# YifanXu74/MQ-Det

Measured on AMD Instinct MI355X. Metric: images/sec MQ-GLIP-T 800×1333 5-shot vision queries, 1/2/4/8 MI355X, higher is better.
Workload: dtype f16; 1 GPU; BASELINE.json configs[1]: MQ-GLIP-T (Swin-T + BERT-base + GCP + 6-layer VLDyHead), 5 vision queries x 40 classes, 141-token caption, LVIS-style post-processing; every step a full forward (feature / language caches OFF; only host-side tokenizer / query-selection results are memoised)); global_batch=8, batch_per_gpu=8, image=800x1333 -> 800x1344, parallelism=dp1, weights=seeded random init (no checkpoints offline), residual_streams=fp32

## Files before the change

include/mqdet_hip.h:

```cpp
#ifndef MQDET_HIP_H
#define MQDET_HIP_H
#ifdef __cplusplus
extern "C" {
#endif

int mq_abi_version(void);

long mq_attn_workspace_bytes(int B, int H, int Nq, int D, int nsplit);
int mq_attn_fwd(const void* q, const void* k, const void* vt, void* o, const float* key_bias, const int* kv_len,
                const unsigned char* qk_mask, long mask_bs, long mask_hs, long mask_rs, void* workspace,
                int B, int H, int Nq, int Nk, int D,
                long q_bs, long q_rs, long q_hs, long k_bs, long k_rs, long k_hs, long vt_bs, long vt_rs, long vt_hs,
                long o_bs, long o_rs, long bias_bs, long bias_hs, float scale, float clamp, int nsplit, void* stream);

int mq_attn_resident_fwd(const void* q, const void* k, const void* vt, void* o, const float* key_bias, const int* kv_len,
                         const unsigned char* qk_mask, long mask_bs, long mask_hs, long mask_rs, int B, int H, int Nq, int Nk, int D,
                         long q_bs, long q_rs, long q_hs, long k_bs, long k_rs, long k_hs, long vt_bs, long vt_rs, long vt_hs,
                         long o_bs, long o_rs, long bias_bs, long bias_hs, float scale, float clamp, void* stream);

int mq_attn_chunked_fwd(const void* q, const void* k, const void* vt, void* o, const float* key_bias, const int* kv_len,
                        void* workspace, int B, int H, int Nq, int Nk, int D,
                        long q_bs, long q_rs, long q_hs, long k_bs, long k_rs, long k_hs, long vt_bs, long vt_rs, long vt_hs,
                        long o_bs, long o_rs, long bias_bs, long bias_hs, float scale, float clamp, int nsplit, void* stream);

int mq_window_attn_fwd(const void* qkv, const void* qkv_bias, const float* rel_bias, void* out,
                       int B, int H, int W, int C, int heads, int ws, int shift, void* stream);
int mq_window_attn_qkv_fwd(const void* x, const void* w, const void* bias, const float* rel_bias, void* out,
                           int B, int H, int W, int C, int heads, int ws, int shift, void* stream);

int mq_gcp_sparse_attn_fwd(const void* q, const void* kv, const int* idx, void* out, int B, int T, int V, int S,
                           int heads, int dim_head, void* stream);

int mq_gcp_gate_residual_fwd(const void* sup, const void* h, const void* w2, const void* x, int x_f32, void* out,
                             float* gate_out, long M, int C, int G, void* stream);

int mq_vlfuse_i2t_fwd(const void* v_ln, const void* kf, const void* vo, long kv_bs, long kv_hs, long kv_ts, const float* bias, const int* kv_len,
                      const void* out_bias, void* out, int B, int N, int T, int heads, int max_kv, float clamp, int variant,
                      void* stream);

long mq_vlfuse_t2i_workspace_bytes(int B, int T, int nsplit);
int mq_vlfuse_t2i_fwd(const void* kf, long kv_bs, long kv_hs, long kv_ts, const void* v_ln, const int* kv_len, const unsigned char* key_mask,
                      long key_mask_bs, void* workspace, void* out, int B, int N, int T, int heads, int nsplit, int max_kv, float clamp, int variant,
                      void* stream);

int mq_layernorm_fwd(const void* x, int x_f32, const void* res, int res_f32, const void* gamma, const void* beta, void* y,
                     float* y32, void* xsum, long rows, int C, float eps, void* stream);

int mq_layernorm2_fwd(const void* x, int x_f32, const void* res, int res_f32, const void* gamma, const void* beta, void* y,
                     float* y32, void* xsum, long rows, int C, float eps, void* stream);
int mq_layernorm_clamp_fwd(const void* x, int x_f32, const void* res, int res_f32, const void* gamma, const void* beta, void* y, float* y32,
                           void* xsum, long rows, int C, float eps, float clamp, void* stream);
int mq_clamp_gelu_clamp(const void* x, void* out, long n, float clamp, void* stream);

int mq_patch_merge_ln_fwd(const void* x, int x_f32, const void* gamma, const void* beta, void* y, int B, int H, int W, int C, float eps,
                          void* stream);

int mq_swin_mlp2_fwd(const float* x, const void* delta, const void* ln_g, const void* ln_b, float eps, const void* w1f,
                     const void* b1, const void* w2f, const void* b2, float* out, const void* next_g, const void* next_b,
                     float eps_next, void* y, long M, int C, int flags, void* stream);

int mq_conv3x3_fwd(const void* x, const void* w, const void* bias, void* out, int B, int H, int W, int C, long x_bs,
                   int N, int out_ld, int stride, void* stream);
int mq_conv3x3_nchw32_fwd(const void* x, const void* w, const void* bias, float* out, int B, int H, int W, int C, long x_bs,
                          int N, void* stream);

int mq_conv3x3_nchw32_v2_fwd(const void* x, const void* w, const void* bias, float* out, int B, int H, int W, int C, long x_bs,
                          int N, void* stream);
typedef struct mq_conv_level {
  const void* x; float* out; long x_bs; int H, W;
} mq_conv_level;
int mq_conv3x3_nchw32_group_fwd(const mq_conv_level* levels, int nl, const void* w, const void* bias, int B, int C, int N, void* stream);
int mq_pool2x2_tokens_fwd(const mq_conv_level* levels, int nl, void* out, int B, int C, void* stream);
int mq_dcnv2_stats_blocks(int H, int W, int stride);
typedef struct mq_dcn_branch {
  const void* x; const float* om; const void* w; const void* bias; void* out; float* stats; const float* wy; const float* wx;
  long x_bs;
  int B, H, W, C, oH, oW, N, out_ld, stride, flags;
} mq_dcn_branch;
int mq_dcnv2_group_fwd(const mq_dcn_branch* branches, int n, void* stream);
int mq_dcnv2_fwd(const void* x, const float* om, const void* w, const void* bias, void* out, float* stats, const float* wy,
                 const float* wx, int B, int H, int W, int C, long x_bs, int oH, int oW, int N, int out_ld, int stride,
                 int flags, void* stream);

int mq_dyconv_stats(const void* y, float* sums, const float* wy, const float* wx, int B, int n, int W, int C, void* stream);
typedef struct mq_coef_branch {
  const float* sums; const void* gamma; const void* beta; float* coef; int nblk, n, nbranches, reserved;
} mq_coef_branch;
int mq_dyconv_coef_group(const mq_coef_branch* branches, int nbr, const float* attn_w, const float* attn_b, int B, int C, int G,
                         float eps, void* stream);
int mq_dyconv_coef(const float* sums, const void* gamma, const void* beta, const float* attn_w, const float* attn_b,
                   float* coef, int B, int n, int nblk, int C, int G, float eps, int nbranches, void* stream);
int mq_dyconv_fuse(const void* y0, const float* coef0, int hs0, int ws0, const void* y1, const float* coef1, int hs1,
                   int ws1, const void* y2, const float* coef2, int hs2, int ws2, int nbranches, void* out, long out_bs,
                   float* pool, int B, int H, int W, int C, void* stream);
int mq_dyrelu_coef(const float* pool, const void* w0, const void* b0, const void* w2, const void* b2, float* coef,
                   int B, int n, int C, void* stream);
typedef struct mq_fuse_level {
  const void* y[3]; const float* coef[3]; int hs[3], ws[3];
  int nbranches, H, W, reserved;
  void* out; long out_bs; float* pool; float* relu_coef;
} mq_fuse_level;
int mq_dyconv_epilogue_group(const mq_fuse_level* levels, int nl, const void* w0, const void* b0, const void* w2, const void* b2,
                             int B, int C, void* stream);
int mq_dyrelu_apply(void* x, const float* coef, int B, int n, int C, long x_bs, void* stream);
int mq_add_upsample_nearest(void* dst, const void* src, int B, int H, int W, int Hc, int Wc, int C, void* stream);
int mq_dyrelu_ln_fwd(const void* x, long x_bs, const float* coef, const int* row_first, int NL, const void* gamma, const void* beta,
                     float eps, void* y, int B, int N, int C, void* stream);

int mq_align_scores_fwd(const void* dot, int dot_f32, const float* tbias, const int* tokidx, long tok_bs, const void* ctr,
                        float* out, float* cls_out, int B, int HW, int T, int L, int MT, float thr, long dot_bs, int agg,
                        void* stream);

int mq_align_fused_fwd(const void* tok, const void* tk, const float* tbias, const void* wbc, const float* bbc, const float* scales,
                       const int* tokidx, long tok_bs, const int* lvl_off, float* ranked, float* cls_out, float* reg, float* ctr_out,
                       float* logits, int B, int N, int T, int kv_max, int L, int MT, int NL, float thr, int agg, void* stream);

int mq_box_decode(const float* val, const long* flat, const void* reg, int reg_f32, const float* anchors, const int* label_ids, long lab_bs,
                  const float* im_wh, float* boxes, float* scores, int* labels, int B, int K, int HW, int L,
                  long out_stride, long out_off, void* stream);

int mq_roi_align_fwd(const void* feat, int feat_f32, const float* rois, float* out, int R, int C, int H, int W,
                     long sn, long sc, long sh, long sw, int PH, int PW, float spatial_scale, int sampling_ratio,
                     int aligned, int reduce_mean, void* stream);

int mq_msdeform_attn_fwd(const void* value, int value_f32, const long* shapes, const long* level_start, const float* loc,
                         const float* attn, void* out, int out_f32, int B, int S, int M, int D, int L, int Q, int P, void* stream);

int mq_msdeform_attn_q_fwd(const void* value, int value_f32, long value_bs, long value_ts, const long* shapes,
                           const long* level_start, const void* qproj, const float* ref, int ref_dim, const int* valid_hw,
                           void* out, int out_f32, int B, int S, int M, int D, int L, int Q, int P, void* stream);

long mq_ml_nms_workspace_bytes(int B, int N);
int mq_ml_nms(const float* boxes, const int* labels, const int* nvalid, void* workspace, unsigned char* keep,
              int B, int N, float thr, void* stream);

int mq_ml_nms_topk(const float* boxes, const int* labels, const int* nvalid, void* workspace, unsigned char* keep,
                   int B, int N, float thr, int max_keep, void* stream);

int mq_patch_embed_fwd(const void* img, int img_f32, const void* w, const float* bias, const float* g0, const float* b0, const float* g1,
                       const float* b1, float* x32, void* h1, int B, int Hi, int Wi, int C, float eps, void* stream);

int mq_attn_text_fwd(const void* q, const void* k, const void* v, void* o, const float* key_bias, const int* kv_len,
                     int B, int H, int Nq, int Nk, int D, long q_bs, long q_rs, long q_hs, long k_bs, long k_rs, long k_hs,
                     long v_bs, long v_rs, long v_hs, long o_bs, long o_rs, long bias_bs, long bias_hs, float scale,
                     float clamp, int max_kv, void* stream);

long mq_post_select_workspace_bytes(const int* hw, const int* k, int NL, int B, int L);
int mq_post_select_fwd(const float* const* ranked, const float* const* reg, const float* const* anchors, const int* hw, const int* k,
                       int NL, int B, int L, const int* label_ids, long lab_bs, const float* im_wh, void* workspace, float* boxes,
                       float* scores, int* labels, int* ids, void* stream);
int mq_post_sort_fwd(const float* boxes, const float* scores, const int* labels, const int* off, int NL, float* boxes_o, float* scores_o,
                     int* labels_o, int* nvalid, int B, int tot, void* stream);
int mq_post_finalize_fwd(const float* boxes, const float* scores, const int* labels, const unsigned char* keep, float* out,
                         int* counts, int B, int tot, int K, int K2, void* stream);

int mq_tta_ingest_fwd(const unsigned char* src, const long* src_off, const int* meta, const int* bounds, const int* coef, float* out,
                      float* out_flip, int* err, int B, int Hp, int Wp, int TH, int R, const float* mean, const float* stdv, int bgr, int x255,
                      void* stream);
int mq_tta_merge_prep(const float* packed, const int* counts, const float* tparam, const float* band, const int* cls_rank,
                      int n_cls, float* boxes, float* scores, int* labels, unsigned char* valid, float* boxes_s, float* scores_s,
                      int* labels_s, int* src_s, int* nvalid, int* ndrop, int T, int B, int K, void* stream);
int mq_tta_merge_finalize(const float* boxes_s, const float* scores_s, const int* labels_s, const int* src_s, const unsigned char* keep,
                          const int* nvalid, float* thr, const int* cls_rank, float* boxes_o, float* scores_o, long long* labels_o, int* counts, int B, int N,
                          int top_n, void* stream);

int mq_lvis_match(const int* pair_dt, const int* pair_gt, const unsigned char* pair_nel, const float* dt_box, const double* gt_box,
                  const double* gt_area, const unsigned char* gt_ign, const unsigned char* gt_nz, const double* area_rng, const double* iou_thr,
                  unsigned long long* dt_bits, int* gt_count, unsigned char* ws, int P, long Ng, void* stream);
int mq_lvis_accumulate(const int* cat_off, const int* order, const unsigned long long* dt_bits, const int* num_gt, const double* rec_thr,
                       double* precision, double* recall, int K, void* stream);

int mq_bank_admit(const float* cand, const long long* sorted_labels, const long long* order, float* pool, float* inv_norm, int* slots, int* counts,
                  int* state, int N, int D, int pool_rows, int cap, int label_lo, int num_labels, int maxq, int exclude, float thr, void* stream);

int mq_gcp_attn_fwd(const float* x, float* x_out, void* y, float* gate_out, const void* kv, const int* idx, const void* wq, const void* wout,
                    const void* wg1, const void* w2, const void* ln_a_g, const void* ln_a_b, const void* ln_g_g, const void* ln_g_b,
                    const void* ln_f_g, const void* ln_f_b, long M, int T, int V, int S, int C, int heads, int dim_head, int G, float eps,
                    int rows_per_block, void* stream);

int mq_bert_attn_qkv_fwd(const void* x, const void* w, const void* bias, void* o, const float* key_bias, const int* kv_len,
                         int B, int T, int C, int H, long x_bs, long x_rs, long o_bs, long o_rs, long bias_bs, float scale, float clamp,
                         void* stream);

#ifdef __cplusplus
#define MQ_BF16_TWIN(name) extern decltype(name) name##_bf16;
#else
#define MQ_BF16_TWIN(name) extern __typeof__(name) name##_bf16;
#endif
MQ_BF16_TWIN(mq_attn_fwd)
MQ_BF16_TWIN(mq_attn_resident_fwd)
MQ_BF16_TWIN(mq_attn_text_fwd)
MQ_BF16_TWIN(mq_bert_attn_qkv_fwd)
MQ_BF16_TWIN(mq_patch_embed_fwd)
MQ_BF16_TWIN(mq_attn_chunked_fwd)
MQ_BF16_TWIN(mq_window_attn_fwd)
MQ_BF16_TWIN(mq_window_attn_qkv_fwd)
MQ_BF16_TWIN(mq_gcp_sparse_attn_fwd)
MQ_BF16_TWIN(mq_gcp_gate_residual_fwd)
MQ_BF16_TWIN(mq_gcp_attn_fwd)
MQ_BF16_TWIN(mq_vlfuse_i2t_fwd)
MQ_BF16_TWIN(mq_vlfuse_t2i_fwd)
MQ_BF16_TWIN(mq_layernorm_fwd)
MQ_BF16_TWIN(mq_layernorm2_fwd)
MQ_BF16_TWIN(mq_layernorm_clamp_fwd)
MQ_BF16_TWIN(mq_clamp_gelu_clamp)
MQ_BF16_TWIN(mq_patch_merge_ln_fwd)
MQ_BF16_TWIN(mq_swin_mlp2_fwd)
MQ_BF16_TWIN(mq_conv3x3_fwd)
MQ_BF16_TWIN(mq_conv3x3_nchw32_fwd)
MQ_BF16_TWIN(mq_conv3x3_nchw32_v2_fwd)
MQ_BF16_TWIN(mq_conv3x3_nchw32_group_fwd)
MQ_BF16_TWIN(mq_dcnv2_fwd)
MQ_BF16_TWIN(mq_dcnv2_group_fwd)
MQ_BF16_TWIN(mq_dyconv_stats)
MQ_BF16_TWIN(mq_dyconv_coef)
MQ_BF16_TWIN(mq_dyconv_coef_group)
MQ_BF16_TWIN(mq_dyconv_fuse)
MQ_BF16_TWIN(mq_dyrelu_coef)
MQ_BF16_TWIN(mq_dyconv_epilogue_group)
MQ_BF16_TWIN(mq_dyrelu_apply)
MQ_BF16_TWIN(mq_add_upsample_nearest)
MQ_BF16_TWIN(mq_pool2x2_tokens_fwd)
MQ_BF16_TWIN(mq_dyrelu_ln_fwd)
MQ_BF16_TWIN(mq_align_scores_fwd)
MQ_BF16_TWIN(mq_align_fused_fwd)
MQ_BF16_TWIN(mq_box_decode)
MQ_BF16_TWIN(mq_roi_align_fwd)
MQ_BF16_TWIN(mq_msdeform_attn_fwd)
MQ_BF16_TWIN(mq_msdeform_attn_q_fwd)

#ifdef __cplusplus
#define MQ_F32_TWIN(name) extern decltype(name) name##_f32;
#else
#define MQ_F32_TWIN(name) extern __typeof__(name) name##_f32;
#endif
MQ_F32_TWIN(mq_attn_fwd)
MQ_F32_TWIN(mq_attn_resident_fwd)
MQ_F32_TWIN(mq_attn_text_fwd)
MQ_F32_TWIN(mq_bert_attn_qkv_fwd)
MQ_F32_TWIN(mq_patch_embed_fwd)
MQ_F32_TWIN(mq_attn_chunked_fwd)
MQ_F32_TWIN(mq_window_attn_fwd)
MQ_F32_TWIN(mq_window_attn_qkv_fwd)
MQ_F32_TWIN(mq_gcp_sparse_attn_fwd)
MQ_F32_TWIN(mq_gcp_gate_residual_fwd)
MQ_F32_TWIN(mq_gcp_attn_fwd)
MQ_F32_TWIN(mq_vlfuse_i2t_fwd)
MQ_F32_TWIN(mq_vlfuse_t2i_fwd)
MQ_F32_TWIN(mq_layernorm_fwd)
MQ_F32_TWIN(mq_layernorm2_fwd)
MQ_F32_TWIN(mq_layernorm_clamp_fwd)
MQ_F32_TWIN(mq_clamp_gelu_clamp)
MQ_F32_TWIN(mq_patch_merge_ln_fwd)
MQ_F32_TWIN(mq_swin_mlp2_fwd)
MQ_F32_TWIN(mq_conv3x3_fwd)
MQ_F32_TWIN(mq_conv3x3_nchw32_fwd)
MQ_F32_TWIN(mq_conv3x3_nchw32_v2_fwd)
MQ_F32_TWIN(mq_conv3x3_nchw32_group_fwd)
MQ_F32_TWIN(mq_dcnv2_fwd)
MQ_F32_TWIN(mq_dcnv2_group_fwd)
MQ_F32_TWIN(mq_dyconv_stats)
MQ_F32_TWIN(mq_dyconv_coef)
MQ_F32_TWIN(mq_dyconv_coef_group)
MQ_F32_TWIN(mq_dyconv_fuse)
MQ_F32_TWIN(mq_dyrelu_coef)
MQ_F32_TWIN(mq_dyconv_epilogue_group)
MQ_F32_TWIN(mq_dyrelu_apply)
MQ_F32_TWIN(mq_dyrelu_ln_fwd)
MQ_F32_TWIN(mq_add_upsample_nearest)
MQ_F32_TWIN(mq_pool2x2_tokens_fwd)
MQ_F32_TWIN(mq_align_scores_fwd)
MQ_F32_TWIN(mq_align_fused_fwd)
MQ_F32_TWIN(mq_box_decode)
MQ_F32_TWIN(mq_msdeform_attn_fwd)
MQ_F32_TWIN(mq_msdeform_attn_q_fwd)

#ifdef __cplusplus
}
#endif
#endif
```

mq_det_amd/build.py:

```python
import os
import subprocess
import sys

HERE = os.path.dirname(os.path.abspath(__file__))
CSRC = os.path.join(HERE, "csrc")
LIB_DIR = os.path.join(HERE, "lib")
LIB = os.path.join(LIB_DIR, "libmqdet_hip.so")
SOURCES = ["api.hip", "attn.hip", "attn_resident.hip", "attn_text.hip", "bert_attn.hip", "vlfuse_attn.hip", "window_attn.hip", "patch_embed.hip", "gcp.hip", "gcp_fused.hip", "conv_igemm.hip", "conv_small.hip", "conv_small2.hip", "conv_small3.hip", "dcn_fused.hip", "layernorm.hip", "layernorm2.hip", "dyconv.hip", "post.hip", "post2.hip", "align_fused.hip", "nms2.hip", "roi_align.hip", "swin_mlp2.hip", "msda.hip", "tta.hip", "lvis_eval.hip", "query_bank.hip"]
F32_SKIP = ("roi_align.hip", "nms2.hip", "post2.hip", "tta.hip", "lvis_eval.hip", "query_bank.hip")
FLAGS = ["--offload-arch=gfx950", "-O3", "-std=c++17", "-fPIC"]
EXTRA_FLAGS = {"dcn_fused.hip": ["-fno-slp-vectorize"],
               "swin_mlp2.hip": ["-fno-slp-vectorize"],
               "attn_resident.hip": ["-fno-slp-vectorize", "-mllvm", "-amdgpu-mfma-vgpr-form"],
               "attn_text.hip": ["-fno-slp-vectorize", "-mllvm", "-amdgpu-mfma-vgpr-form"],
               "bert_attn.hip": ["-fno-slp-vectorize", "-mllvm", "-amdgpu-mfma-vgpr-form"]}


STAMP = os.path.join(LIB_DIR, "libmqdet_hip.stamp")


def _digest():
    import hashlib
    h = hashlib.sha256()
    deps = sorted(os.path.join(CSRC, f) for f in os.listdir(CSRC)) + [os.path.join(HERE, "..", "include", "mqdet_hip.h"), os.path.abspath(__file__)]
    for d in deps:
        if os.path.isfile(d):
            with open(d, "rb") as f:
                h.update(os.path.basename(d).encode() + b"\0" + f.read())
    return h.hexdigest()


def _stale():
    if not os.path.exists(LIB) or not os.path.exists(STAMP):
        return True
    with open(STAMP) as f:
        return f.read().strip() != _digest()


def build(force=False, verbose=True):
    if not force and not _stale():
        return LIB
    os.makedirs(LIB_DIR, exist_ok=True)
    digest = _digest()
    hipcc = os.environ.get("HIPCC", "/opt/rocm/bin/hipcc")
    objs = []
    procs = []
    for src in SOURCES:
        for suffix, defs in (("", []), ("_bf16", ["-DMQ_BF16"]), ("_f32", ["-DMQ_F32"])):
            if suffix and src == "api.hip":
                continue
            if suffix == "_f32" and src in F32_SKIP:
                continue
            obj = os.path.join(LIB_DIR, src.replace(".hip", suffix + ".o"))
            objs.append(obj)
            procs.append((src + suffix, subprocess.Popen([hipcc, *FLAGS, *EXTRA_FLAGS.get(src, []), *defs, "-c", os.path.join(CSRC, src), "-o", obj],
                                                         stdout=subprocess.PIPE, stderr=subprocess.STDOUT)))
    for src, p in procs:
        out, _ = p.communicate()
        if p.returncode != 0:
            raise RuntimeError(f"hipcc failed on {src}:\n{out.decode()}")
    subprocess.check_call([hipcc, "--offload-arch=gfx950", "-shared", "-fPIC", *objs, "-o", LIB])
    with open(STAMP, "w") as f:
        f.write(digest)
    if verbose:
        print(f"built {LIB}")
    return LIB


if __name__ == "__main__":
    build(force="--force" in sys.argv)
```

mq_det_amd/modeling/pipeline.py:

```python
import math
import os

import torch
import torch.nn.functional as F

from .. import ops

NEG = -1.0e30


def _pack_swin(P, sd, SW, p, device, dtype):
    def h(name):
        return sd[name].detach().to(device=device, dtype=dtype).contiguous()
    ws = SW.WINDOW_SIZE
    N = ws * ws
    for i, (depth, heads) in enumerate(zip(SW.DEPTHS, SW.NUM_HEADS)):
        for j in range(depth):
            b = f"{p}.layers.{i}.blocks.{j}.attn"
            idx = sd[b + ".relative_position_index"].to(device).reshape(-1)
            rel = sd[b + ".relative_position_bias_table"].detach().to(device=device, dtype=torch.float32)[idx]
            rel = rel.reshape(N, N, heads).permute(2, 0, 1)
            NP = ops.window_pad(ws)
            P[b + ".rel_bias"] = F.pad(rel, (0, NP - N, 0, NP - N)).contiguous()
    P["_swin_fused_mlp"] = bool(SW.get("FUSED_MLP", True)) and P["_r32"] and ops.KERNELS["SWIN_MLP_VARIANT"] == 2
    P["_swin_fused_widths"] = tuple(w for w in SW.get("FUSED_MLP_WIDTHS", ops.SWIN_MLP_WIDTHS) if w in ops.SWIN_MLP_WIDTHS)
    for i, depth in enumerate(SW.DEPTHS):
        Ci = SW.EMBED_DIM * 2 ** i
        if P["_swin_fused_mlp"] and Ci in P["_swin_fused_widths"]:
            for j in range(depth):
                b = f"{p}.layers.{i}.blocks.{j}.mlp"
                P[b + ".w1f"], P[b + ".w2f"] = ops.swin_mlp2_pack(h(b + ".fc1.weight"), h(b + ".fc2.weight"))
    w = sd[p + ".patch_embed.proj.weight"].detach().to(device=device, dtype=torch.float32)
    P[p + ".patch_embed.lin"] = w.permute(0, 2, 3, 1).reshape(w.shape[0], -1).to(dtype).contiguous()
    if w.shape[0] in (96, 192) and tuple(w.shape[1:]) == (3, 4, 4):
        P[p + ".patch_embed.wpk"] = ops.patch_embed_pack(w).to(dtype).contiguous()
        P[p + ".patch_embed.wpk_nchw"] = ops.patch_embed_pack(w, nchw=True).to(dtype).contiguous()
        P[p + ".patch_embed.f32"] = [sd[n].detach().to(device=device, dtype=torch.float32).contiguous() for n in
                                     (p + ".patch_embed.proj.bias", p + ".patch_embed.norm.weight", p + ".patch_embed.norm.bias",
                                      p + ".layers.0.blocks.0.norm1.weight", p + ".layers.0.blocks.0.norm1.bias")]


def _pack_language(P, sd, cfg, p, device, dtype):
    def h(name):
        return sd[name].detach().to(device=device, dtype=dtype).contiguous()

    def f32(name):
        return sd[name].detach().to(device=device, dtype=torch.float32).contiguous()
    LB = cfg.MODEL.LANGUAGE_BACKBONE
    nl = LB.get("NUM_HIDDEN_LAYERS", 12)
    for i in range(nl):
        _pack_bert_layer(P, sd, f"{p}.encoder.layer.{i}", device, dtype)
    if cfg.VISION_QUERY.ENABLED:
        qv0 = LB.get("QV_START", 6)
        for i in range(nl - qv0):
            b = f"{p}.encoder.qv_layer.{i}"
            P[b + ".ff.linear2.gated"] = (f32(b + ".ff.linear2.weight") * torch.tanh(f32(b + ".ff_gate"))).to(dtype)
            P[b + ".attn_gate.w2"] = h(b + ".attn_gate.linear2.weight").reshape(-1)
            for n in (".attn.to_q", ".attn.to_out", ".attn_gate.linear1"):
                _pack_frag(P, b + n + ".frag", h(b + n + ".weight"))
        for i in range(2):
            b = f"{p}.pre_select.layers.{i}.image_condition"
            wkv = h(b + ".to_kv.weight")
            half = wkv.shape[0] // 2
            P[b + ".to_k.weight"], P[b + ".to_v.weight"] = wkv[:half].contiguous(), wkv[half:].contiguous()


def _pack_frag(P, key, w):
    if w.shape[0] % 16 == 0 and w.shape[1] % 32 == 0:
        P[key] = ops.pack_b_fragments(w)


def _pack_bert_layer(P, sd, b, device, dtype):
    def h(name):
        return sd[name].detach().to(device=device, dtype=dtype).contiguous()
    P[b + ".qk.weight"] = torch.cat([h(b + ".attention.self.query.weight"), h(b + ".attention.self.key.weight")], 0)
    P[b + ".qk.bias"] = torch.cat([h(b + ".attention.self.query.bias"), h(b + ".attention.self.key.bias")], 0)
    P[b + ".qkv.weight"] = torch.cat([P[b + ".qk.weight"], h(b + ".attention.self.value.weight")], 0)
    P[b + ".qkv.bias"] = torch.cat([P[b + ".qk.bias"], h(b + ".attention.self.value.bias")], 0)
    _pack_frag(P, b + ".qkv.frag", P[b + ".qkv.weight"])


def _dcn_tiles(P, key):
    if ops.dcn_bdma():
        P[key + ".tiles"] = ops.dcn_weight_tiles(P[key + ".packed"])


def _dcn_w(P, key):
    return P[key + ".tiles"] if (ops.dcn_bdma() and (key + ".tiles") in P) else P[key + ".packed"]


def build_plan(sd, cfg, device, dtype=torch.float16):
    P = {}
    M = cfg.MODEL
    P["_r32"] = bool(M.get("RESIDUAL_FP32", True))

    def h(name):
        return sd[name].detach().to(device=device, dtype=dtype).contiguous()

    def f32(name):
        return sd[name].detach().to(device=device, dtype=torch.float32).contiguous()
    for k, v in sd.items():
        if v.dtype.is_floating_point:
            P[k] = v.detach().to(device=device, dtype=dtype).contiguous()
    _pack_swin(P, sd, M.SWINT, "backbone.body", device, dtype)
    for k in list(P):
        if torch.is_tensor(P[k]) and P[k].dim() == 4:
            P[k] = P[k].contiguous(memory_format=torch.channels_last)
    _pack_language(P, sd, cfg, "language_backbone.body.model", device, dtype)

    def bert(b):
        _pack_bert_layer(P, sd, b, device, dtype)
    D = M.DYHEAD
    hd = 2048 // 8
    for i in range(D.NUM_CONVS):
        b = f"rpn.head.dyhead_tower.{3 * i}.b_attn"
        sc = hd ** -0.5
        P[b + ".q.weight"] = (f32(b + ".attn.v_proj.weight") * sc).to(dtype)
        P[b + ".q.bias"] = (f32(b + ".attn.v_proj.bias") * sc).to(dtype)
        gv, gl = f32(b + ".gamma_v"), f32(b + ".gamma_l")
        P[b + ".ov.weight"] = (f32(b + ".attn.out_v_proj.weight") * gv[:, None]).to(dtype)
        P[b + ".ov.bias"] = (f32(b + ".attn.out_v_proj.bias") * gv).to(dtype)
        P[b + ".ol.weight"] = (f32(b + ".attn.out_l_proj.weight") * gl[:, None]).to(dtype)
        P[b + ".ol.bias"] = (f32(b + ".attn.out_l_proj.bias") * gl).to(dtype)
        P[b + ".Wov8"] = P[b + ".ov.weight"].reshape(-1, 8, hd).permute(1, 2, 0).contiguous()
        P[b + ".Wq8"] = P[b + ".q.weight"].reshape(8, hd, -1).contiguous()
        P[b + ".bq8"] = (f32(b + ".attn.v_proj.bias") * sc).reshape(8, hd).contiguous()
        wol = (f32(b + ".attn.out_l_proj.weight") * gl[:, None]).reshape(-1, 8, hd)
        wvv = f32(b + ".attn.values_v_proj.weight").reshape(8, hd, -1)
        P[b + ".olc.weight"] = torch.einsum("ohe,hec->ohc", wol, wvv).reshape(wol.shape[0], -1).to(dtype).contiguous()
        P[b + ".olc.bias"] = (torch.einsum("ohe,he->o", wol, f32(b + ".attn.values_v_proj.bias").reshape(8, hd))
                              + f32(b + ".attn.out_l_proj.bias") * gl).to(dtype)
        wl = f32(b + ".attn.l_proj.weight").reshape(8, hd, -1)
        bl = f32(b + ".attn.l_proj.bias").reshape(8, hd)
        wvl = f32(b + ".attn.values_l_proj.weight").reshape(8, hd, -1)
        bvl = f32(b + ".attn.values_l_proj.bias").reshape(8, hd)
        wq8 = (f32(b + ".attn.v_proj.weight") * sc).reshape(8, hd, -1)
        bq8 = (f32(b + ".attn.v_proj.bias") * sc).reshape(8, hd)
        wov8 = (f32(b + ".attn.out_v_proj.weight") * gv[:, None]).reshape(-1, 8, hd).permute(1, 2, 0)
        w_kf = torch.einsum("hec,hek->hck", wq8, wl).reshape(8 * wq8.shape[2], -1)
        b_kf = torch.einsum("hec,he->hc", wq8, bl).reshape(-1)
        w_vo = torch.einsum("heo,hek->hok", wov8, wvl).reshape(8 * wov8.shape[2], -1)
        b_vo = torch.einsum("heo,he->ho", wov8, bvl).reshape(-1)
        w_b = torch.einsum("he,hek->hk", bq8, wl)
        b_b = (bq8 * bl).sum(-1)
        z = w_b.new_zeros(8, w_b.shape[1])
        P[b + ".tprep.weight"] = torch.cat([w_kf, w_vo, w_b, z], 0).to(dtype).contiguous()
        P[b + ".tprep.bias"] = torch.cat([b_kf, b_vo, b_b, b_b.new_zeros(8)], 0).to(dtype).contiguous()
        bert(f"rpn.head.dyhead_tower.{3 * i + 1}")
        b = f"rpn.head.dyhead_tower.{3 * i + 2}"
        for k in range(3):
            w = f32(f"{b}.DyConv.{k}.conv.weight")
            P[f"{b}.DyConv.{k}.packed"] = w.permute(0, 2, 3, 1).reshape(w.shape[0], -1).to(dtype).contiguous()
            _dcn_tiles(P, f"{b}.DyConv.{k}")
        wo = f32(b + ".offset.weight").permute(0, 2, 3, 1).reshape(27, -1)
        P[b + ".offset.packed"] = torch.cat([wo, wo.new_zeros(5, wo.shape[1])], 0).to(dtype).contiguous()
        P[b + ".attn_w"] = f32(b + ".AttnConv.1.weight").reshape(-1)
        P[b + ".attn_b"] = f32(b + ".AttnConv.1.bias")
    for n in ("fpn_layer2", "fpn_layer3", "fpn_layer4", "top_blocks.p6", "top_blocks.p7"):
        w = f32(f"backbone.fpn.{n}.weight")
        P[f"backbone.fpn.{n}.packed"] = w.permute(0, 2, 3, 1).reshape(w.shape[0], -1).to(dtype).contiguous()
        _dcn_tiles(P, f"backbone.fpn.{n}")
    for n in ("fpn_inner2", "fpn_inner3", "fpn_inner4"):
        P[f"backbone.fpn.{n}.lin"] = h(f"backbone.fpn.{n}.weight").reshape(sd[f"backbone.fpn.{n}.weight"].shape[0], -1).contiguous()
    for l in range(5):
        s = f32(f"rpn.head.scales.{l}.scale")
        wb = (f32("rpn.head.bbox_pred.weight") * s).reshape(4, -1)
        wc = f32("rpn.head.centerness.weight").reshape(1, -1)
        P[f"rpn.head.boxctr.{l}.weight"] = torch.cat([wb, wc, wb.new_zeros(3, wb.shape[1])], 0).to(dtype).contiguous()
        P[f"rpn.head.boxctr.{l}.bias"] = torch.cat([f32("rpn.head.bbox_pred.bias") * s, f32("rpn.head.centerness.bias"),
                                                    wb.new_zeros(3)], 0).to(dtype).contiguous()
    wbc = torch.cat([f32("rpn.head.bbox_pred.weight").reshape(4, -1), f32("rpn.head.centerness.weight").reshape(1, -1)], 0)
    P["rpn.head.wbc"] = torch.cat([wbc, wbc.new_zeros(11, wbc.shape[1])], 0).to(dtype).contiguous()
    P["rpn.head.bbc"] = torch.cat([f32("rpn.head.bbox_pred.bias"), f32("rpn.head.centerness.bias"), wbc.new_zeros(3)], 0).contiguous()
    P["rpn.head.scales"] = torch.cat([f32(f"rpn.head.scales.{l}.scale").reshape(1) for l in range(5)], 0).contiguous()
    P["rpn.head.tok.weight"] = f32("rpn.head.dot_product_projection_text.weight")
    P["rpn.head.tok.bias"] = f32("rpn.head.dot_product_projection_text.bias")
    P["rpn.head.bias_lang32"] = f32("rpn.head.bias_lang")
    P["rpn.head.bias0_32"] = f32("rpn.head.bias0")
    P["rpn.head.inv_scale"] = float(math.exp(-float(sd["rpn.head.log_scale"])))
    for l in range(5):
        P[f"anchors.cell.{l}"] = f32(f"rpn.anchor_generator.cell_anchors.{l}")
    return P


def _ln(P, name, x, eps=1e-5, **kw):
    return ops.layer_norm(x.contiguous(), P[name + ".weight"], P[name + ".bias"], eps, **kw)


def _add_ln(P, name, x, res, eps=1e-5, **kw):
    return ops.layer_norm(x.contiguous(), P[name + ".weight"], P[name + ".bias"], eps, residual=res.contiguous(), **kw)


def _lin(P, name, x):
    return F.linear(x, P[name + ".weight"], P.get(name + ".bias"))


_NSPLIT_TARGET = int(os.environ.get("MQ_NSPLIT_TARGET", "768"))


def _nsplit(n_blocks, n_key_tiles, target=None):
    target = target or _NSPLIT_TARGET
    if n_blocks >= 256 or n_key_tiles < 8:
        return 1
    return max(1, min(n_key_tiles // 4, -(-target // n_blocks), 32))


def _nsplit_t2i(n_img, heads, t_live, n_key_tiles, cus_per_xcd=32):
    if n_key_tiles < 8:
        return 1
    members = -(-(heads * (-(-t_live // 16))) // 8)
    best, best_cost = 1, None
    for ns in range(1, min(32, n_key_tiles // 4) + 1):
        per_xcd = -(-(n_img * ns) // 8) * members
        cost = (-(-per_xcd // cus_per_xcd)) * (-(-n_key_tiles // ns) + 6)
        if best_cost is None or cost < best_cost:
            best, best_cost = ns, cost
    return best


def swin_forward(P, cfg, img, p="backbone.body", SW=None):
    M = SW if SW is not None else cfg.MODEL.SWINT
    ws = M.WINDOW_SIZE
    _, _, H0, W0 = img.shape
    if W0 % 4 or H0 % 4:
        img = F.pad(img, (0, (4 - W0 % 4) % 4, 0, (4 - H0 % 4) % 4))
    B, Cin, Hi, Wi = img.shape
    H, W = Hi // 4, Wi // 4
    r32 = P["_r32"]
    h1_first = None
    nhwc = img.permute(0, 2, 3, 1)
    pe = ops.KERNELS["PATCH_EMBED_FUSED"] == 1 and r32 and Cin == 3 and (p + ".patch_embed.wpk") in P
    if pe and img.dtype == torch.float32 and img.is_contiguous():
        x, h1_first = ops.patch_embed(img, P[p + ".patch_embed.wpk_nchw"], *P[p + ".patch_embed.f32"], eps=1e-5)
    elif pe and img.dtype != torch.float32 and nhwc.is_contiguous():
        x, h1_first = ops.patch_embed(nhwc, P[p + ".patch_embed.wpk"], *P[p + ".patch_embed.f32"], eps=1e-5)
    else:
        if img.dtype == torch.float32:
            nhwc = nhwc.to(P[p + ".patch_embed.lin"].dtype)
        patches = nhwc.reshape(B, H, 4, W, 4, Cin).permute(0, 1, 3, 2, 4, 5).reshape(B, H * W, 16 * Cin)
        x = F.linear(patches, P[p + ".patch_embed.lin"], P[p + ".patch_embed.proj.bias"])
        x = _ln(P, p + ".patch_embed.norm", x, want_y=not r32, want_y32=r32)
    outs = []
    for i, (depth, heads) in enumerate(zip(M.DEPTHS, M.NUM_HEADS)):
        C = x.shape[-1]
        fused = P["_swin_fused_mlp"] and C in P["_swin_fused_widths"] and x.dtype == torch.float32
        pend = None
        h1 = None
        if i == 0 and h1_first is not None:
            h1 = h1_first
        for j in range(depth):
            b = f"{p}.layers.{i}.blocks.{j}"
            shift = 0 if j % 2 == 0 else ws // 2
            if h1 is None:
                if pend is None:
                    h1 = _ln(P, b + ".norm1", x)
                else:
                    h1, x = _add_ln(P, b + ".norm1", pend, x)
            if ops.window_qkv_fused(C, ws, h1.numel()):
                a = ops.window_attention_qkv(h1.reshape(B, H, W, C), P[b + ".attn.qkv.weight"], P[b + ".attn.qkv.bias"],
                                             P[b + ".attn.rel_bias"], heads, ws, shift)
            else:
                qkv = _lin(P, b + ".attn.qkv", h1).reshape(B, H, W, 3 * C)
                a = ops.window_attention(qkv, P[b + ".attn.qkv.bias"], P[b + ".attn.rel_bias"], heads, ws, shift)
            proj = _lin(P, b + ".attn.proj", a.reshape(B, H * W, C))
            if fused:
                nxt = f"{p}.layers.{i}.blocks.{j + 1}.norm1" if j + 1 < depth else (f"{p}.norm{i}" if i > 0 else None)
                nln = None if nxt is None else (P[nxt + ".weight"], P[nxt + ".bias"], 1e-5)
                r = ops.swin_mlp2(x.contiguous(), proj.contiguous(), P[b + ".norm2.weight"], P[b + ".norm2.bias"], 1e-5,
                                  P[b + ".mlp.w1f"], P[b + ".mlp.fc1.bias"], P[b + ".mlp.w2f"], P[b + ".mlp.fc2.bias"], next_ln=nln)
                x, h1 = r if nxt is not None else (r, None)
                pend = None
            else:
                h2, x = _add_ln(P, b + ".norm2", proj, x)
                pend = _lin(P, b + ".mlp.fc2", F.gelu(_lin(P, b + ".mlp.fc1", h2)))
                h1 = None
        if fused:
            if i > 0:
                outs.append(h1.reshape(B, H, W, C))
        elif i > 0:
            o, x = _add_ln(P, f"{p}.norm{i}", pend, x)
            outs.append(o.reshape(B, H, W, C))
        else:
            x = x + pend
        if i < len(M.DEPTHS) - 1:
            d = f"{p}.layers.{i}.downsample"
            if ops.KERNELS["PATCH_MERGE_FUSED"] == 1:
                yn = ops.patch_merge_ln(x.reshape(B, H, W, C).contiguous(), P[d + ".norm.weight"], P[d + ".norm.bias"], 1e-5)
                H, W = (H + 1) // 2, (W + 1) // 2
            else:
                y = x.reshape(B, H, W, C)
                if H % 2 or W % 2:
                    y = F.pad(y, (0, 0, 0, W % 2, 0, H % 2))
                y = torch.cat([y[:, 0::2, 0::2], y[:, 1::2, 0::2], y[:, 0::2, 1::2], y[:, 1::2, 1::2]], -1)
                H, W = (H + 1) // 2, (W + 1) // 2
                yn = _ln(P, d + ".norm", y.reshape(B, H * W, 4 * C))
            wr = P[d + ".reduction.weight"]
            if r32 and yn.is_cuda and yn.dtype != torch.float32 and os.environ.get("MQ_SWIN_RED_F32OUT") == "1":
                x = torch.mm(yn.reshape(-1, yn.shape[-1]), wr.t(), out_dtype=torch.float32).view(B, H * W, wr.shape[0])
            else:
                x = F.linear(yn, wr)
                if r32:
                    x = x.float()
    return outs


def fpn_forward(P, feats_nhwc):
    p = "backbone.fpn"
    c3, c4, c5 = feats_nhwc

    def lateral(name, x):
        return F.linear(x, P[f"{p}.{name}.lin"], P[f"{p}.{name}.bias"])

    def conv3(name, x, stride=1):
        return ops.conv3x3(x, P[f"{p}.{name}.packed"], P[f"{p}.{name}.bias"], P[f"{p}.{name}.packed"].shape[0], stride)
    via_dcn = ops.KERNELS["FPN_VIA_DCN"] == 1
    inner = lateral("fpn_inner4", c5)
    inners = [("fpn_layer4", inner)]
    for feat, idx in ((c4, 3), (c3, 2)):
        lat = lateral(f"fpn_inner{idx}", feat)
        if ops.KERNELS["FPN_TOPDOWN_FUSED"] == 1:
            inner = ops.add_upsample_nearest_(lat.contiguous(), inner.contiguous())
        else:
            up = F.interpolate(inner.permute(0, 3, 1, 2), size=lat.shape[1:3], mode="nearest").permute(0, 2, 3, 1)
            inner = (lat + up).contiguous()
        inners.insert(0, (f"fpn_layer{idx}", inner))
    if via_dcn:
        outs = ops.dcnv2_group([dict(x=x, om=_zero_offsets(x.shape[0], x.shape[1], x.shape[2], x.device), w=_dcn_w(P, f"{p}.{n}"),
                                     bias=P[f"{p}.{n}.bias"], stride=1, plain=True) for n, x in inners], want_stats=False, tag="dcnv2_fpn")
        res = [y.reshape(x.shape[0], hw[0], hw[1], 256) for (y, hw, _), (_, x) in zip(outs, inners)]

        def conv3s2(name, x):
            Ho, Wo = (x.shape[1] - 1) // 2 + 1, (x.shape[2] - 1) // 2 + 1
            y, hw = ops.dcnv2(x, _zero_offsets(x.shape[0], Ho, Wo, x.device), _dcn_w(P, f"{p}.{name}"), P[f"{p}.{name}.bias"], 2, tag="dcnv2_fpn", plain=True)
            return y.reshape(x.shape[0], hw[0], hw[1], 256)
        p6 = conv3s2("top_blocks.p6", res[-1])
        p7 = conv3s2("top_blocks.p7", F.relu(p6))
    else:
        res = [conv3(n, x) for n, x in inners]
        p6 = conv3("top_blocks.p6", res[-1], 2)
        p7 = conv3("top_blocks.p7", F.relu(p6), 2)
    return [t.permute(0, 3, 1, 2) for t in res + [p6, p7]]


_ZERO_OM = {}


def _zero_offsets(B, Ho, Wo, device):
    key = (B, Ho, Wo, str(device))
    if key not in _ZERO_OM:
        if len(_ZERO_OM) > 64:
            _ZERO_OM.clear()
        om = torch.zeros(B, 27, Ho, Wo, dtype=torch.float32, device=device)
        om[:, 18:] = 100.0
        _ZERO_OM[key] = om
    return _ZERO_OM[key]


def pooled_fpn_tokens(feats):
    if ops.KERNELS.get("POOLED_TOKENS_FUSED", 0) == 1 and ops.pool2x2_tokens_supported(feats):
        return ops.pool2x2_tokens(feats)
    return torch.cat([F.avg_pool2d(f, 2).permute(0, 2, 3, 1).flatten(1, 2) for f in feats], 1)


def bert_layer(P, b, x, key_bias, clamp, kv_len=None, x32=None, qk_mask=None, max_kv=0):
    Bn, T, C = x.shape
    r32 = x32 is not None
    if ops.KERNELS["BERT_ATTN_QKV_FUSED"] >= 1 and qk_mask is None and (b + ".qkv.frag") in P and ops.bert_attention_qkv_fits(T, C, 12, key_bias, batch=Bn):
        ctx = ops.bert_attention_qkv(x, P[b + ".qkv.frag"], P[b + ".qkv.bias"], 12, key_bias=key_bias, clamp=50000.0 if clamp else 0.0, kv_len=kv_len, packed=True)
    elif ops.KERNELS["BERT_QKV_FUSED"] == 1 and qk_mask is None and ops.attention_text_fits(T, kv_len, max_kv) and (b + ".qkv.weight") in P \
            and (key_bias is None or key_bias.dim() == 2):
        ctx = ops.attention_text(_lin(P, b + ".qkv", x), 12, key_bias=key_bias, clamp=50000.0 if clamp else 0.0, kv_len=kv_len, max_kv=max_kv)
    else:
        qk = _lin(P, b + ".qk", x)
        vt = torch.baddbmm(P[b + ".attention.self.value.bias"][None, :, None], P[b + ".attention.self.value.weight"][None]
                           .expand(Bn, -1, -1), x.transpose(1, 2))
        ctx = ops.attention(qk[:, :, :C], qk[:, :, C:], vt, 12, C // 12, key_bias=key_bias, clamp=50000.0 if clamp else 0.0,
                            kv_len=kv_len, qk_mask=qk_mask)
    a = _add_ln(P, b + ".attention.output.LayerNorm", _lin(P, b + ".attention.output.dense", ctx), x32 if r32 else x, 1e-12,
                want_sum=False, want_y32=r32)
    a16, a32 = a if r32 else (a, None)
    hmid = _lin(P, b + ".intermediate.dense", a16)
    if clamp and ops.KERNELS["BERT_CLAMP_FUSED"] == 1 and hmid.numel() % 8 == 0:
        o = _lin(P, b + ".output.dense", ops.clamp_gelu_clamp(hmid.contiguous(), 50000.0))
        return ops.layer_norm(o.contiguous(), P[b + ".output.LayerNorm.weight"], P[b + ".output.LayerNorm.bias"], 1e-12,
                              residual=(a32 if r32 else a16).contiguous(), want_sum=False, want_y32=r32, clamp=50000.0)
    if clamp:
        hmid = F.gelu(hmid.clamp(-50000, 50000)).clamp(-50000, 50000)
        o = _lin(P, b + ".output.dense", hmid).clamp(-50000, 50000)
    else:
        o = _lin(P, b + ".output.dense", F.gelu(hmid))
    y = _add_ln(P, b + ".output.LayerNorm", o, a32 if r32 else a16, 1e-12, want_sum=False, want_y32=r32)
    if not r32:
        return y.clamp(-50000, 50000) if clamp else y
    y16, y32 = y
    if clamp:
        y16, y32 = y16.clamp(-50000, 50000), y32.clamp(-50000, 50000)
    return y16, y32


def pre_select(P, p, vision, image, scale, side_ok=False):
    vision, image = vision * scale, image * scale
    Bn, Np, C = image.shape
    pad = (-Np) % 8
    if pad:
        image = F.pad(image, (0, 0, 0, pad))

    def image_kv(i):
        ic = f"{p}.layers.{i}.image_condition"
        kn = _ln(P, ic + ".norm_kv", image)
        return F.linear(kn, P[ic + ".to_k.weight"]), torch.matmul(P[ic + ".to_v.weight"], kn.transpose(1, 2))
    ahead = None
    if side_ok and image.is_cuda:
        main, side = torch.cuda.current_stream(), _side_streams(image.device, 1, "pre_kv")[0]
        side.wait_stream(main)
        with torch.cuda.stream(side):
            ahead = image_kv(1)
    for i in range(2):
        b = f"{p}.layers.{i}"
        ic = b + ".image_condition"
        q = F.linear(_ln(P, ic + ".norm", vision), P[ic + ".to_q.weight"])
        if i == 1 and ahead is not None:
            main.wait_stream(side)
            k, vt = ahead
        else:
            k, vt = image_kv(i)
        nq_tiles = -(-q.shape[1] // 128)
        att = ops.attention(q, k, vt, 8, 32, nk=Np, nsplit=_nsplit(nq_tiles * Bn * 8, -(-Np // 64)))
        v16 = vision if vision.dtype == image.dtype else vision.to(image.dtype)
        res = F.linear(v16, P[b + ".res_mapping.weight"]) if (b + ".res_mapping.weight") in P else vision
        att_o = F.linear(att, P[ic + ".to_out.weight"])
        vision = att_o.float() + res.float() if P["_r32"] else att_o + res
        ff = b + ".ff"
        vision = vision + F.linear(F.gelu(F.linear(_ln(P, ff + ".norm", vision), P[ff + ".linear1.weight"])),
                                   P[ff + ".linear2.weight"])
    return vision


def gcp_kv(P, b, vision):
    return F.linear(_ln(P, b + ".attn.norm_kv", vision), P[b + ".attn.to_kv.weight"])


def gcp_block(P, b, x, vision, idx, gates=None, kv=None):
    if kv is None:
        kv = gcp_kv(P, b, vision)
    ff = b + ".ff"
    if ops.KERNELS["GCP_ATTN_FUSED"] >= 1 and (b + ".attn.to_q.frag") in P and ops.gcp_attention_fits(x, idx, policy=True):
        def ln(n):
            return (P[n + ".weight"], P[n + ".bias"])
        r = ops.gcp_attention(x.contiguous(), kv.contiguous(), idx, P[b + ".attn.to_q.frag"], P[b + ".attn.to_out.frag"], P[b + ".attn_gate.linear1.frag"],
                              P[b + ".attn_gate.w2"], ln(b + ".attn.norm"), ln(b + ".attn_gate.norm"), ln(ff + ".norm"), want_gate=gates is not None,
                              packed=True)
        x, xn = r[0], r[1]
        if gates is not None:
            gates.append(r[2])
        return x + F.linear(F.gelu(F.linear(xn, P[ff + ".linear1.weight"])), P[ff + ".linear2.gated"])
    q = F.linear(_ln(P, b + ".attn.norm", x), P[b + ".attn.to_q.weight"])
    sup = F.linear(ops.gcp_sparse_attention(q, kv, idx), P[b + ".attn.to_out.weight"])
    gh = F.linear(_ln(P, b + ".attn_gate.norm", sup), P[b + ".attn_gate.linear1.weight"])
    if gates is not None:
        x, g = ops.gcp_gate_residual(sup, gh, P[b + ".attn_gate.w2"], x.contiguous(), want_gate=True)
        gates.append(g)
    else:
        x = ops.gcp_gate_residual(sup, gh, P[b + ".attn_gate.w2"], x.contiguous())
    return x + F.linear(F.gelu(F.linear(_ln(P, ff + ".norm", x), P[ff + ".linear1.weight"])), P[ff + ".linear2.gated"])


def language_front(P, cfg, input_ids, attention_mask, use_vq, p="language_backbone.body.model", position_ids=None, qk_mask=None, max_kv=0):
    LB = cfg.MODEL.LANGUAGE_BACKBONE
    T = input_ids.shape[1]
    pe = P[p + ".embeddings.position_embeddings.weight"]
    e = P[p + ".embeddings.word_embeddings.weight"][input_ids].float() \
        + P[p + ".embeddings.token_type_embeddings.weight"][0].float() \
        + (pe[:T].float()[None] if position_ids is None else pe[position_ids].float())
    x32 = F.layer_norm(e, (e.shape[-1],), P[p + ".embeddings.LayerNorm.weight"].float(),
                       P[p + ".embeddings.LayerNorm.bias"].float(), 1e-12)
    x = x32.to(P[p + ".embeddings.LayerNorm.weight"].dtype)
    if not P["_r32"]:
        x32 = None
    key_bias = kv_len = None
    if attention_mask is not None:
        key_bias = ((1.0 - attention_mask.float()) * NEG).contiguous()
        kv_len = (attention_mask.to(torch.int32) * torch.arange(1, T + 1, device=attention_mask.device, dtype=torch.int32)) \
            .amax(1).to(torch.int32).contiguous()
    nl, qv0 = LB.get("NUM_HIDDEN_LAYERS", 12), LB.get("QV_START", 6)
    n_front = qv0 if use_vq else nl
    hidden = []
    for i in range(n_front):
        x, x32 = _bert(P, f"{p}.encoder.layer.{i}", x, x32, key_bias, False, kv_len, qk_mask, max_kv=max_kv)
        hidden.append(x if x32 is None else x32)
    return {"x": x, "x32": x32, "hidden": hidden, "key_bias": key_bias, "kv_len": kv_len, "next": n_front, "qk_mask": qk_mask}


def _bert(P, b, x, x32, key_bias, clamp, kv_len, qk_mask=None, max_kv=0):
    if x32 is None:
        return bert_layer(P, b, x, key_bias, clamp, kv_len, qk_mask=qk_mask, max_kv=max_kv), None
    return bert_layer(P, b, x, key_bias, clamp, kv_len, x32=x32, qk_mask=qk_mask, max_kv=max_kv)


def language_backbone(P, cfg, input_ids, attention_mask, vision, images, idx, want_gates=False, front=None, max_kv=0, side_ok=False):
    p = "language_backbone.body.model"
    LB = cfg.MODEL.LANGUAGE_BACKBONE
    use_vq = vision is not None
    if front is None:
        front = language_front(P, cfg, input_ids, attention_mask, use_vq, max_kv=max_kv)
    x, x32, hidden, key_bias, kv_len = front["x"], front.get("x32"), list(front["hidden"]), front["key_bias"], front["kv_len"]
    nl, qv0 = LB.get("NUM_HIDDEN_LAYERS", 12), LB.get("QV_START", 6)
    kv_ahead, kv_join = {}, None
    if use_vq:
        vision = pre_select(P, p + ".pre_select", vision, images, cfg.VISION_QUERY.VISION_SCALE, side_ok=side_ok)
        first = max(front["next"], qv0)
        if side_ok and vision.is_cuda and nl - first > 1:
            main, side = torch.cuda.current_stream(), _side_streams(vision.device, 1, "gcp_kv")[0]
            side.wait_stream(main)
            with torch.cuda.stream(side):
                for i in range(first + 1, nl):
                    kv_ahead[i] = gcp_kv(P, f"{p}.encoder.qv_layer.{i - qv0}", vision)
            kv_join = (main, side)
    gates = [] if want_gates else None
    for i in range(front["next"], nl):
        if use_vq and i >= qv0:
            if kv_join is not None and i in kv_ahead:
                kv_join[0].wait_stream(kv_join[1])
                kv_join = None
            if x32 is None:
                x = gcp_block(P, f"{p}.encoder.qv_layer.{i - qv0}", x, vision, idx, gates, kv=kv_ahead.get(i))
            else:
                x32 = gcp_block(P, f"{p}.encoder.qv_layer.{i - qv0}", x32, vision, idx, gates, kv=kv_ahead.get(i))
                x = x32.to(x.dtype)
        x, x32 = _bert(P, f"{p}.encoder.layer.{i}", x, x32, key_bias, False, kv_len, max_kv=max_kv)
        hidden.append(x if x32 is None else x32)
    n = LB.N_LAYERS
    feats = hidden[-1].float() if n == 1 else torch.stack(hidden[-n:], 1).float().mean(1) / n
    m = attention_mask.unsqueeze(-1).float()
    embedded = feats * m
    aggregate = embedded.sum(1) / attention_mask.sum(-1, keepdim=True).float()
    return {"aggregate": aggregate, "embedded": embedded, "masks": attention_mask, "hidden": x, "hidden32": x32,
            "key_bias": key_bias, "kv_len": kv_len, "vision_query_gates": gates, "augmented_vision": vision}


def _to_tokens(feats):
    sizes = [tuple(f.shape[-2:]) for f in feats]
    return torch.cat([f.permute(0, 2, 3, 1).flatten(1, 2) for f in feats], 1), sizes


def _level_views(tok, sizes):
    Bn, N, C = tok.shape
    out, s = [], 0
    for (hh, ww) in sizes:
        out.append(tok[:, s:s + hh * ww].reshape(Bn, hh, ww, C).permute(0, 3, 1, 2))
        s += hh * ww
    return out


def vl_text_prep(P, b, hidden, key_bias, hidden32=None):
    Bn = hidden.shape[0]
    if hidden32 is not None:
        l_ln, l_res = _ln(P, b + ".layer_norm_l", hidden32, want_y32=True)
    else:
        l_ln = l_res = _ln(P, b + ".layer_norm_l", hidden)
    T = l_ln.shape[1]
    C = P[b + ".Wq8"].shape[2]
    t = _lin(P, b + ".tprep", l_ln)
    kf = t[..., :8 * C].unflatten(-1, (8, C)).permute(0, 2, 1, 3)
    vo = t[..., 8 * C:16 * C].unflatten(-1, (8, C)).permute(0, 2, 1, 3)
    bias = (t[..., 16 * C:16 * C + 8].float().permute(0, 2, 1) + key_bias[:, None, :]).contiguous()
    return {"l_ln": l_ln, "l_res": l_res, "kf": kf, "vo": vo, "bias": bias}


def vl_image_side(P, b, v_ln, prep, kv_len=None, max_kv=0):
    return ops.vlfuse_i2t(v_ln, prep["kf"], prep["vo"], prep["bias"], P[b + ".ov.bias"], kv_len=kv_len, max_kv=max_kv)


def vl_text_side(P, b, v_ln, prep, kv_len=None, max_kv=0):
    Bn, N, _ = v_ln.shape
    T = prep["l_ln"].shape[1]
    t_live = min(T, max_kv) if (kv_len is not None and max_kv > 0) else T
    out_l = ops.vlfuse_t2i(prep["kf"], v_ln, _nsplit_t2i(Bn, prep["kf"].shape[1], t_live, -(-N // 64)), kv_len=kv_len, max_kv=t_live)
    return prep["l_res"] + _lin(P, b + ".olc", out_l)


def vl_fuse_tokens(P, b, v, hidden, key_bias, kv_len=None, max_kv=0):
    v_ln = ops.layer_norm(v, P[b + ".layer_norm_v.weight"], P[b + ".layer_norm_v.bias"], 1e-5)
    prep = vl_text_prep(P, b, hidden, key_bias)
    return vl_image_side(P, b, v_ln, prep, kv_len, max_kv), vl_text_side(P, b, v_ln, prep, kv_len, max_kv)


def vl_fuse(P, b, feats, hidden, key_bias, kv_len=None, max_kv=0):
    v, sizes = _to_tokens(feats)
    v_new, l_new = vl_fuse_tokens(P, b, v.contiguous(), hidden, key_bias, kv_len, max_kv)
    return _level_views(v_new, sizes), l_new


_UP_W = {}


def _upsample_pool_weights(hs, ws, H, W, device):
    key = (hs, ws, H, W, device)
    if key not in _UP_W:
        def axis(n_src, n_dst):
            w = torch.zeros(n_src, dtype=torch.float64)
            for o in range(n_dst):
                s = o * (n_src - 1) / (n_dst - 1) if n_dst > 1 else 0.0
                i0 = min(int(s), n_src - 1)
                i1 = min(i0 + 1, n_src - 1)
                l = s - i0
                w[i0] += 1 - l
                w[i1] += l
            return (w / n_dst).float().to(device)
        _UP_W[key] = (axis(hs, H), axis(ws, W))
    return _UP_W[key]


def dyconv_tokens(P, cfg, b, tok, sizes, defer_relu=False):
    G = cfg.MODEL.GROUP_NORM
    nl = len(sizes)
    Bn, N, C = tok.shape
    offs = [0]
    for (hh, ww) in sizes:
        offs.append(offs[-1] + hh * ww)
    lv = [tok[:, offs[l]:offs[l + 1]].reshape(Bn, sizes[l][0], sizes[l][1], C) for l in range(nl)]
    out = torch.empty_like(tok)
    streams = bool(cfg.MODEL.DYHEAD.get("LEVEL_STREAMS", True) and tok.is_cuda and nl > 1)

    def fan_out(fn):
        if not streams:
            for l in range(nl):
                fn(l)
            return
        main = torch.cuda.current_stream()
        side = _side_streams(tok.device, max(1, min(nl - 1, _LEVEL_SIDE_STREAMS)))
        for s_ in side:
            s_.wait_stream(main)
        for l in range(1, nl):
            with torch.cuda.stream(side[(l - 1) % len(side)]):
                fn(l)
        fn(0)
        for s_ in side:
            main.wait_stream(s_)

    om = [None] * nl

    def offsets(lvl):
        om[lvl] = ops.conv3x3_nchw32(lv[lvl], P[b + ".offset.packed"], P[b + ".offset.bias"], 27)
    if ops.KERNELS["OFFSET_CONV_VARIANT"] == 3 and ops.conv3x3_nchw32_group_supported(lv, 27):
        om = ops.conv3x3_nchw32_group(lv, P[b + ".offset.packed"], P[b + ".offset.bias"], 27)
    else:
        fan_out(offsets)

    branches, owner = [], []
    for lvl in range(nl):
        H, W = sizes[lvl]
        spec = [(1, lv[lvl], 1)]
        if lvl > 0:
            spec.append((2, lv[lvl - 1], 2))
        if lvl < nl - 1:
            spec.append((0, lv[lvl + 1], 1))
        for k, x_nhwc, stride in spec:
            Ho, Wo = (x_nhwc.shape[1] - 1) // stride + 1, (x_nhwc.shape[2] - 1) // stride + 1
            wy = wx = None
            if (Ho, Wo) != (H, W):
                wy, wx = _upsample_pool_weights(Ho, Wo, H, W, tok.device)
            branches.append({"x": x_nhwc, "om": om[lvl], "w": _dcn_w(P, f"{b}.DyConv.{k}"), "bias": P[f"{b}.DyConv.{k}.conv.bias"],
                             "stride": stride, "wy": wy, "wx": wx})
            owner.append((lvl, k, len(spec)))
    ys = ops.dcnv2_group(branches, want_stats=True)
    coefs = ops.dyconv_coef_group(
        [{"sums": sums, "n": Ho * Wo, "gamma": P[f"{b}.DyConv.{k}.bn.weight"], "beta": P[f"{b}.DyConv.{k}.bn.bias"], "nbranches": nb}
         for (lvl, k, nb), (y, (Ho, Wo), sums) in zip(owner, ys)], P[b + ".attn_w"], P[b + ".attn_b"], G.NUM_GROUPS, G.EPSILON)

    relu_coef = torch.empty(nl, Bn, 4, C, dtype=torch.float32, device=tok.device) if defer_relu else None

    def epilogue(lvl):
        H, W = sizes[lvl]
        fused = [(y, coef, Ho, Wo) for (l2, k, nb), (y, (Ho, Wo), sums), coef in zip(owner, ys, coefs) if l2 == lvl]
        o = out[:, offs[lvl]:offs[lvl + 1]]
        _, pool = ops.dyconv_fuse(fused, H, W, out=o)
        rw = (P[b + ".relu.fc.0.weight"], P[b + ".relu.fc.0.bias"], P[b + ".relu.fc.2.weight"], P[b + ".relu.fc.2.bias"])
        if defer_relu:
            ops.dyrelu_coef(pool, H * W, *rw, out=relu_coef[lvl])
        else:
            ops.dyrelu_(o, pool, *rw)
    if ops.KERNELS["DYCONV_EPILOGUE_GROUPED"] == 1 and C == 256 and nl <= 8:
        rw = (P[b + ".relu.fc.0.weight"], P[b + ".relu.fc.0.bias"], P[b + ".relu.fc.2.weight"], P[b + ".relu.fc.2.bias"])
        rc = relu_coef if defer_relu else torch.empty(nl, Bn, 4, C, dtype=torch.float32, device=tok.device)
        ops.dyconv_epilogue_group(
            [([(y, coef, Ho, Wo) for (l2, k, nb), (y, (Ho, Wo), sums), coef in zip(owner, ys, coefs) if l2 == lvl], sizes[lvl][0], sizes[lvl][1],
              out[:, offs[lvl]:offs[lvl + 1]]) for lvl in range(nl)], *rw, rc)
        if not defer_relu:
            fan_out(lambda lvl: ops.dyrelu_apply_(out[:, offs[lvl]:offs[lvl + 1]], rc[lvl]))
    else:
        fan_out(epilogue)
    return (out, relu_coef) if defer_relu else out


def dyconv(P, cfg, b, feats):
    tok, sizes = _to_tokens(feats)
    return _level_views(dyconv_tokens(P, cfg, b, tok.contiguous(), sizes), sizes)


_SIDE_STREAMS = {}
_LEVEL_SIDE_STREAMS = int(os.environ.get("MQ_LEVEL_SIDE_STREAMS", "4"))


_STREAM_PRIORITY = dict((kv.split(":")[0], int(kv.split(":")[1])) for kv in os.environ.get("MQ_STREAM_PRIORITY", "").split(",") if ":" in kv)


def _side_streams(device, n, tag="levels"):
    key = (device.index, n, tag)
    if key not in _SIDE_STREAMS:
        _SIDE_STREAMS[key] = [torch.cuda.Stream(device=device, priority=_STREAM_PRIORITY.get(tag, 0)) for _ in range(n)]
    return _SIDE_STREAMS[key]


def vldyhead(P, cfg, feats, lang, trace=None):
    p = "rpn.head"
    hidden, key_bias, kv_len = lang["hidden"], lang["key_bias"], lang.get("kv_len")
    h32 = lang.get("hidden32")
    max_kv = lang.get("max_kv", 0)
    tok, sizes = _to_tokens(feats)
    tok = tok.contiguous()
    L = cfg.MODEL.DYHEAD.NUM_CONVS
    t = f"{p}.dyhead_tower"
    two_streams = bool(tok.is_cuda and cfg.MODEL.DYHEAD.get("LEVEL_STREAMS", True)) and trace is None

    def text_side(b, v_ln, prep):
        hnew = vl_text_side(P, b, v_ln, prep, kv_len, max_kv)
        return (hnew.to(tok.dtype), hnew) if h32 is not None else (hnew, None)

    defer = ops.KERNELS["DYRELU_IN_LN"] == 1 and tok.shape[-1] == 256 and len(sizes) <= 8
    relu_coef = None

    def relu_applied_copy():
        if relu_coef is None:
            return tok
        cp, off = tok.clone(), 0
        for l, (hh, ww) in enumerate(sizes):
            ops.dyrelu_apply_(cp[:, off:off + hh * ww], relu_coef[l])
            off += hh * ww
        return cp

    def norm_v(b):
        if relu_coef is not None:
            return ops.dyrelu_layer_norm(tok, relu_coef, sizes, P[b + ".layer_norm_v.weight"], P[b + ".layer_norm_v.bias"], 1e-5)
        return ops.layer_norm(tok, P[b + ".layer_norm_v.weight"], P[b + ".layer_norm_v.bias"], 1e-5)

    def dyconv_layer(i):
        if defer and i + 1 < L:
            return dyconv_tokens(P, cfg, f"{t}.{3 * i + 2}", tok, sizes, defer_relu=True)
        return dyconv_tokens(P, cfg, f"{t}.{3 * i + 2}", tok, sizes), None

    if not two_streams:
        for i in range(L):
            b = f"{t}.{3 * i}.b_attn"
            v_ln = norm_v(b)
            prep = vl_text_prep(P, b, hidden, key_bias, h32)
            tok = vl_image_side(P, b, v_ln, prep, kv_len, max_kv)
            hidden, h32 = text_side(b, v_ln, prep)
            rec = {"fuse_tok": tok, "fuse_hidden": hidden if h32 is None else h32}
            hidden, h32 = _bert(P, f"{t}.{3 * i + 1}", hidden, h32, key_bias, True, kv_len, max_kv=max_kv)
            tok, relu_coef = dyconv_layer(i)
            if trace is not None:
                rec.update(bert_hidden=hidden if h32 is None else h32, dyconv_tok=relu_applied_copy())
                trace.append(rec)
    else:
        main, text = torch.cuda.current_stream(), _side_streams(tok.device, 1, "text")[0]
        text.wait_stream(main)
        with torch.cuda.stream(text):
            prep = vl_text_prep(P, f"{t}.0.b_attn", hidden, key_bias, h32)
        keep = []
        for i in range(L):
            b = f"{t}.{3 * i}.b_attn"
            v_ln = norm_v(b)
            main.wait_stream(text)
            keep.clear()
            keep.append(v_ln)
            text.wait_stream(main)
            cur = prep
            with torch.cuda.stream(text):
                hidden, h32 = text_side(b, v_ln, cur)
                hidden, h32 = _bert(P, f"{t}.{3 * i + 1}", hidden, h32, key_bias, True, kv_len, max_kv=max_kv)
                if i + 1 < L:
                    prep = vl_text_prep(P, f"{t}.{3 * (i + 1)}.b_attn", hidden, key_bias, h32)
            tok = vl_image_side(P, b, v_ln, cur, kv_len, max_kv)
            tok, relu_coef = dyconv_layer(i)
        main.wait_stream(text)
        keep.clear()
    emb = F.normalize((hidden if h32 is None else h32).float(), p=2, dim=-1)
    tk = F.linear(emb / 2.0, P[p + ".tok.weight"], P[p + ".tok.bias"]) * P[p + ".inv_scale"]
    tbias = (emb @ P[p + ".bias_lang32"] + P[p + ".bias0_32"]).contiguous()
    live = min(tk.shape[1], max_kv) if max_kv > 0 else tk.shape[1]
    fits = ops.f32_operands() != 1 or -(-live // 16) * 16 <= 144
    if ops.KERNELS["ALIGN_FUSED"] == 1 and tk.shape[1] <= 256 and tok.shape[-1] == 256 and len(sizes) <= 8 and fits:
        return {"tok": tok, "sizes": sizes, "tk16": tk.to(tok.dtype).contiguous(), "tbias": tbias, "max_kv": max_kv,
                "wbc": P[p + ".wbc"], "bbc": P[p + ".bbc"], "scales": P[p + ".scales"],
                "feats": _level_views(tok, sizes), "hidden": hidden if h32 is None else h32}
    tok16_t = tk.to(tok.dtype).transpose(1, 2)
    Bn, N, C = tok.shape
    dots_all = torch.bmm(tok, tok16_t)
    bbox, ctr, dots = [], [], []
    off = 0
    for l, (H, W) in enumerate(sizes):
        tokens = tok[:, off:off + H * W]
        bc = F.linear(tokens, P[f"{p}.boxctr.{l}.weight"], P[f"{p}.boxctr.{l}.bias"]).reshape(Bn, H, W, 8)
        bbox.append(bc[..., :4].permute(0, 3, 1, 2))
        ctr.append(bc[..., 4:5].permute(0, 3, 1, 2))
        dots.append(dots_all[:, off:off + H * W])
        off += H * W
    return {"bbox_reg": bbox, "centerness": ctr, "dot": dots, "tbias": tbias, "feats": _level_views(tok, sizes),
            "hidden": hidden if h32 is None else h32}


def grid_anchors(P, sizes, strides, device):
    out = []
    for l, ((H, W), s) in enumerate(zip(sizes, strides)):
        sx = torch.arange(0, W * s, step=s, dtype=torch.float32, device=device)
        sy = torch.arange(0, H * s, step=s, dtype=torch.float32, device=device)
        yy, xx = torch.meshgrid(sy, sx, indexing="ij")
        sh = torch.stack([xx.reshape(-1), yy.reshape(-1), xx.reshape(-1), yy.reshape(-1)], 1)
        out.append((sh[:, None, :] + P[f"anchors.cell.{l}"][None]).reshape(-1, 4).contiguous())
    return out


TIE_SLOTS = 16


def postprocess(cfg, head, anchors, im_wh, tokidx, label_ids, want_cls=False, level_streams=None):
    A = cfg.MODEL.ATSS
    dev = head["tbias"].device
    Bn = head["tbias"].shape[0]
    L = tokidx.shape[-2]
    if not torch.is_tensor(im_wh):
        im_wh = torch.tensor([[w, h] for (h, w) in im_wh], dtype=torch.float32, device=dev)
    agg = ops.SCORE_AGG[str(cfg.MODEL.DYHEAD.get("SCORE_AGG", "MEAN")).upper()]
    fused = None
    if "tok" in head:
        fused = ops.align_fused(head["tok"], head["tk16"], head["tbias"], head["wbc"], head["bbc"], head["scales"], tokidx, head["sizes"],
                                A.INFERENCE_TH, agg=agg, kv_max=head.get("max_kv", 0), want_cls=want_cls, want_logits=want_cls)
        hws = [h * w for (h, w) in head["sizes"]]
        if want_cls:
            T = head["tbias"].shape[1]
            offs_ = [0]
            for n_ in hws:
                offs_.append(offs_[-1] + n_)
            head["dot"] = [fused["logits"][:, offs_[l]:offs_[l + 1]] for l in range(len(hws))]
            head["bbox_reg"] = [fused["reg"][l].reshape(Bn, h, w, 4).permute(0, 3, 1, 2) for l, (h, w) in enumerate(head["sizes"])]
            head["centerness"] = [fused["ctr"][:, offs_[l]:offs_[l + 1]].reshape(Bn, 1, h, w) for l, (h, w) in enumerate(head["sizes"])]
    else:
        hws = [d.shape[1] for d in head["dot"]]
    ks = [min(A.PRE_NMS_TOP_N, hw * L) for hw in hws]
    tot = sum(ks)
    Kd = int(A.DETECTIONS_PER_IMG)
    K = min(Kd, tot) if Kd > 0 else tot
    K2 = min(K + int(A.get("TIE_SLOTS", TIE_SLOTS)), tot) if Kd > 0 else tot
    if ops.KERNELS["POST_FUSED"] == 1 and tot <= 16384 and (Kd <= 0 or tot <= 6656) and all(a.shape[0] == hw for a, hw in zip(anchors, hws)) \
            and ops.post_select_supported(hws, ks, Bn, L):
        if fused is not None:
            ranked_l, reg_l = fused["ranked"], fused["reg"]
            cls_all = fused["cls"] if want_cls else None
        else:
            ranked_l, reg_l, cls_all = [], [], []
            for l, HW in enumerate(hws):
                ctr_flat = head["centerness"][l].permute(0, 2, 3, 1).reshape(Bn, HW).contiguous()
                r = ops.align_scores(head["dot"][l], head["tbias"], tokidx, ctr_flat, A.INFERENCE_TH, want_cls=want_cls, agg=agg)
                if want_cls:
                    r, c_ = r
                    cls_all.append(c_)
                ranked_l.append(r.float().contiguous())
                reg_l.append(head["bbox_reg"][l].permute(0, 2, 3, 1).reshape(Bn, HW, 4).float().contiguous())
        lab32 = label_ids if label_ids.dtype == torch.int32 else label_ids.to(torch.int32)
        wh32 = im_wh if (im_wh.dtype == torch.float32 and im_wh.is_contiguous()) else im_wh.float().contiguous()
        ub, us, ul, uid = ops.post_select(ranked_l, reg_l, [a.contiguous() for a in anchors], ks, lab32.contiguous(), wh32)
        boxes, scores, labels, nvalid = ops.post_sort(ub, us, ul, ks)
        keep8 = ops.ml_nms(boxes, labels, nvalid, A.NMS_TH, max_keep=K2 if Kd > 0 else 0, as_bool=False)
        packed, cnt = ops.post_finalize(boxes, scores, labels, keep8, K, K2)
        out = {"boxes": packed[..., :4], "scores": packed[..., 4], "labels": packed[..., 5].to(torch.int64), "counts": cnt & 0xFFFF,
               "tie_overflow": (cnt >> 16) > 0, "packed": packed, "counts_packed": cnt,
               "pre_nms": {"boxes": boxes, "scores": scores, "labels": labels, "nvalid": nvalid, "keep": keep8.bool()}}
        if want_cls:
            out["cls"] = cls_all
        return out
    boxes = torch.empty(Bn, tot, 4, dtype=torch.float32, device=dev)
    scores = torch.empty(Bn, tot, dtype=torch.float32, device=dev)
    labels = torch.empty(Bn, tot, dtype=torch.int32, device=dev)
    cls_all = [None] * len(ks)
    offs = [0]
    for k in ks:
        offs.append(offs[-1] + k)

    def level(l):
        anc, k, HW = anchors[l], ks[l], hws[l]
        if fused is not None:
            r, reg_nhwc = fused["ranked"][l], fused["reg"][l]
            if want_cls:
                cls_all[l] = fused["cls"][l]
        else:
            dot, reg, ctr = head["dot"][l], head["bbox_reg"][l], head["centerness"][l]
            ctr_flat = ctr.permute(0, 2, 3, 1).reshape(Bn, HW).contiguous()
            r = ops.align_scores(dot, head["tbias"], tokidx, ctr_flat, A.INFERENCE_TH, want_cls=want_cls, agg=agg)
            if want_cls:
                r, cls_all[l] = r
            reg_nhwc = reg.permute(0, 2, 3, 1).reshape(Bn, HW, 4).contiguous()
        val, flat = torch.topk(r.reshape(Bn, HW * L), k, dim=1, sorted=False)
        ops.box_decode(val.contiguous(), flat.contiguous(), reg_nhwc, anc, label_ids, im_wh, boxes, scores, labels, HW, L, offs[l])

    if level_streams is None:
        level_streams = cfg.MODEL.DYHEAD.get("LEVEL_STREAMS", True)
    if boxes.is_cuda and level_streams and len(ks) > 1:
        main = torch.cuda.current_stream()
        side = _side_streams(dev, len(ks) - 1)
        for s_ in side:
            s_.wait_stream(main)
        for l in range(1, len(ks)):
            with torch.cuda.stream(side[l - 1]):
                level(l)
        level(0)
        for s_ in side:
            main.wait_stream(s_)
    else:
        for l in range(len(ks)):
            level(l)
    order = torch.argsort(scores, dim=1, descending=True, stable=True)
    scores = torch.gather(scores, 1, order)
    labels = torch.gather(labels, 1, order.to(torch.int64)).contiguous()
    boxes = torch.gather(boxes, 1, order[:, :, None].expand(-1, -1, 4)).contiguous()
    nvalid = (scores > 0).sum(1).to(torch.int32)
    keep = ops.ml_nms(boxes, labels, nvalid, A.NMS_TH, max_keep=K2 if Kd > 0 else 0)
    kept_scores = torch.where(keep, scores, torch.full_like(scores, -1.0))
    top, ti = torch.topk(kept_scores, K2, dim=1, sorted=True)
    if K2 > K:
        tie = top[:, K:] == top[:, K - 1:K]
        top = torch.cat([top[:, :K], torch.where(tie, top[:, K:], torch.full_like(top[:, K:], -1.0))], 1)
    overflow = ((top[:, K2 - 1] == top[:, K - 1]) & (top[:, K - 1] > 0)) if 0 < K < K2 < tot else torch.zeros(Bn, dtype=torch.bool, device=dev)
    out = {"boxes": torch.gather(boxes, 1, ti[:, :, None].expand(-1, -1, 4)), "scores": top,
           "labels": torch.gather(labels, 1, ti).to(torch.int64), "counts": (top > 0).sum(1), "tie_overflow": overflow,
           "pre_nms": {"boxes": boxes, "scores": scores, "labels": labels, "nvalid": nvalid, "keep": keep}}
    if want_cls:
        out["cls"] = cls_all
    return out
```

mq_det_amd/ops.py:

```python
import ctypes
import math
import os

import torch

_LIB = None
_LIB_PATH = os.path.join(os.path.dirname(os.path.abspath(__file__)), "lib", "libmqdet_hip.so")

_vp, _i, _l, _f = ctypes.c_void_p, ctypes.c_int, ctypes.c_long, ctypes.c_float
EXPECTED_ABI = 31
_SIGNATURES = {
    "mq_abi_version": (_i, []),
    "mq_attn_workspace_bytes": (_l, [_i, _i, _i, _i, _i]),
    "mq_attn_fwd": (_i, [_vp, _vp, _vp, _vp, _vp, _vp, _vp, _l, _l, _l, _vp, _i, _i, _i, _i, _i] + [_l] * 13 + [_f, _f, _i, _vp]),
    "mq_attn_resident_fwd": (_i, [_vp, _vp, _vp, _vp, _vp, _vp, _vp, _l, _l, _l, _i, _i, _i, _i, _i] + [_l] * 13 + [_f, _f, _vp]),
    "mq_patch_embed_fwd": (_i, [_vp, _i, _vp, _vp, _vp, _vp, _vp, _vp, _vp, _vp, _i, _i, _i, _i, _f, _vp]),
    "mq_attn_text_fwd": (_i, [_vp, _vp, _vp, _vp, _vp, _vp, _i, _i, _i, _i, _i] + [_l] * 13 + [_f, _f, _i, _vp]),
    "mq_bert_attn_qkv_fwd": (_i, [_vp, _vp, _vp, _vp, _vp, _vp, _i, _i, _i, _i, _l, _l, _l, _l, _l, _f, _f, _vp]),
    "mq_attn_chunked_fwd": (_i, [_vp, _vp, _vp, _vp, _vp, _vp, _vp, _i, _i, _i, _i, _i] + [_l] * 13 + [_f, _f, _i, _vp]),
    "mq_window_attn_fwd": (_i, [_vp, _vp, _vp, _vp, _i, _i, _i, _i, _i, _i, _i, _vp]),
    "mq_window_attn_qkv_fwd": (_i, [_vp, _vp, _vp, _vp, _vp, _i, _i, _i, _i, _i, _i, _i, _vp]),
    "mq_gcp_sparse_attn_fwd": (_i, [_vp, _vp, _vp, _vp, _i, _i, _i, _i, _i, _i, _vp]),
    "mq_gcp_gate_residual_fwd": (_i, [_vp, _vp, _vp, _vp, _i, _vp, _vp, _l, _i, _i, _vp]),
    "mq_gcp_attn_fwd": (_i, [_vp] * 16 + [_l, _i, _i, _i, _i, _i, _i, _i, _f, _i, _vp]),
    "mq_vlfuse_i2t_fwd": (_i, [_vp, _vp, _vp, _l, _l, _l, _vp, _vp, _vp, _vp, _i, _i, _i, _i, _i, _f, _i, _vp]),
    "mq_vlfuse_t2i_workspace_bytes": (_l, [_i, _i, _i]),
    "mq_vlfuse_t2i_fwd": (_i, [_vp, _l, _l, _l, _vp, _vp, _vp, _l, _vp, _vp, _i, _i, _i, _i, _i, _i, _f, _i, _vp]),
    "mq_layernorm_fwd": (_i, [_vp, _i, _vp, _i, _vp, _vp, _vp, _vp, _vp, _l, _i, _f, _vp]),
    "mq_layernorm2_fwd": (_i, [_vp, _i, _vp, _i, _vp, _vp, _vp, _vp, _vp, _l, _i, _f, _vp]),
    "mq_layernorm_clamp_fwd": (_i, [_vp, _i, _vp, _i, _vp, _vp, _vp, _vp, _vp, _l, _i, _f, _f, _vp]),
    "mq_clamp_gelu_clamp": (_i, [_vp, _vp, _l, _f, _vp]),
    "mq_patch_merge_ln_fwd": (_i, [_vp, _i, _vp, _vp, _vp, _i, _i, _i, _i, _f, _vp]),
    "mq_swin_mlp2_fwd": (_i, [_vp, _vp, _vp, _vp, _f, _vp, _vp, _vp, _vp, _vp, _vp, _vp, _f, _vp, _l, _i, _i, _vp]),
    "mq_conv3x3_fwd": (_i, [_vp, _vp, _vp, _vp, _i, _i, _i, _i, _l, _i, _i, _i, _vp]),
    "mq_conv3x3_nchw32_fwd": (_i, [_vp, _vp, _vp, _vp, _i, _i, _i, _i, _l, _i, _vp]),
    "mq_conv3x3_nchw32_v2_fwd": (_i, [_vp, _vp, _vp, _vp, _i, _i, _i, _i, _l, _i, _vp]),
    "mq_conv3x3_nchw32_group_fwd": (_i, [_vp, _i, _vp, _vp, _i, _i, _i, _vp]),
    "mq_dcnv2_stats_blocks": (_i, [_i, _i, _i]),
    "mq_dcnv2_fwd": (_i, [_vp, _vp, _vp, _vp, _vp, _vp, _vp, _vp, _i, _i, _i, _i, _l, _i, _i, _i, _i, _i, _i, _vp]),
    "mq_dcnv2_group_fwd": (_i, [_vp, _i, _vp]),
    "mq_dyconv_stats": (_i, [_vp, _vp, _vp, _vp, _i, _i, _i, _i, _vp]),
    "mq_dyconv_coef": (_i, [_vp, _vp, _vp, _vp, _vp, _vp, _i, _i, _i, _i, _i, _f, _i, _vp]),
    "mq_dyconv_coef_group": (_i, [_vp, _i, _vp, _vp, _i, _i, _i, _f, _vp]),
    "mq_dyconv_fuse": (_i, [_vp, _vp, _i, _i, _vp, _vp, _i, _i, _vp, _vp, _i, _i, _i, _vp, _l, _vp, _i, _i, _i, _i, _vp]),
    "mq_dyrelu_coef": (_i, [_vp, _vp, _vp, _vp, _vp, _vp, _i, _i, _i, _vp]),
    "mq_dyconv_epilogue_group": (_i, [_vp, _i, _vp, _vp, _vp, _vp, _i, _i, _vp]),
    "mq_add_upsample_nearest": (_i, [_vp, _vp, _i, _i, _i, _i, _i, _i, _vp]),
    "mq_pool2x2_tokens_fwd": (_i, [_vp, _i, _vp, _i, _i, _vp]),
    "mq_dyrelu_ln_fwd": (_i, [_vp, _l, _vp, _vp, _i, _vp, _vp, _f, _vp, _i, _i, _i, _vp]),
    "mq_dyrelu_apply": (_i, [_vp, _vp, _i, _i, _i, _l, _vp]),
    "mq_align_scores_fwd": (_i, [_vp, _i, _vp, _vp, _l, _vp, _vp, _vp, _i, _i, _i, _i, _i, _f, _l, _i, _vp]),
    "mq_align_fused_fwd": (_i, [_vp, _vp, _vp, _vp, _vp, _vp, _vp, _l, _vp, _vp, _vp, _vp, _vp, _vp, _i, _i, _i, _i, _i, _i, _i, _f, _i, _vp]),
    "mq_box_decode": (_i, [_vp, _vp, _vp, _i, _vp, _vp, _l, _vp, _vp, _vp, _vp, _i, _i, _i, _i, _l, _l, _vp]),
    "mq_roi_align_fwd": (_i, [_vp, _i, _vp, _vp, _i, _i, _i, _i, _l, _l, _l, _l, _i, _i, _f, _i, _i, _i, _vp]),
    "mq_msdeform_attn_fwd": (_i, [_vp, _i, _vp, _vp, _vp, _vp, _vp, _i, _i, _i, _i, _i, _i, _i, _i, _vp]),
    "mq_msdeform_attn_q_fwd": (_i, [_vp, _i, _l, _l, _vp, _vp, _vp, _vp, _i, _vp, _vp, _i, _i, _i, _i, _i, _i, _i, _i, _vp]),
    "mq_post_select_workspace_bytes": (_l, [_vp, _vp, _i, _i, _i]),
    "mq_post_select_fwd": (_i, [_vp, _vp, _vp, _vp, _vp, _i, _i, _i, _vp, _l, _vp, _vp, _vp, _vp, _vp, _vp, _vp]),
    "mq_post_sort_fwd": (_i, [_vp, _vp, _vp, _vp, _i, _vp, _vp, _vp, _vp, _i, _i, _vp]),
    "mq_post_finalize_fwd": (_i, [_vp, _vp, _vp, _vp, _vp, _vp, _i, _i, _i, _i, _vp]),
    "mq_ml_nms_workspace_bytes": (_l, [_i, _i]),
    "mq_ml_nms_topk": (_i, [_vp, _vp, _vp, _vp, _vp, _i, _i, _f, _i, _vp]),
    "mq_ml_nms": (_i, [_vp, _vp, _vp, _vp, _vp, _i, _i, _f, _vp]),
    "mq_tta_ingest_fwd": (_i, [_vp] * 8 + [_i] * 5 + [_vp, _vp, _i, _i, _vp]),
    "mq_tta_merge_prep": (_i, [_vp] * 5 + [_i] + [_vp] * 10 + [_i, _i, _i, _vp]),
    "mq_tta_merge_finalize": (_i, [_vp] * 12 + [_i, _i, _i, _vp]),
    "mq_lvis_match": (_i, [_vp] * 13 + [_i, _l, _vp]),
    "mq_lvis_accumulate": (_i, [_vp] * 7 + [_i, _vp]),
    "mq_bank_admit": (_i, [_vp] * 8 + [_i] * 8 + [_f, _vp]),
}
BF16_TWINS = ("mq_attn_fwd", "mq_attn_resident_fwd", "mq_attn_text_fwd", "mq_bert_attn_qkv_fwd", "mq_patch_embed_fwd", "mq_attn_chunked_fwd", "mq_window_attn_fwd", "mq_window_attn_qkv_fwd", "mq_gcp_sparse_attn_fwd", "mq_gcp_gate_residual_fwd", "mq_gcp_attn_fwd", "mq_vlfuse_i2t_fwd", "mq_vlfuse_t2i_fwd",
              "mq_layernorm_fwd", "mq_layernorm2_fwd", "mq_layernorm_clamp_fwd", "mq_clamp_gelu_clamp", "mq_patch_merge_ln_fwd", "mq_swin_mlp2_fwd", "mq_conv3x3_fwd", "mq_conv3x3_nchw32_fwd", "mq_conv3x3_nchw32_v2_fwd", "mq_conv3x3_nchw32_group_fwd", "mq_dcnv2_fwd", "mq_dcnv2_group_fwd",
              "mq_dyconv_stats", "mq_dyconv_coef", "mq_dyconv_coef_group", "mq_dyconv_fuse", "mq_dyrelu_coef", "mq_dyconv_epilogue_group", "mq_dyrelu_apply", "mq_dyrelu_ln_fwd", "mq_add_upsample_nearest", "mq_pool2x2_tokens_fwd",
              "mq_align_scores_fwd", "mq_align_fused_fwd", "mq_box_decode", "mq_roi_align_fwd", "mq_msdeform_attn_fwd", "mq_msdeform_attn_q_fwd")
F32_TWINS = tuple(n for n in BF16_TWINS if n not in ("mq_roi_align_fwd",))
for _n in BF16_TWINS:
    _SIGNATURES[_n + "_bf16"] = _SIGNATURES[_n]
for _n in F32_TWINS:
    _SIGNATURES[_n + "_f32"] = _SIGNATURES[_n]
EXPORTS = tuple(_SIGNATURES)


from .selection import KERNEL_DEFAULTS, KERNELS, _ThreadLocalTable, configure, activate


def lib_path():
    return _LIB_PATH


def load_library():
    global _LIB
    if _LIB is None:
        if not os.path.exists(_LIB_PATH):
            raise RuntimeError(f"{_LIB_PATH} not found: the MI355X HIP library is required (python -m mq_det_amd.build); "
                               "there is no CPU / eager fallback for the MQ-Det hot path")
        lib = ctypes.CDLL(_LIB_PATH)
        for name, (res, args) in _SIGNATURES.items():
            fn = getattr(lib, name)
            fn.restype, fn.argtypes = res, args
        got = lib.mq_abi_version()
        if got != EXPECTED_ABI:
            raise RuntimeError(f"{_LIB_PATH} has ABI version {got}, these bindings are written for {EXPECTED_ABI}: "
                               "rebuild it (python -m mq_det_amd.build --force)")
        _LIB = lib
    return _LIB


def _stream():
    return ctypes.c_void_p(torch.cuda.current_stream().cuda_stream)


_TIMING = None


def timing_active():
    return _TIMING is not None


def start_timing():
    global _TIMING
    _TIMING = []


def stop_timing():
    global _TIMING
    rec, _TIMING = _TIMING or [], None
    torch.cuda.synchronize()
    out = {}
    for tag, a, b, nb in rec:
        n, t, by = out.get(tag, (0, 0.0, 0))
        out[tag] = (n + 1, t + a.elapsed_time(b), by + nb)
    return out


class _timed:

    def __init__(self, tag, nbytes=0):
        self.tag, self.nbytes = tag, nbytes

    def __enter__(self):
        if _TIMING is not None:
            self.a = torch.cuda.Event(enable_timing=True)
            self.a.record()

    def __exit__(self, *exc):
        if _TIMING is not None:
            b = torch.cuda.Event(enable_timing=True)
            b.record()
            _TIMING.append((self.tag, self.a, b, int(self.nbytes)))


def _ptr(t):
    return ctypes.c_void_p(t.data_ptr()) if t is not None else ctypes.c_void_p(0)


def _chk(rc, name):
    if rc != 0:
        raise RuntimeError(f"{name} failed with code {rc}")


class _OperandTypes:

    def _cur(self):
        return (torch.float32,) if KERNELS.get("F32_OPERANDS", 0) else (torch.float16, torch.bfloat16)

    def __contains__(self, dtype):
        return dtype in self._cur()

    def __iter__(self):
        return iter(self._cur())

    def __getitem__(self, i):
        return self._cur()[i]

    def __add__(self, other):
        return self._cur() + tuple(other)

    def __radd__(self, other):
        return tuple(other) + self._cur()


_H16 = _OperandTypes()


def f32_operands():
    return KERNELS.get("F32_OPERANDS", 0)


def _fn(lib, name, *ts):
    if KERNELS.get("F32_OPERANDS", 0):
        return getattr(lib, name + "_f32") if name in F32_TWINS else getattr(lib, name)
    kinds = {t.dtype for t in ts if t is not None and t.dtype in (torch.float16, torch.bfloat16)}
    if len(kinds) > 1:
        raise TypeError(f"{name}: fp16 and bf16 operands in one call")
    return getattr(lib, name + "_bf16") if torch.bfloat16 in kinds else getattr(lib, name)


def _need_gpu(*ts):
    for t in ts:
        if t is not None and not t.is_cuda:
            raise RuntimeError("mq_det_amd ops need GPU tensors: the hot path has no CPU fallback")


def patch_embed_pack(w, nchw=False):
    C = w.shape[0]
    out = w.new_zeros(C, 64)
    out[:, :48] = w.reshape(C, 48) if nchw else w.permute(0, 2, 3, 1).reshape(C, 48)
    return out.contiguous()


def patch_embed(img, wpk, bias, g0, b0, g1, b1, eps=1e-5):
    lib = load_library()
    _need_gpu(img, wpk, bias, g0, b0, g1, b1)
    f32 = img.dtype == torch.float32
    if f32 and f32_operands() and img.shape[-1] == 3 and img.shape[1] != 3:
        f32 = False
    if f32:
        B, Cin, Hi, Wi = img.shape
    else:
        B, Hi, Wi, Cin = img.shape
    C = wpk.shape[0]
    assert Cin == 3 and img.is_contiguous() and (f32 or img.dtype == wpk.dtype) and wpk.dtype in _H16 and wpk.shape == (C, 64) and wpk.is_contiguous()
    assert all(t.dtype == torch.float32 and t.is_contiguous() and t.numel() == C for t in (bias, g0, b0, g1, b1))
    n = (Hi // 4) * (Wi // 4)
    x32 = torch.empty(B, n, C, dtype=torch.float32, device=img.device)
    h1 = torch.empty(B, n, C, dtype=wpk.dtype, device=img.device)
    with _timed(f"patch_embed_c{C}", img.numel() * img.element_size() + x32.numel() * 4 + h1.numel() * 2):
        _chk(_fn(lib, "mq_patch_embed_fwd", wpk)(_ptr(img), int(f32), _ptr(wpk), _ptr(bias), _ptr(g0), _ptr(b0), _ptr(g1), _ptr(b1), _ptr(x32), _ptr(h1),
                                                 B, Hi, Wi, C, float(eps), _stream()), "mq_patch_embed_fwd")
    return x32, h1


def attention_text_fits(T, kv_len=None, max_kv=0):
    live = max_kv if (kv_len is not None and 0 < max_kv < T) else T
    return T <= 256 and (f32_operands() != 1 or live <= 160)


FUSED_TEXT_MAX_ROWS = 9216
FUSED_BERT_MAX_WORKGROUPS = 768


def bert_attention_qkv_fits(T, C, heads, key_bias=None, batch=None):
    ok = (C == 768 and C == 64 * heads and T <= (160 if f32_operands() == 1 else 256) and (key_bias is None or key_bias.dim() == 2))
    if ok and batch is not None and KERNELS["BERT_ATTN_QKV_FUSED"] == 1:
        ok = batch * heads <= FUSED_BERT_MAX_WORKGROUPS and not f32_operands()
    return ok


def bert_attention_qkv(x, wqkv, bqkv, heads, key_bias=None, clamp=0.0, kv_len=None, scale=None, packed=False):
    lib = load_library()
    _need_gpu(x, wqkv, bqkv, key_bias, kv_len)
    B, T, C = x.shape
    assert bert_attention_qkv_fits(T, C, heads, key_bias) and x.dtype in _H16 and x.stride(2) == 1
    wqkv = _b_fragments(wqkv, 3 * C, C, packed)
    assert bqkv.shape == (3 * C,) and bqkv.is_contiguous() and wqkv.dtype == bqkv.dtype == x.dtype
    bias_bs = 0
    if key_bias is not None:
        assert key_bias.dtype == torch.float32 and key_bias.shape == (B, T) and key_bias.stride(1) == 1
        bias_bs = key_bias.stride(0)
    if kv_len is not None:
        assert kv_len.dtype == torch.int32 and kv_len.shape == (B,) and kv_len.is_contiguous()
    o = torch.empty(B, T, C, dtype=x.dtype, device=x.device)
    D = C // heads
    with _timed(f"bert_attn_qkv_t{T}"):
        rc = _fn(lib, "mq_bert_attn_qkv_fwd", x)(_ptr(x), _ptr(wqkv), _ptr(bqkv), _ptr(o), _ptr(key_bias), _ptr(kv_len), B, T, C, heads,
                                                 x.stride(0), x.stride(1), o.stride(0), o.stride(1), bias_bs,
                                                 float(scale if scale is not None else 1.0 / math.sqrt(D)), float(clamp), _stream())
    _chk(rc, "mq_bert_attn_qkv_fwd")
    return o


def attention_text(qkv, heads, key_bias=None, clamp=0.0, kv_len=None, max_kv=0, scale=None):
    lib = load_library()
    _need_gpu(qkv, key_bias, kv_len)
    B, T, C3 = qkv.shape
    HD = C3 // 3
    D = HD // heads
    assert C3 == 3 * heads * D and qkv.dtype in _H16 and qkv.stride(2) == 1 and T <= 256 and D in (32, 64)
    assert attention_text_fits(T, kv_len, max_kv), "precise mode: mq_attn_text_fwd_f32 holds up to 160 live keys in LDS"
    if kv_len is not None:
        assert kv_len.dtype == torch.int32 and kv_len.shape == (B,) and kv_len.is_contiguous()
        if max_kv > 0 and os.environ.get("MQ_DEBUG_SYNC") == "1":
            assert int(kv_len.max()) <= max(max_kv, 1), f"attention_text: max_kv = {max_kv} < kv_len.max() = {int(kv_len.max())}"
    bias_bs = bias_hs = 0
    if key_bias is not None:
        assert key_bias.dtype == torch.float32 and key_bias.shape[-1] == T and key_bias.stride(-1) == 1
        if key_bias.dim() == 2:
            bias_bs = key_bias.stride(0)
        else:
            bias_bs, bias_hs = key_bias.stride(0), key_bias.stride(1)
    o = torch.empty(B, T, HD, dtype=qkv.dtype, device=qkv.device)
    q, k, v = qkv[:, :, :HD], qkv[:, :, HD:2 * HD], qkv[:, :, 2 * HD:]
    bs, rs = qkv.stride(0), qkv.stride(1)
    with _timed(f"attn_text_d{D}_nq{T}_nk{T}"):
        rc = _fn(lib, "mq_attn_text_fwd", qkv)(_ptr(q), _ptr(k), _ptr(v), _ptr(o), _ptr(key_bias), _ptr(kv_len), B, heads, T, T, D,
                                               bs, rs, D, bs, rs, D, bs, rs, D, o.stride(0), o.stride(1), bias_bs, bias_hs,
                                               float(scale if scale is not None else 1.0 / math.sqrt(D)), float(clamp), int(max_kv), _stream())
    _chk(rc, "mq_attn_text_fwd")
    return o


def attention4(q4, k4, vt4, key_bias=None, scale=None, clamp=0.0, nsplit=1, nk=None, kv_len=None, qk_mask=None):
    lib = load_library()
    _need_gpu(q4, k4, vt4, key_bias, kv_len)
    B, Nq, H, D = q4.shape
    if kv_len is not None:
        assert kv_len.dtype == torch.int32 and kv_len.shape == (B,) and kv_len.is_contiguous()
    Nk = k4.shape[1] if nk is None else nk
    assert k4.shape[0] == B and k4.shape[2:] == (H, D) and vt4.shape[:3] == (B, H, D) and vt4.shape[3] >= Nk
    assert q4.dtype == k4.dtype == vt4.dtype and q4.dtype in _H16
    assert q4.stride(3) == 1 and k4.stride(3) == 1 and vt4.stride(3) == 1
    bias_bs = bias_hs = 0
    if key_bias is not None:
        assert key_bias.dtype == torch.float32 and key_bias.shape[-1] == Nk and key_bias.stride(-1) == 1
        if key_bias.dim() == 2:
            assert key_bias.shape == (B, Nk)
            bias_bs = key_bias.stride(0)
        else:
            assert key_bias.shape == (B, H, Nk)
            bias_bs, bias_hs = key_bias.stride(0), key_bias.stride(1)
    mask_bs = mask_hs = mask_rs = 0
    if qk_mask is not None:
        _need_gpu(qk_mask)
        if qk_mask.dtype == torch.bool:
            qk_mask = qk_mask.view(torch.uint8)
        assert qk_mask.dtype == torch.uint8 and qk_mask.shape == (B, H, Nq, Nk) and qk_mask.stride(3) == 1
        mask_bs, mask_hs, mask_rs = qk_mask.stride(0), qk_mask.stride(1), qk_mask.stride(2)
    o = torch.empty(B, Nq, H * D, dtype=q4.dtype, device=q4.device)
    mask_ok = qk_mask is None or (Nk % 4 == 0 and mask_bs % 4 == 0 and mask_hs % 4 == 0 and mask_rs % 4 == 0 and qk_mask.data_ptr() % 4 == 0)
    if nsplit <= 1 and Nk <= 256 and D in (32, 64) and mask_ok and o.stride(1) % 4 == 0 and KERNELS["ATTN_RESIDENT"] == 1:
        with _timed(f"attn_res_d{D}_nq{Nq}_nk{Nk}"):
            rc = _fn(lib, "mq_attn_resident_fwd", q4)(
                _ptr(q4), _ptr(k4), _ptr(vt4), _ptr(o), _ptr(key_bias), _ptr(kv_len), _ptr(qk_mask), mask_bs, mask_hs, mask_rs,
                B, H, Nq, Nk, D, q4.stride(0), q4.stride(1), q4.stride(2), k4.stride(0), k4.stride(1), k4.stride(2),
                vt4.stride(0), vt4.stride(2), vt4.stride(1), o.stride(0), o.stride(1), bias_bs, bias_hs,
                float(scale if scale is not None else 1.0 / math.sqrt(D)), float(clamp), _stream())
        _chk(rc, "mq_attn_resident_fwd")
        return o
    ws = None
    if nsplit > 1:
        ws = torch.empty(lib.mq_attn_workspace_bytes(B, H, Nq, D, nsplit) // 4, dtype=torch.float32, device=q4.device)
    if qk_mask is None and D in (32, 64) and o.stride(1) % 4 == 0 and KERNELS["ATTN_RESIDENT"] == 1:
        with _timed(f"attn_chk_d{D}_nq{Nq}_nk{Nk}_s{nsplit}"):
            rc = _fn(lib, "mq_attn_chunked_fwd", q4)(
                _ptr(q4), _ptr(k4), _ptr(vt4), _ptr(o), _ptr(key_bias), _ptr(kv_len), _ptr(ws), B, H, Nq, Nk, D,
                q4.stride(0), q4.stride(1), q4.stride(2), k4.stride(0), k4.stride(1), k4.stride(2),
                vt4.stride(0), vt4.stride(2), vt4.stride(1), o.stride(0), o.stride(1), bias_bs, bias_hs,
                float(scale if scale is not None else 1.0 / math.sqrt(D)), float(clamp), int(nsplit), _stream())
        _chk(rc, "mq_attn_chunked_fwd")
        return o
    with _timed(f"attn_d{D}_nq{Nq}_nk{Nk}_s{nsplit}"):
        rc = _fn(lib, "mq_attn_fwd", q4)(_ptr(q4), _ptr(k4), _ptr(vt4), _ptr(o), _ptr(key_bias), _ptr(kv_len), _ptr(qk_mask), mask_bs, mask_hs,
                             mask_rs, _ptr(ws), B, H, Nq, Nk, D,
                             q4.stride(0), q4.stride(1), q4.stride(2), k4.stride(0), k4.stride(1), k4.stride(2),
                             vt4.stride(0), vt4.stride(2), vt4.stride(1), o.stride(0), o.stride(1), bias_bs, bias_hs,
                             float(scale if scale is not None else 1.0 / math.sqrt(D)), float(clamp), int(nsplit), _stream())
    _chk(rc, "mq_attn_fwd")
    return o


def attention(q, k, vt, num_heads, head_dim, key_bias=None, scale=None, clamp=0.0, nsplit=1, nk=None, kv_len=None, qk_mask=None):
    B, Nq, HD = q.shape
    H, D = num_heads, head_dim
    assert HD == H * D and k.shape[2] == HD and vt.shape[1] == HD
    assert q.stride(2) == 1 and k.stride(2) == 1 and vt.stride(2) == 1
    q4 = q.as_strided((B, Nq, H, D), (q.stride(0), q.stride(1), D, 1), q.storage_offset())
    k4 = k.as_strided((B, k.shape[1], H, D), (k.stride(0), k.stride(1), D, 1), k.storage_offset())
    vt4 = vt.as_strided((B, H, D, vt.shape[2]), (vt.stride(0), D * vt.stride(1), vt.stride(1), 1), vt.storage_offset())
    return attention4(q4, k4, vt4, key_bias, scale, clamp, nsplit, nk, kv_len, qk_mask)


def window_pad(ws):
    n = ws * ws
    if n > 160:
        raise ValueError(f"window {ws}x{ws} = {n} tokens: mq_window_attn_fwd supports up to 160")
    return 64 if n <= 64 else 160


def pad_rel_bias(rel_bias, ws=None):
    h, n, _ = rel_bias.shape
    npad = window_pad(ws) if ws is not None else (64 if n <= 64 else 160)
    out = rel_bias.new_zeros(h, npad, npad)
    out[:, :n, :n] = rel_bias
    return out.contiguous()


def window_attention(qkv, qkv_bias, rel_bias, heads, ws, shift):
    lib = load_library()
    _need_gpu(qkv, qkv_bias, rel_bias)
    B, H, W, C3 = qkv.shape
    C = C3 // 3
    NP = window_pad(ws)
    assert qkv.is_contiguous() and qkv.dtype in _H16 and qkv_bias.dtype == qkv.dtype
    if rel_bias.shape == (heads, ws * ws, ws * ws) and ws * ws != NP:
        rel_bias = pad_rel_bias(rel_bias, ws)
    assert rel_bias.dtype == torch.float32 and rel_bias.is_contiguous() and rel_bias.shape == (heads, NP, NP)
    out = torch.empty(B, H, W, C, dtype=qkv.dtype, device=qkv.device)
    with _timed(f"window_attn_c{C}", qkv.numel() * 2 + out.numel() * 2):
        _chk(_fn(lib, "mq_window_attn_fwd", qkv)(_ptr(qkv), _ptr(qkv_bias), _ptr(rel_bias), _ptr(out), B, H, W, C, heads, ws, shift,
                                    _stream()), "mq_window_attn_fwd")
    return out


WINDOW_QKV_WIDTHS = (96, 192)


def window_qkv_fused(C, ws, numel=0):
    k = KERNELS["SWIN_QKV_FUSED"]
    return ws * ws <= 64 and numel < 2 ** 31 and ((k >= 1 and C == 96) or (k >= 2 and C == 192))



def window_attention_qkv(x, w, bias, rel_bias, heads, ws, shift):
    lib = load_library()
    _need_gpu(x, w, bias, rel_bias)
    B, H, W, C = x.shape
    NP = window_pad(ws)
    assert C in WINDOW_QKV_WIDTHS and NP == 64 and heads * 32 == C
    assert x.is_contiguous() and x.dtype in _H16 and w.dtype == x.dtype == bias.dtype and w.is_contiguous() and w.shape == (3 * C, C)
    if rel_bias.shape == (heads, ws * ws, ws * ws) and ws * ws != NP:
        rel_bias = pad_rel_bias(rel_bias, ws)
    assert rel_bias.dtype == torch.float32 and rel_bias.is_contiguous() and rel_bias.shape == (heads, NP, NP)
    out = torch.empty(B, H, W, C, dtype=x.dtype, device=x.device)
    with _timed(f"window_attn_qkv_c{C}", 2 * x.numel() * 2):
        _chk(_fn(lib, "mq_window_attn_qkv_fwd", x)(_ptr(x), _ptr(w), _ptr(bias), _ptr(rel_bias), _ptr(out), B, H, W, C, heads, ws, shift,
                                                   _stream()), "mq_window_attn_qkv_fwd")
    return out


def gcp_sparse_attention(q, kv, idx, heads=8, dim_head=64):
    lib = load_library()
    _need_gpu(q, kv, idx)
    B, T, HD = q.shape
    V, S = kv.shape[1], idx.shape[2]
    assert q.is_contiguous() and kv.is_contiguous() and idx.is_contiguous() and idx.dtype == torch.int32
    assert q.dtype == kv.dtype and q.dtype in _H16 and kv.shape[2] == 2 * HD
    out = torch.empty_like(q)
    with _timed(f"gcp_sparse_attn_s{S}", q.numel() * 4 + kv.numel() * 2):
        _chk(_fn(lib, "mq_gcp_sparse_attn_fwd", q)(_ptr(q), _ptr(kv), _ptr(idx), _ptr(out), B, T, V, S, heads, dim_head, _stream()),
             "mq_gcp_sparse_attn_fwd")
    return out


def gcp_attention_fits(x, idx, policy=False):
    ok = x.dtype == torch.float32 and x.shape[-1] == 768 and idx.shape[-1] <= 8
    if ok and policy and KERNELS["GCP_ATTN_FUSED"] == 1:
        ok = x.numel() // 768 <= FUSED_TEXT_MAX_ROWS and not f32_operands()
    return ok


def pack_b_fragments(w):
    N, K = w.shape
    assert N % 16 == 0 and K % 32 == 0
    return w.view(N // 16, 16, K // 32, 4, 8).permute(0, 2, 3, 1, 4).contiguous().view(N // 16, K // 32, 64, 8)


def unpack_b_fragments(wp):
    nt, ks = wp.shape[:2]
    return wp.view(nt, ks, 4, 16, 8).permute(0, 3, 1, 2, 4).reshape(nt * 16, ks * 32)


def _b_fragments(w, N, K, packed):
    if packed:
        assert w.shape == (N // 16, K // 32, 64, 8) and w.is_contiguous(), "expected pack_b_fragments(weight)"
        return w
    assert w.shape == (N, K)
    return pack_b_fragments(w)


def gcp_attention(x, kv, idx, wq, wout, wg1, w2, ln_a, ln_g, ln_f=None, eps=1e-5, want_gate=False, rows_per_block=0, packed=False):
    lib = load_library()
    _need_gpu(x, kv, idx, wq, wout, wg1, w2)
    B, T, C = x.shape
    V, S = kv.shape[1], idx.shape[2]
    assert gcp_attention_fits(x, idx) and x.is_contiguous() and kv.shape == (B, V, 1024) and kv.is_contiguous() and kv.dtype in _H16
    assert idx.dtype == torch.int32 and idx.shape[:2] == (B, T) and idx.is_contiguous()
    wq, wout, wg1 = _b_fragments(wq, 512, C, packed), _b_fragments(wout, C, 512, packed), _b_fragments(wg1, 384, C, packed)
    assert w2.numel() == 384
    ws = [wq, wout, wg1, w2, *ln_a, *ln_g] + (list(ln_f) if ln_f is not None else [])
    assert all(w.dtype == kv.dtype and w.is_contiguous() for w in ws)
    out = torch.empty_like(x)
    y = torch.empty(B, T, C, dtype=kv.dtype, device=x.device) if ln_f is not None else None
    gate = torch.empty(B, T, dtype=torch.float32, device=x.device) if want_gate else None
    with _timed(f"gcp_attn_fused_s{S}"):
        rc = _fn(lib, "mq_gcp_attn_fwd", kv)(_ptr(x), _ptr(out), _ptr(y), _ptr(gate), _ptr(kv), _ptr(idx), _ptr(wq), _ptr(wout), _ptr(wg1), _ptr(w2),
                                            _ptr(ln_a[0]), _ptr(ln_a[1]), _ptr(ln_g[0]), _ptr(ln_g[1]),
                                            _ptr(ln_f[0]) if ln_f is not None else _vp(0), _ptr(ln_f[1]) if ln_f is not None else _vp(0),
                                            B * T, T, V, S, C, 8, 64, 384, float(eps), int(rows_per_block), _stream())
    _chk(rc, "mq_gcp_attn_fwd")
    res = (out,) + ((y,) if y is not None else ()) + ((gate,) if want_gate else ())
    return res if len(res) > 1 else out


def gcp_gate_residual(sup, h, w2, x, want_gate=False):
    lib = load_library()
    _need_gpu(sup, h, w2, x)
    C, G = sup.shape[-1], h.shape[-1]
    M = sup.numel() // C
    assert sup.is_contiguous() and h.is_contiguous() and x.is_contiguous() and w2.is_contiguous()
    assert sup.dtype == h.dtype == w2.dtype and sup.dtype in _H16 and x.dtype in (sup.dtype, torch.float32)
    out = torch.empty_like(x)
    gate = torch.empty(M, dtype=torch.float32, device=x.device) if want_gate else None
    _chk(_fn(lib, "mq_gcp_gate_residual_fwd", sup)(_ptr(sup), _ptr(h), _ptr(w2), _ptr(x), int(x.dtype == torch.float32), _ptr(out), _ptr(gate),
                                      M, C, G, _stream()), "mq_gcp_gate_residual_fwd")
    return (out, gate) if want_gate else out


def _kv_strides(kf, vo=None):
    st = kf.stride()
    unit = 16 // kf.element_size()
    assert st[3] == 1 and st[2] >= 256 and all(x % unit == 0 for x in st[:3]) and kf.data_ptr() % 16 == 0, st
    if vo is not None:
        assert vo.stride() == st and vo.data_ptr() % 16 == 0, (vo.stride(), st)
    return int(st[0]), int(st[1]), int(st[2])


def vlfuse_i2t(v_ln, kf, vo, bias, out_bias, kv_len=None, max_kv=0, clamp=50000.0, variant=None):
    lib = load_library()
    _need_gpu(v_ln, kf, vo, out_bias)
    B, N, C = v_ln.shape
    Hh, T = kf.shape[1], kf.shape[2]
    assert C == 256 and kf.shape == (B, Hh, T, 256) and vo.shape == kf.shape and T <= 256 and 1 <= Hh <= 8
    assert v_ln.is_contiguous() and out_bias.is_contiguous()
    kv_bs, kv_hs, kv_ts = _kv_strides(kf, vo)
    assert v_ln.dtype == kf.dtype == vo.dtype == out_bias.dtype and v_ln.dtype in _H16
    if bias is not None:
        assert bias.shape == (B, Hh, T) and bias.dtype == torch.float32 and bias.is_contiguous()
    if kv_len is not None:
        assert kv_len.dtype == torch.int32 and kv_len.numel() == B and kv_len.is_contiguous()
    live = max_kv if (kv_len is not None and 0 < max_kv < T) else T
    out = torch.empty_like(v_ln)
    variant = KERNELS["VLFUSE_I2T_VARIANT"] if variant is None else int(variant)
    if f32_operands():
        variant = 0
    with _timed(f"vlfuse_i2t_n{N}_t{T}"):
        _chk(_fn(lib, "mq_vlfuse_i2t_fwd", v_ln)(_ptr(v_ln), _ptr(kf), _ptr(vo), kv_bs, kv_hs, kv_ts, _ptr(bias), _ptr(kv_len), _ptr(out_bias), _ptr(out),
                                   B, N, T, Hh, int(max_kv), float(clamp), int(variant),
                                   _stream()), "mq_vlfuse_i2t_fwd")
    return out


def vlfuse_t2i(kf, v_ln, nsplit, clamp=50000.0, kv_len=None, key_mask=None, max_kv=0, variant=0):
    lib = load_library()
    _need_gpu(kf, v_ln, key_mask)
    B, N, C = v_ln.shape
    Hh, T = kf.shape[1], kf.shape[2]
    assert C == 256 and kf.shape == (B, Hh, T, 256) and v_ln.is_contiguous() and 1 <= Hh <= 8
    kv_bs, kv_hs, kv_ts = _kv_strides(kf)
    km_bs = 0
    if key_mask is not None:
        assert key_mask.dtype == torch.uint8 and key_mask.dim() == 2 and key_mask.shape[0] == B and key_mask.stride(1) == 1
        km_bs = key_mask.stride(0)
        assert km_bs % 4 == 0 and key_mask.shape[1] >= -(-N // 64) * 64
    assert kf.dtype == v_ln.dtype and kf.dtype in _H16
    nsplit = max(1, int(nsplit))
    if kv_len is not None:
        assert kv_len.dtype == torch.int32 and kv_len.numel() == B and kv_len.is_contiguous()
    else:
        max_kv = 0
    ws = torch.empty(lib.mq_vlfuse_t2i_workspace_bytes(B, T, nsplit) // 4, dtype=torch.float32, device=kf.device)
    out = torch.empty(B, T, Hh * 256, dtype=kf.dtype, device=kf.device)
    with _timed(f"vlfuse_t2i_n{N}_t{T}_s{nsplit}"):
        _chk(_fn(lib, "mq_vlfuse_t2i_fwd", kf)(_ptr(kf), kv_bs, kv_hs, kv_ts, _ptr(v_ln), _ptr(kv_len), _ptr(key_mask), km_bs, _ptr(ws), _ptr(out), B, N, T, Hh,
                                   nsplit, int(max_kv), float(clamp), int(variant), _stream()), "mq_vlfuse_t2i_fwd")
    return out


def image_key_mask(mask):
    B, N = mask.shape
    out = torch.ones(B, -(-N // 64) * 64, dtype=torch.uint8, device=mask.device)
    out[:, :N] = mask.to(torch.uint8)
    return out


def layer_norm(x, gamma, beta, eps=1e-5, residual=None, want_sum=True, want_y32=False, want_y=True, clamp=0.0):
    lib = load_library()
    _need_gpu(x, gamma, beta, residual)
    C = x.shape[-1]
    h16 = gamma.dtype
    assert x.is_contiguous() and x.dtype in (h16, torch.float32)
    assert h16 in _H16 and beta.dtype == h16
    rows = x.numel() // C
    xf = x.dtype == torch.float32
    rf = False
    y = torch.empty(x.shape, dtype=h16, device=x.device) if want_y else None
    y32 = torch.empty(x.shape, dtype=torch.float32, device=x.device) if want_y32 else None
    xsum = None
    if residual is not None:
        assert residual.shape == x.shape and residual.is_contiguous() and residual.dtype in (h16, torch.float32)
        rf = residual.dtype == torch.float32
        if want_sum:
            xsum = torch.empty(x.shape, dtype=torch.float32 if (xf or rf) else h16, device=x.device)
    with _timed(f"layernorm_c{C}", sum(t.numel() * t.element_size() for t in (x, residual, y, y32, xsum) if t is not None)):
        name = "mq_layernorm2_fwd" if KERNELS["LN_VARIANT"] == 2 else "mq_layernorm_fwd"
        if clamp > 0:
            _chk(_fn(lib, "mq_layernorm_clamp_fwd", gamma)(_ptr(x), int(xf), _ptr(residual), int(rf), _ptr(gamma), _ptr(beta), _ptr(y), _ptr(y32), _ptr(xsum),
                                                           rows, C, float(eps), float(clamp), _stream()), "mq_layernorm_clamp_fwd")
        else:
            _chk(_fn(lib, name, gamma)(_ptr(x), int(xf), _ptr(residual), int(rf), _ptr(gamma), _ptr(beta), _ptr(y), _ptr(y32), _ptr(xsum),
                                       rows, C, float(eps), _stream()), name)
    out = [t for t in (y, y32, xsum) if t is not None]
    return out[0] if len(out) == 1 else tuple(out)


def clamp_gelu_clamp(x, clamp):
    lib = load_library()
    _need_gpu(x)
    assert x.is_contiguous() and x.dtype in _H16 and x.numel() % 8 == 0 and clamp > 0
    out = torch.empty_like(x)
    with _timed("clamp_gelu_clamp", 2 * x.numel() * 2):
        _chk(_fn(lib, "mq_clamp_gelu_clamp", x)(_ptr(x), _ptr(out), x.numel(), float(clamp), _stream()), "mq_clamp_gelu_clamp")
    return out


def patch_merge_ln(x, gamma, beta, eps=1e-5):
    lib = load_library()
    _need_gpu(x, gamma, beta)
    B, H, W, C = x.shape
    h16 = gamma.dtype
    assert x.is_contiguous() and x.dtype in (h16, torch.float32) and h16 in _H16 and beta.dtype == h16
    assert gamma.numel() == 4 * C and beta.numel() == 4 * C and C % 8 == 0 and 4 * C <= 3072
    y = torch.empty(B, ((H + 1) // 2) * ((W + 1) // 2), 4 * C, dtype=h16, device=x.device)
    with _timed(f"patch_merge_ln_c{C}", x.numel() * x.element_size() + y.numel() * 2):
        _chk(_fn(lib, "mq_patch_merge_ln_fwd", gamma)(_ptr(x), int(x.dtype == torch.float32), _ptr(gamma), _ptr(beta), _ptr(y), B, H, W, C,
                                                     float(eps), _stream()), "mq_patch_merge_ln_fwd")
    return y


SWIN_MLP_WIDTHS = (96, 192, 384)


def swin_mlp_w2_perm(K, device=None):
    k = torch.arange(K, device=device)
    blk, slot = k >> 5, k & 31
    g, t = slot >> 3, slot & 7
    return blk * 32 + torch.where(t < 4, 4 * g + t, 16 + 4 * g + (t - 4))


def split_planar_blocks(t, block=512):
    assert t.dtype == torch.float32 and t.numel() % block == 0
    x = t.reshape(-1, block)
    hi = x.to(torch.float16)
    lo = ((x - hi.float()) * 2048.0).to(torch.float16)
    return torch.cat([hi, lo], 1).contiguous().view(torch.float32).reshape(t.shape)


def unsplit_planar_blocks(t, block=512):
    h = t.reshape(-1, block).contiguous().view(torch.float16).reshape(-1, 2, block).float()
    return (h[:, 0] + h[:, 1] / 2048.0).reshape(t.shape)


def swin_mlp2_pack(w1, w2):
    HID, C = w1.shape
    assert w2.shape == (C, HID) and C % 32 == 0 and HID % 32 == 0
    KS, CT, NCH = C // 32, C // 16, HID // 32
    w1f = w1.reshape(NCH, 2, 16, KS, 4, 8).permute(0, 1, 3, 4, 2, 5).reshape(NCH, -1)
    w1f = torch.cat([w1f, w1f.new_zeros(2, w1f.shape[1])], 0).reshape(-1).contiguous()
    w2p = w2[:, swin_mlp_w2_perm(HID, w2.device)]
    w2f = w2p.reshape(CT, 16, NCH, 4, 8).permute(2, 0, 3, 1, 4).reshape(-1).contiguous()
    if w1f.dtype == torch.float32 and f32_operands():
        w1f, w2f = split_planar_blocks(w1f), split_planar_blocks(w2f)
    return w1f, w2f


def swin_mlp2(x, delta, ln_g, ln_b, eps, w1f, b1, w2f, b2, next_ln=None, flags=None, into=None):
    lib = load_library()
    _need_gpu(x, delta, ln_g, ln_b, w1f, b1, w2f, b2)
    C = x.shape[-1]
    M = x.numel() // C
    assert C in SWIN_MLP_WIDTHS and x.dtype == torch.float32 and x.is_contiguous()
    assert delta is None or (delta.dtype == w1f.dtype and delta.is_contiguous() and delta.shape == x.shape)
    assert w1f.numel() == (4 * C // 32 + 2) * (C // 16) * 512 and w2f.numel() == (4 * C // 32) * (C // 16) * 512
    assert w1f.is_contiguous() and w2f.is_contiguous() and w1f.dtype == w2f.dtype == b1.dtype == b2.dtype == ln_g.dtype and w1f.dtype in _H16
    out = torch.empty_like(x) if into is None else into[0]
    y, ng, nb, ne = None, None, None, 0.0
    if next_ln is not None:
        ng, nb, ne = next_ln
        y = torch.empty(x.shape, dtype=w1f.dtype, device=x.device) if into is None else into[1]
    flags = KERNELS["SWIN_MLP2_FLAGS"] if flags is None else int(flags)
    auto = flags < 0
    if auto:
        flags = 3 if C < 384 else 2
    if f32_operands():
        flags = 0 if auto else flags & ~2
    fn = _fn(lib, "mq_swin_mlp2_fwd", w1f)

    def call(fl):
        _chk(fn(_ptr(x), _ptr(delta), _ptr(ln_g), _ptr(ln_b), float(eps), _ptr(w1f), _ptr(b1), _ptr(w2f), _ptr(b2),
                _ptr(out), _ptr(ng), _ptr(nb), float(ne), _ptr(y), M, C, fl, _stream()), "mq_swin_mlp2_fwd")
    side = _tail_stream(x.device) if (KERNELS["SWIN_MLP_TAIL_STREAM"] == 1 and x.is_cuda and not (flags & 29) and _TIMING is None) else None
    with _timed(f"swin_mlp_c{C}", M * C * (4 + 4 + (2 if delta is not None else 0) + (2 if y is not None else 0))):
        if side is None:
            call(flags)
        else:
            main = torch.cuda.current_stream()
            side.wait_stream(main)
            with torch.cuda.stream(side):
                call(flags | 16)
            call(flags | 8)
            main.wait_stream(side)
    return (out, y) if y is not None else out


_TAIL_STREAMS = {}


def _tail_stream(device):
    s = _TAIL_STREAMS.get(device.index)
    if s is None:
        s = _TAIL_STREAMS[device.index] = torch.cuda.Stream(device=device)
    return s


def conv3x3(x_nhwc, w_packed, bias, n_out, stride=1):
    lib = load_library()
    _need_gpu(x_nhwc, w_packed, bias)
    B, H, W, C = x_nhwc.shape
    assert x_nhwc.dtype in _H16 and x_nhwc.stride(3) == 1 and x_nhwc.stride(2) == C and x_nhwc.stride(1) == W * C
    assert w_packed.is_contiguous() and w_packed.shape == (32 if n_out <= 32 else 256, 9 * C) and w_packed.dtype == x_nhwc.dtype
    Ho, Wo = (H + 2 - 3) // stride + 1, (W + 2 - 3) // stride + 1
    ld = n_out if n_out % 8 == 0 else (n_out + 7) // 8 * 8
    out = torch.empty(B, Ho, Wo, ld, dtype=x_nhwc.dtype, device=x_nhwc.device)
    with _timed("conv3x3"):
        _chk(_fn(lib, "mq_conv3x3_fwd", x_nhwc)(_ptr(x_nhwc), _ptr(w_packed), _ptr(bias), _ptr(out), B, H, W, C, x_nhwc.stride(0), n_out, ld,
                                stride, _stream()), "mq_conv3x3_fwd")
    return out if ld == n_out else out[..., :n_out]


def conv3x3_nchw32(x_nhwc, w_packed, bias, n_out):
    lib = load_library()
    _need_gpu(x_nhwc, w_packed, bias)
    B, H, W, C = x_nhwc.shape
    assert x_nhwc.dtype in _H16 and x_nhwc.stride(3) == 1 and x_nhwc.stride(2) == C and x_nhwc.stride(1) == W * C
    assert w_packed.is_contiguous() and w_packed.shape == (32, 9 * C) and w_packed.dtype == x_nhwc.dtype and n_out <= 32
    out = torch.empty(B, n_out, H, W, dtype=torch.float32, device=x_nhwc.device)
    with _timed("conv3x3_small", B * H * W * C * 2 + out.numel() * 4):
        name = "mq_conv3x3_nchw32_v2_fwd" if KERNELS["OFFSET_CONV_VARIANT"] >= 2 else "mq_conv3x3_nchw32_fwd"
        _chk(_fn(lib, name, x_nhwc)(_ptr(x_nhwc), _ptr(w_packed), _ptr(bias), _ptr(out), B, H, W, C, x_nhwc.stride(0), n_out, _stream()), name)
    return out


class _ConvLevel(ctypes.Structure):
    _fields_ = [("x", _vp), ("out", _vp), ("x_bs", _l), ("H", _i), ("W", _i)]


def conv3x3_nchw32_group_supported(levels, n_out):
    if f32_operands() == 1:
        return False
    return 0 < len(levels) <= 8 and n_out <= 32 and all(x.shape[3] == 256 and x.shape[1] * x.shape[2] * 256 < 2 ** 31 for x in levels)


def conv3x3_nchw32_group(levels, w_packed, bias, n_out):
    lib = load_library()
    _need_gpu(w_packed, bias, *levels)
    assert conv3x3_nchw32_group_supported(levels, n_out)
    B, C = levels[0].shape[0], levels[0].shape[3]
    assert w_packed.is_contiguous() and w_packed.shape == (32, 9 * C) and w_packed.dtype == levels[0].dtype
    arr = (_ConvLevel * len(levels))()
    outs, nbytes = [], 0
    for a, x in zip(arr, levels):
        Bx, H, W, Cx = x.shape
        assert Bx == B and Cx == C and x.dtype == levels[0].dtype and x.stride(3) == 1 and x.stride(2) == C and x.stride(1) == W * C
        out = torch.empty(B, n_out, H, W, dtype=torch.float32, device=x.device)
        a.x, a.out, a.x_bs, a.H, a.W = _ptr(x).value, _ptr(out).value, x.stride(0), H, W
        outs.append(out)
        nbytes += B * H * W * C * 2 + out.numel() * 4
    with _timed("conv3x3_group", nbytes):
        _chk(_fn(lib, "mq_conv3x3_nchw32_group_fwd", levels[0])(ctypes.cast(arr, _vp), len(levels), _ptr(w_packed), _ptr(bias), B, C, n_out, _stream()),
             "mq_conv3x3_nchw32_group_fwd")
    return outs


def dcnv2(x_nhwc, om, w_packed, bias, stride, want_stats=False, wy=None, wx=None, mask_prob=False, tag="dcnv2_fused", plain=False):
    lib = load_library()
    _need_gpu(x_nhwc, om, w_packed, bias, wy, wx)
    B, H, W, C = x_nhwc.shape
    assert x_nhwc.dtype in _H16 and x_nhwc.stride(3) == 1 and x_nhwc.stride(2) == C and x_nhwc.stride(1) == W * C
    assert om.is_contiguous() and om.dtype == torch.float32 and om.shape[1] == 27
    assert w_packed.is_contiguous() and w_packed.shape == (256, 9 * C) and w_packed.dtype == x_nhwc.dtype
    Ho, Wo = (H + 2 - 3) // stride + 1, (W + 2 - 3) // stride + 1
    y = torch.empty(B, Ho * Wo, 256, dtype=x_nhwc.dtype, device=x_nhwc.device)
    sums = None
    if want_stats:
        sums = torch.empty(B, lib.mq_dcnv2_stats_blocks(H, W, stride), 256, 3, dtype=torch.float32, device=y.device)
        if wy is not None:
            assert wy.dtype == wx.dtype == torch.float32 and wy.numel() == Ho and wx.numel() == Wo
    w_packed, wflag = _dcn_w(w_packed)
    with _timed(tag):
        _chk(_fn(lib, "mq_dcnv2_fwd", x_nhwc)(_ptr(x_nhwc), _ptr(om), _ptr(w_packed), _ptr(bias), _ptr(y), _ptr(sums), _ptr(wy), _ptr(wx),
                              B, H, W, C, x_nhwc.stride(0), om.shape[2], om.shape[3], 256, 256, stride, int(bool(mask_prob)) | (2 if plain else 0) | wflag,
                              _stream()), "mq_dcnv2_fwd")
    return (y, (Ho, Wo), sums) if want_stats else (y, (Ho, Wo))


_DCN_TILED = {}


def dcn_weight_tiles(w):
    import weakref
    N, K = w.shape
    C = K // 9
    assert N == 256 and K == 9 * C and C % 128 == 0 and w.is_contiguous()
    if w.dtype == torch.float32:
        blk = w.view(256, 9, C // 32, 32).permute(2, 1, 0, 3).reshape(-1, 256 * 32)
        hi = blk.to(torch.float16)
        lo = ((blk - hi.float()) * 2048.0).to(torch.float16)
        out = torch.cat([hi, lo], 1).contiguous().view(torch.float32).reshape(256, K)
    else:
        blk = w.view(256, 9, C // 64, 8, 8).permute(2, 1, 0, 3, 4).reshape(-1, 256, 8, 8)
        r = torch.arange(256, device=w.device)[:, None]
        pos = torch.arange(8, device=w.device)[None, :]
        src = (pos ^ (r & 7))
        out = torch.gather(blk, 2, src[None, :, :, None].expand(blk.shape[0], -1, -1, 8)).reshape(256, K).contiguous()
    if len(_DCN_TILED) > 4096:
        for k in [k for k, ref in _DCN_TILED.items() if ref() is None]:
            del _DCN_TILED[k]
    _DCN_TILED[id(out)] = weakref.ref(out)
    return out


def dcn_weight_rows(wt):
    N, K = wt.shape
    C = K // 9
    assert N == 256 and K == 9 * C and C % 128 == 0
    if wt.dtype == torch.float32:
        planes = wt.contiguous().view(torch.float16).reshape(-1, 2, 256, 32)
        blk = planes[:, 0].float() + planes[:, 1].float() / 2048.0
        return blk.view(C // 32, 9, 256, 32).permute(2, 1, 0, 3).reshape(256, K).contiguous()
    blk = wt.contiguous().view(-1, 256, 8, 8)
    r = torch.arange(256, device=wt.device)[:, None]
    pos = torch.arange(8, device=wt.device)[None, :]
    chunk = torch.gather(blk, 2, (pos ^ (r & 7))[None, :, :, None].expand(blk.shape[0], -1, -1, 8))
    return chunk.view(C // 64, 9, 256, 8, 8).permute(2, 1, 0, 3, 4).reshape(256, K).contiguous()


def dcn_is_tiled(w):
    ref = _DCN_TILED.get(id(w))
    return ref is not None and ref() is w


def dcn_bdma():
    k = KERNELS.get("DCN_BDMA", 1)
    return k == 1 or (k == -1 and bool(f32_operands()))


def _dcn_w(w):
    ref = _DCN_TILED.get(id(w))
    if ref is not None and ref() is w:
        return w, 4
    if dcn_bdma():
        return dcn_weight_tiles(w), 4
    return w, 0


class _DcnBranch(ctypes.Structure):
    _fields_ = [(n, _vp) for n in ("x", "om", "w", "bias", "out", "stats", "wy", "wx")] + [("x_bs", _l)] + \
               [(n, _i) for n in ("B", "H", "W", "C", "oH", "oW", "N", "out_ld", "stride", "flags")]


def dcnv2_group(branches, want_stats=True, tag="dcnv2_fused", ablation=0):
    lib = load_library()
    arr = (_DcnBranch * len(branches))()
    outs = []
    keep = []
    for i, (a, br) in enumerate(zip(arr, branches)):
        x, om, w, bias, stride = br["x"], br["om"], br["w"], br["bias"], br["stride"]
        wy, wx = br.get("wy"), br.get("wx")
        _need_gpu(x, om, w, bias, wy, wx)
        B, H, W, C = x.shape
        assert x.dtype in _H16 and x.stride(3) == 1 and x.stride(2) == C and x.stride(1) == W * C
        assert om.is_contiguous() and om.dtype == torch.float32 and om.shape[1] == 27
        assert w.is_contiguous() and w.shape == (256, 9 * C) and w.dtype == x.dtype
        Ho, Wo = (H + 2 - 3) // stride + 1, (W + 2 - 3) // stride + 1
        y = torch.empty(B, Ho * Wo, 256, dtype=x.dtype, device=x.device)
        sums = None
        if want_stats:
            sums = torch.empty(B, lib.mq_dcnv2_stats_blocks(H, W, stride), 256, 3, dtype=torch.float32, device=y.device)
            if wy is not None:
                assert wy.dtype == wx.dtype == torch.float32 and wy.numel() == Ho and wx.numel() == Wo
        w, wflag = _dcn_w(w)
        keep.append(w)
        a.x, a.om, a.w, a.bias, a.out = _ptr(x).value, _ptr(om).value, _ptr(w).value, _ptr(bias).value, _ptr(y).value
        a.stats, a.wy, a.wx = _ptr(sums).value, _ptr(wy).value, _ptr(wx).value
        a.x_bs, a.B, a.H, a.W, a.C, a.oH, a.oW = x.stride(0), B, H, W, C, om.shape[2], om.shape[3]
        a.N, a.out_ld, a.stride, a.flags = 256, 256, stride, (int(bool(br.get("mask_prob", False))) | (2 if br.get("plain", False) else 0) | wflag
                                                             | ((int(ablation) & 15) << 8 if i == 0 else 0))
        outs.append((y, (Ho, Wo), sums))
    with _timed(tag):
        _chk(_fn(lib, "mq_dcnv2_group_fwd", *[br["x"] for br in branches])(ctypes.cast(arr, _vp), len(branches), _stream()), "mq_dcnv2_group_fwd")
    return outs


def dyconv_branch_coef(y, Wsrc, gamma, beta, attn_w, attn_b, groups, eps, nbranches, wy=None, wx=None, sums=None):
    lib = load_library()
    _need_gpu(y, gamma, beta, attn_w, attn_b, wy, wx)
    B, n, C = y.shape
    assert y.is_contiguous() and y.dtype in _H16 and gamma.dtype == y.dtype
    assert attn_w.dtype == torch.float32 and attn_b.dtype == torch.float32
    coef = torch.empty(B, C, 2, dtype=torch.float32, device=y.device)
    nblk = 0
    if sums is None:
        sums = torch.empty(B, (n + 255) // 256, C, 3, dtype=torch.float32, device=y.device)
        with _timed("dyconv_stats"):
            _chk(_fn(lib, "mq_dyconv_stats", y)(_ptr(y), _ptr(sums), _ptr(wy), _ptr(wx), B, n, Wsrc, C, _stream()), "mq_dyconv_stats")
    else:
        assert sums.dtype == torch.float32 and sums.is_contiguous() and sums.shape[0] == B and sums.shape[2:] == (C, 3)
        nblk = sums.shape[1]
    _chk(_fn(lib, "mq_dyconv_coef", gamma)(_ptr(sums), _ptr(gamma), _ptr(beta), _ptr(attn_w), _ptr(attn_b), _ptr(coef), B, n, nblk, C, groups,
                            float(eps), nbranches, _stream()), "mq_dyconv_coef")
    return coef


class _CoefBranch(ctypes.Structure):
    _fields_ = [(n, _vp) for n in ("sums", "gamma", "beta", "coef")] + [(n, _i) for n in ("nblk", "n", "nbranches", "reserved")]


def dyconv_coef_group(items, attn_w, attn_b, groups, eps):
    lib = load_library()
    arr = (_CoefBranch * len(items))()
    outs = []
    B = C = None
    for a, it in zip(arr, items):
        sums = it["sums"]
        _need_gpu(sums, it["gamma"], it["beta"], attn_w, attn_b)
        assert sums.dtype == torch.float32 and sums.is_contiguous() and sums.shape[2:] == (256, 3)
        B, C = sums.shape[0], sums.shape[2]
        coef = torch.empty(B, C, 2, dtype=torch.float32, device=sums.device)
        a.sums, a.gamma, a.beta, a.coef = _ptr(sums).value, _ptr(it["gamma"]).value, _ptr(it["beta"]).value, _ptr(coef).value
        a.nblk, a.n, a.nbranches, a.reserved = sums.shape[1], int(it["n"]), int(it["nbranches"]), 0
        outs.append(coef)
    _chk(_fn(lib, "mq_dyconv_coef_group", *[it["gamma"] for it in items])(ctypes.cast(arr, _vp), len(items), _ptr(attn_w), _ptr(attn_b), B, C, groups, float(eps), _stream()),
         "mq_dyconv_coef_group")
    return outs


def dyconv_fuse(branches, H, W, out=None):
    lib = load_library()
    y0 = branches[0][0]
    B, _, C = y0.shape
    if out is None:
        out = torch.empty(B, H * W, C, dtype=y0.dtype, device=y0.device)
    assert out.shape == (B, H * W, C) and out.dtype == y0.dtype and y0.dtype in _H16 and out.stride(2) == 1 and out.stride(1) == C
    pool = torch.empty(B, (H * W + 127) // 128, C, dtype=torch.float32, device=y0.device)
    args = []
    for k in range(3):
        if k < len(branches):
            y, cf, hs, ws = branches[k]
            _need_gpu(y, cf)
            assert y.is_contiguous() and cf.is_contiguous() and y.shape[1] == hs * ws
            args += [_ptr(y), _ptr(cf), hs, ws]
        else:
            args += [_ptr(None), _ptr(None), 0, 0]
    with _timed("dyconv_fuse", sum(b_[0].numel() * 2 for b_ in branches) + out.shape[0] * out.shape[1] * C * 2):
        _chk(_fn(lib, "mq_dyconv_fuse", *[b_[0] for b_ in branches])(*args, len(branches), _ptr(out), out.stride(0), _ptr(pool), B, H, W, C, _stream()), "mq_dyconv_fuse")
    return out, pool


class _FuseLevel(ctypes.Structure):
    _fields_ = [("y", _vp * 3), ("coef", _vp * 3), ("hs", _i * 3), ("ws", _i * 3), ("nbranches", _i), ("H", _i), ("W", _i), ("reserved", _i),
                ("out", _vp), ("out_bs", _l), ("pool", _vp), ("relu_coef", _vp)]


def dyconv_epilogue_group(levels, w0, b0, w2, b2, relu_coef):
    lib = load_library()
    _need_gpu(w0, b0, w2, b2, relu_coef)
    y0 = levels[0][0][0][0]
    B, _, C = y0.shape
    assert 0 < len(levels) <= 8 and C == 256 and relu_coef.shape == (len(levels), B, 4, C) and relu_coef.is_contiguous() and relu_coef.dtype == torch.float32
    assert w0.is_contiguous() and w2.is_contiguous() and w0.dtype == y0.dtype and y0.dtype in _H16
    arr = (_FuseLevel * len(levels))()
    keep, nbytes = [], 0
    for l, (a, (branches, H, W, out)) in enumerate(zip(arr, levels)):
        assert out.shape == (B, H * W, C) and out.dtype == y0.dtype and out.stride(2) == 1 and out.stride(1) == C and 1 <= len(branches) <= 3
        pool = torch.empty(B, (H * W + 127) // 128, C, dtype=torch.float32, device=y0.device)
        keep.append(pool)
        for k, (y, cf, hs, ws) in enumerate(branches):
            _need_gpu(y, cf)
            assert y.is_contiguous() and cf.is_contiguous() and y.shape == (B, hs * ws, C) and y.dtype == y0.dtype and cf.dtype == torch.float32
            a.y[k], a.coef[k], a.hs[k], a.ws[k] = _ptr(y).value, _ptr(cf).value, hs, ws
            nbytes += y.numel() * 2
        a.nbranches, a.H, a.W, a.reserved = len(branches), H, W, 0
        a.out, a.out_bs, a.pool, a.relu_coef = _ptr(out).value, out.stride(0), _ptr(pool).value, _ptr(relu_coef[l]).value
        nbytes += B * H * W * C * 2
    with _timed("dyconv_epilogue_group", nbytes):
        _chk(_fn(lib, "mq_dyconv_epilogue_group", y0)(ctypes.cast(arr, _vp), len(levels), _ptr(w0), _ptr(b0), _ptr(w2), _ptr(b2), B, C, _stream()),
             "mq_dyconv_epilogue_group")
    return relu_coef


def dyrelu_(x, pool, w0, b0, w2, b2):
    lib = load_library()
    _need_gpu(x, pool, w0, b0, w2, b2)
    B, n, C = x.shape
    assert x.stride(2) == 1 and x.stride(1) == C and w0.is_contiguous() and w2.is_contiguous() and w0.dtype == x.dtype and x.dtype in _H16
    coef = torch.empty(B, 4, C, dtype=torch.float32, device=x.device)
    _chk(_fn(lib, "mq_dyrelu_coef", w0)(_ptr(pool), _ptr(w0), _ptr(b0), _ptr(w2), _ptr(b2), _ptr(coef), B, n, C, _stream()),
         "mq_dyrelu_coef")
    with _timed("dyrelu_apply", 2 * B * n * C * 2):
        _chk(_fn(lib, "mq_dyrelu_apply", x)(_ptr(x), _ptr(coef), B, n, C, x.stride(0), _stream()), "mq_dyrelu_apply")
    return x


def dyrelu_coef(pool, n, w0, b0, w2, b2, out=None):
    lib = load_library()
    _need_gpu(pool, w0, b0, w2, b2)
    B, C = pool.shape[0], pool.shape[-1]
    assert pool.is_contiguous() and pool.dtype == torch.float32 and pool.numel() == B * ((int(n) + 127) // 128) * C
    coef = torch.empty(B, 4, C, dtype=torch.float32, device=pool.device) if out is None else out
    assert coef.shape == (B, 4, C) and coef.is_contiguous() and coef.dtype == torch.float32 and w0.is_contiguous() and w2.is_contiguous()
    _chk(_fn(lib, "mq_dyrelu_coef", w0)(_ptr(pool), _ptr(w0), _ptr(b0), _ptr(w2), _ptr(b2), _ptr(coef), B, int(n), C, _stream()), "mq_dyrelu_coef")
    return coef


def add_upsample_nearest_(dst, src):
    lib = load_library()
    _need_gpu(dst, src)
    B, H, W, C = dst.shape
    assert src.shape[0] == B and src.shape[3] == C and dst.is_contiguous() and src.is_contiguous() and dst.dtype == src.dtype and dst.dtype in _H16
    with _timed("fpn_topdown", 2 * dst.numel() * 2 + src.numel() * 2):
        _chk(_fn(lib, "mq_add_upsample_nearest", dst)(_ptr(dst), _ptr(src), B, H, W, src.shape[1], src.shape[2], C, _stream()),
             "mq_add_upsample_nearest")
    return dst


def pool2x2_tokens_supported(feats):
    if not (0 < len(feats) <= 8):
        return False
    B, C = feats[0].shape[0], feats[0].shape[1]
    for f in feats:
        if f.dim() != 4 or f.shape[0] != B or f.shape[1] != C or f.dtype != feats[0].dtype or f.shape[2] < 2 or f.shape[3] < 2:
            return False
        if f.stride(1) != 1 or f.stride(3) != C or f.stride(2) != f.shape[3] * C or f.data_ptr() % 16 or f.stride(0) % 8:
            return False
    return C % 8 == 0 and feats[0].dtype in (torch.float16, torch.bfloat16, torch.float32)


def pool2x2_tokens(feats):
    lib = load_library()
    _need_gpu(*feats)
    assert 0 < len(feats) <= 8
    B, C = feats[0].shape[0], feats[0].shape[1]
    arr = (_ConvLevel * len(feats))()
    n = 0
    for a, f in zip(arr, feats):
        x = f.permute(0, 2, 3, 1)
        Bx, H, W, Cx = x.shape
        assert Bx == B and Cx == C and x.dtype == feats[0].dtype and x.stride(3) == 1 and x.stride(2) == C and x.stride(1) == W * C and H >= 2 and W >= 2
        a.x, a.out, a.x_bs, a.H, a.W = _ptr(x).value, None, x.stride(0), H, W
        n += (H // 2) * (W // 2)
    out = torch.empty(B, n, C, dtype=feats[0].dtype, device=feats[0].device)
    with _timed("pool2x2_tokens", sum(f.numel() for f in feats) * 2 + out.numel() * 2):
        _chk(_fn(lib, "mq_pool2x2_tokens_fwd", feats[0])(ctypes.cast(arr, _vp), len(feats), _ptr(out), B, C, _stream()), "mq_pool2x2_tokens_fwd")
    return out


def dyrelu_apply_(x, coef):
    lib = load_library()
    _need_gpu(x, coef)
    B, n, C = x.shape
    assert x.stride(2) == 1 and x.stride(1) == C and x.dtype in _H16 and coef.shape == (B, 4, C) and coef.is_contiguous()
    _chk(_fn(lib, "mq_dyrelu_apply", x)(_ptr(x), _ptr(coef), B, n, C, x.stride(0), _stream()), "mq_dyrelu_apply")
    return x


def dyrelu_layer_norm(x, coef, sizes, gamma, beta, eps):
    lib = load_library()
    _need_gpu(x, coef, gamma, beta)
    B, N, C = x.shape
    NL = len(sizes)
    offs = [0]
    for (h, w) in sizes:
        offs.append(offs[-1] + int(h) * int(w))
    assert C == 256 and offs[-1] == N and x.stride(2) == 1 and x.stride(1) == C and x.dtype in _H16 and gamma.dtype == x.dtype
    assert coef.shape == (NL, B, 4, C) and coef.is_contiguous() and coef.dtype == torch.float32
    y = torch.empty(B, N, C, dtype=x.dtype, device=x.device)
    rf = (ctypes.c_int * (NL + 1))(*offs)
    with _timed("layernorm_c256_dyrelu", 2 * x.numel() * 2):
        _chk(_fn(lib, "mq_dyrelu_ln_fwd", x)(_ptr(x), x.stride(0), _ptr(coef), ctypes.cast(rf, _vp), NL, _ptr(gamma), _ptr(beta), float(eps),
                                             _ptr(y), B, N, C, _stream()), "mq_dyrelu_ln_fwd")
    return y


SCORE_AGG = {"MEAN": 0, "MAX": 1, "POWER": 2, "ONEHOT": 0}


def align_scores(dot, tbias, tokidx, ctr, thr, want_cls=False, agg=0):
    lib = load_library()
    _need_gpu(dot, tbias, tokidx, ctr)
    B, HW, T = dot.shape
    L, MT = tokidx.shape[-2:]
    assert dot.stride(2) == 1 and dot.stride(1) == T and dot.dtype in (ctr.dtype, torch.float32)
    assert ctr.dtype in _H16 and ctr.is_contiguous()
    assert tbias.dtype == torch.float32 and tbias.is_contiguous() and tokidx.dtype == torch.int32 and tokidx.is_contiguous()
    assert tokidx.dim() == 2 or tokidx.shape[0] == B
    out = torch.empty(B, HW, L, dtype=torch.float32, device=dot.device)
    cls = torch.empty_like(out) if want_cls else None
    with _timed("align_scores", B * HW * T * dot.element_size() + out.numel() * 4):
        _chk(_fn(lib, "mq_align_scores_fwd", ctr)(_ptr(dot), int(dot.dtype == torch.float32), _ptr(tbias), _ptr(tokidx),
                                     L * MT if tokidx.dim() == 3 else 0, _ptr(ctr), _ptr(out), _ptr(cls), B, HW, T, L, MT,
                                     float(thr), dot.stride(0), int(agg), _stream()), "mq_align_scores_fwd")
    return (out, cls) if want_cls else out


def align_fused(tok, tk, tbias, wbc, bbc, scales, tokidx, sizes, thr, agg=0, kv_max=0, want_cls=False, want_logits=False):
    lib = load_library()
    _need_gpu(tok, tk, tbias, wbc, bbc, scales, tokidx)
    B, N, C = tok.shape
    T = tk.shape[1]
    L, MT = tokidx.shape[-2:]
    NL = len(sizes)
    offs = [0]
    for (h, w) in sizes:
        offs.append(offs[-1] + int(h) * int(w))
    assert C == 256 and offs[-1] == N and tk.shape == (B, T, 256) and tok.is_contiguous() and tk.is_contiguous()
    assert tok.dtype == tk.dtype == wbc.dtype and tok.dtype in _H16 and wbc.shape == (16, 256) and wbc.is_contiguous()
    assert tbias.dtype == torch.float32 and tbias.shape == (B, T) and tbias.is_contiguous()
    assert bbc.dtype == scales.dtype == torch.float32 and bbc.numel() >= 8 and scales.numel() >= NL
    assert tokidx.dtype == torch.int32 and tokidx.is_contiguous() and (tokidx.dim() == 2 or tokidx.shape[0] == B)
    live = kv_max if 0 < kv_max < T else T
    if f32_operands() == 1 and -(-live // 16) * 16 > 144:
        raise RuntimeError(f"mq_align_fused_fwd_f32: the text tile of {live} live tokens does not fit the LDS at fp32 (up to 144; the GEMM path takes longer captions)")
    dev = tok.device
    ranked = torch.empty(B * N * L, dtype=torch.float32, device=dev)
    cls = torch.empty(B * N * L, dtype=torch.float32, device=dev) if want_cls else None
    reg = torch.empty(B * N * 4, dtype=torch.float32, device=dev)
    ctr = torch.empty(B, N, dtype=torch.float32, device=dev)
    logits = torch.zeros(B, N, T, dtype=torch.float32, device=dev) if want_logits else None
    lvl = (ctypes.c_int * (NL + 1))(*offs)
    with _timed("align_fused", tok.numel() * 2 + ranked.numel() * 4 + reg.numel() * 4):
        _chk(_fn(lib, "mq_align_fused_fwd", tok)(_ptr(tok), _ptr(tk), _ptr(tbias), _ptr(wbc), _ptr(bbc), _ptr(scales), _ptr(tokidx),
                                                 L * MT if tokidx.dim() == 3 else 0, ctypes.cast(lvl, _vp), _ptr(ranked), _ptr(cls), _ptr(reg),
                                                 _ptr(ctr), _ptr(logits), B, N, T, int(kv_max), L, MT, NL, float(thr), int(agg), _stream()),
             "mq_align_fused_fwd")

    def levels(flat, width):
        return [flat[offs[l] * B * width:offs[l + 1] * B * width].view(B, offs[l + 1] - offs[l], width) for l in range(NL)]
    out = {"ranked": levels(ranked, L), "reg": levels(reg, 4), "ctr": ctr}
    if want_cls:
        out["cls"] = levels(cls, L)
    if want_logits:
        out["logits"] = logits
    return out


def post_select_supported(hws, ks, B, L):
    NL = len(hws)
    if NL < 1 or NL > 8:
        return False
    hw = (ctypes.c_int * NL)(*[int(h) for h in hws])
    kk = (ctypes.c_int * NL)(*[int(k) for k in ks])
    return load_library().mq_post_select_workspace_bytes(ctypes.cast(hw, _vp), ctypes.cast(kk, _vp), NL, int(B), int(L)) >= 0


def post_select(ranked, reg, anchors, ks, label_ids, im_wh):
    lib = load_library()
    NL = len(ranked)
    B, _, L = ranked[0].shape
    dev = ranked[0].device
    _need_gpu(*ranked, *reg, *anchors, label_ids, im_wh)
    for r, g, a in zip(ranked, reg, anchors):
        assert r.dtype == g.dtype == a.dtype == torch.float32 and r.is_contiguous() and g.is_contiguous() and a.is_contiguous()
        assert r.shape[0] == B and r.shape[2] == L and g.shape == (B, r.shape[1], 4) and a.shape == (r.shape[1], 4)
    assert label_ids.dtype == torch.int32 and label_ids.is_contiguous() and im_wh.dtype == torch.float32 and im_wh.is_contiguous()
    tot = int(sum(ks))
    boxes = torch.empty(B, tot, 4, dtype=torch.float32, device=dev)
    scores = torch.empty(B, tot, dtype=torch.float32, device=dev)
    labels = torch.empty(B, tot, dtype=torch.int32, device=dev)
    ids = torch.empty(B, tot, dtype=torch.int32, device=dev)
    pp = lambda ts: (ctypes.c_void_p * NL)(*[_ptr(t).value for t in ts])
    hw = (ctypes.c_int * NL)(*[int(r.shape[1]) for r in ranked])
    kk = (ctypes.c_int * NL)(*[int(k) for k in ks])
    wsb = lib.mq_post_select_workspace_bytes(ctypes.cast(hw, _vp), ctypes.cast(kk, _vp), NL, B, L)
    if wsb < 0:
        raise RuntimeError("mq_post_select_fwd: level sizes out of range (ops.post_select_supported)")
    ws = torch.empty(max(wsb, 8), dtype=torch.uint8, device=dev)
    with _timed("post_select", sum(r.numel() for r in ranked) * 4):
        _chk(lib.mq_post_select_fwd(ctypes.cast(pp(ranked), _vp), ctypes.cast(pp(reg), _vp), ctypes.cast(pp(anchors), _vp), ctypes.cast(hw, _vp),
                                    ctypes.cast(kk, _vp), NL, B, L, _ptr(label_ids), L if label_ids.dim() == 2 else 0, _ptr(im_wh), _ptr(ws), _ptr(boxes),
                                    _ptr(scores), _ptr(labels), _ptr(ids), _stream()), "mq_post_select_fwd")
    return boxes, scores, labels, ids


def post_sort(boxes, scores, labels, ks):
    lib = load_library()
    _need_gpu(boxes, scores, labels)
    B, tot = scores.shape
    NL = len(ks)
    offs = [0]
    for k in ks:
        offs.append(offs[-1] + int(k))
    assert offs[-1] == tot
    off = (ctypes.c_int * (NL + 1))(*offs)
    bo, so, lo = torch.empty_like(boxes), torch.empty_like(scores), torch.empty_like(labels)
    nvalid = torch.empty(B, dtype=torch.int32, device=scores.device)
    with _timed("post_sort"):
        _chk(lib.mq_post_sort_fwd(_ptr(boxes), _ptr(scores), _ptr(labels), ctypes.cast(off, _vp), NL, _ptr(bo), _ptr(so), _ptr(lo), _ptr(nvalid), B, tot,
                                  _stream()), "mq_post_sort_fwd")
    return bo, so, lo, nvalid


def post_finalize(boxes, scores, labels, keep, K, K2):
    lib = load_library()
    _need_gpu(boxes, scores, labels, keep)
    B, tot = scores.shape
    assert keep.dtype == torch.uint8 and keep.is_contiguous() and keep.shape == (B, tot)
    out = torch.empty(B, K2, 6, dtype=torch.float32, device=scores.device)
    counts = torch.empty(B, dtype=torch.int32, device=scores.device)
    with _timed("post_finalize"):
        _chk(lib.mq_post_finalize_fwd(_ptr(boxes), _ptr(scores), _ptr(labels), _ptr(keep), _ptr(out), _ptr(counts), B, tot, int(K), int(K2), _stream()),
             "mq_post_finalize_fwd")
    return out, counts


def box_decode(val, flat, reg, anchors, label_ids, im_wh, boxes, scores, labels, HW, L, out_off):
    lib = load_library()
    _need_gpu(val, flat, reg, anchors, label_ids, im_wh, boxes, scores, labels)
    B, K = val.shape
    assert val.dtype == torch.float32 and flat.dtype == torch.int64 and reg.dtype in _H16 + (torch.float32,)
    assert val.is_contiguous() and flat.is_contiguous() and reg.is_contiguous() and anchors.is_contiguous()
    assert boxes.dtype == torch.float32 and scores.dtype == torch.float32 and labels.dtype == torch.int32
    assert label_ids.is_contiguous() and label_ids.dtype == torch.int32 and (label_ids.dim() == 1 or label_ids.shape[0] == B)
    _chk(_fn(lib, "mq_box_decode", reg)(_ptr(val), _ptr(flat), _ptr(reg), int(reg.dtype == torch.float32), _ptr(anchors), _ptr(label_ids), L if label_ids.dim() == 2 else 0,
                           _ptr(im_wh), _ptr(boxes), _ptr(scores), _ptr(labels), B, K, HW, L, boxes.shape[1], out_off, _stream()),
         "mq_box_decode")


def roi_align(feat, rois, output_size, spatial_scale, sampling_ratio, aligned=True, reduce_mean=False):
    lib = load_library()
    _need_gpu(feat, rois)
    N, C, H, W = feat.shape
    PH, PW = (output_size, output_size) if isinstance(output_size, int) else output_size
    assert feat.dtype in _H16 + (torch.float32,) and rois.dtype == torch.float32 and rois.shape[1] == 5
    rois = rois.contiguous()
    R = rois.shape[0]
    out = torch.empty((R, C) if reduce_mean else (R, C, PH, PW), dtype=torch.float32, device=feat.device)
    _chk(_fn(lib, "mq_roi_align_fwd", feat)(_ptr(feat), int(feat.dtype == torch.float32), _ptr(rois), _ptr(out), R, C, H, W, feat.stride(0),
                              feat.stride(1), feat.stride(2), feat.stride(3), PH, PW, float(spatial_scale), int(sampling_ratio),
                              int(bool(aligned)), int(bool(reduce_mean)), _stream()), "mq_roi_align_fwd")
    return out


_MSDA_SHAPES = {}


def ms_deform_attn(value, spatial_shapes, sampling_locations, attention_weights, out_dtype=None):
    lib = load_library()
    _need_gpu(value, sampling_locations, attention_weights)
    B, S, M, D = value.shape
    _, Q, _, L, P, _ = sampling_locations.shape
    shapes = tuple((int(h), int(w)) for h, w in spatial_shapes)
    assert len(shapes) == L and sum(h * w for h, w in shapes) == S
    assert value.is_contiguous() and value.dtype in _H16 + (torch.float32,)
    assert sampling_locations.dtype == attention_weights.dtype == torch.float32
    assert sampling_locations.is_contiguous() and attention_weights.is_contiguous() and attention_weights.shape == (B, Q, M, L, P)
    hw, start = _msda_shapes(shapes, value.device)
    out_dtype = out_dtype or value.dtype
    out = torch.empty(B, Q, M * D, dtype=out_dtype, device=value.device)
    nb = value.numel() * value.element_size() + sampling_locations.numel() * 4 + attention_weights.numel() * 4 + out.numel() * out.element_size()
    with _timed(f"msdeform_attn_q{Q}", nb):
        _chk(_fn(lib, "mq_msdeform_attn_fwd", value, out)(_ptr(value), int(value.dtype == torch.float32), _ptr(hw), _ptr(start), _ptr(sampling_locations),
                                      _ptr(attention_weights), _ptr(out), int(out_dtype == torch.float32), B, S, M, D, L, Q, P, _stream()),
             "mq_msdeform_attn_fwd")
    return out


def _msda_shapes(shapes, device):
    key = (shapes, device)
    if key not in _MSDA_SHAPES:
        hw = torch.tensor(shapes, dtype=torch.int64)
        start = torch.cat([hw.new_zeros(1), (hw[:, 0] * hw[:, 1]).cumsum(0)[:-1]])
        _MSDA_SHAPES[key] = (hw.to(device), start.to(device))
    return _MSDA_SHAPES[key]


def ms_deform_attn_q(value, spatial_shapes, qproj, ref, heads, out_dtype=None, valid_hw=None):
    lib = load_library()
    _need_gpu(value, qproj, ref)
    B, S, C = value.shape
    D = C // heads
    Q = qproj.shape[1]
    shapes = tuple((int(h), int(w)) for h, w in spatial_shapes)
    L, P = len(shapes), 4
    assert sum(h * w for h, w in shapes) == S and value.stride(2) == 1 and value.dtype in _H16 + (torch.float32,)
    assert qproj.dtype in _H16 and qproj.is_contiguous() and qproj.shape == (B, Q, heads * L * P * 3)
    assert ref.dtype == torch.float32 and ref.is_contiguous() and ref.shape[:3] == (B, Q, L) and ref.shape[3] in (2, 4)
    if valid_hw is not None:
        _need_gpu(valid_hw)
        assert valid_hw.dtype == torch.int32 and valid_hw.is_contiguous() and valid_hw.shape == (B, L, 2)
    hw, start = _msda_shapes(shapes, value.device)
    out_dtype = out_dtype or value.dtype
    out = torch.empty(B, Q, C, dtype=out_dtype, device=value.device)
    nb = B * S * C * value.element_size() + qproj.numel() * 2 + ref.numel() * 4 + out.numel() * out.element_size()
    with _timed(f"msdeform_attn_q{Q}", nb):
        _chk(_fn(lib, "mq_msdeform_attn_q_fwd", value, qproj, out)(_ptr(value), int(value.dtype == torch.float32), value.stride(0), value.stride(1), _ptr(hw),
                                        _ptr(start), _ptr(qproj), _ptr(ref), ref.shape[3], _ptr(valid_hw), _ptr(out),
                                        int(out_dtype == torch.float32), B, S, heads, D, L, Q, P, _stream()),
             "mq_msdeform_attn_q_fwd")
    return out


def ml_nms(boxes, labels, nvalid, thresh, max_keep=0, as_bool=True):
    lib = load_library()
    _need_gpu(boxes, labels, nvalid)
    B, N, _ = boxes.shape
    assert boxes.is_contiguous() and labels.is_contiguous() and boxes.dtype == torch.float32
    assert labels.dtype == torch.int32 and nvalid.dtype == torch.int32
    ws = torch.empty(max(lib.mq_ml_nms_workspace_bytes(B, N), 8), dtype=torch.uint8, device=boxes.device)
    keep = torch.empty(B, N, dtype=torch.uint8, device=boxes.device)
    if max_keep > 0 and N <= 6656 and KERNELS["NMS_EARLY_STOP"] == 1:
        _chk(lib.mq_ml_nms_topk(_ptr(boxes), _ptr(labels), _ptr(nvalid), _ptr(ws), _ptr(keep), B, N, float(thresh), int(max_keep), _stream()),
             "mq_ml_nms_topk")
        return keep.bool() if as_bool else keep
    _chk(lib.mq_ml_nms(_ptr(boxes), _ptr(labels), _ptr(nvalid), _ptr(ws), _ptr(keep), B, N, float(thresh), _stream()),
         "mq_ml_nms")
    return keep.bool() if as_bool else keep


TTA_MERGE_MAX_ROWS = 256 * 64
def tta_ingest(src, src_off, meta, bounds, coef, B, Hp, Wp, TH, R, mean, std, bgr, x255, flip, err):
    lib = load_library()
    _need_gpu(src, src_off, meta, bounds, coef, err)
    assert src.dtype == torch.uint8 and src_off.dtype == torch.int64 and meta.dtype == bounds.dtype == coef.dtype == torch.int32
    out = torch.empty(B, 3, Hp, Wp, dtype=torch.float32, device=src.device)
    out_f = torch.empty_like(out) if flip else None
    m, s = (ctypes.c_float * 3)(*[float(v) for v in mean]), (ctypes.c_float * 3)(*[float(v) for v in std])
    with _timed("tta_ingest", src.numel() + out.numel() * 4 * (2 if flip else 1)):
        _chk(lib.mq_tta_ingest_fwd(_ptr(src), _ptr(src_off), _ptr(meta), _ptr(bounds), _ptr(coef), _ptr(out), _ptr(out_f), _ptr(err), B, Hp, Wp, TH, R,
                                   ctypes.cast(m, ctypes.c_void_p), ctypes.cast(s, ctypes.c_void_p), int(bgr), int(x255), _stream()),
             "mq_tta_ingest_fwd")
    return out, out_f


def tta_merge(packed, counts, tparam, band, cls_rank, thresh, top_n):
    lib = load_library()
    _need_gpu(packed, counts, tparam, band, cls_rank)
    T, B, K, _ = packed.shape
    N, dev = T * K, packed.device
    assert packed.dtype == torch.float32 and packed.is_contiguous() and counts.dtype == torch.int32 and cls_rank.dtype == torch.int32
    f = lambda *s: torch.empty(*s, dtype=torch.float32, device=dev)
    i = lambda *s: torch.empty(*s, dtype=torch.int32, device=dev)
    boxes, scores, labels, valid = f(B, N, 4), f(B, N), i(B, N), torch.empty(B, N, dtype=torch.uint8, device=dev)
    boxes_s, scores_s, labels_s, src_s = f(B, N, 4), f(B, N), i(B, N), i(B, N)
    nz = torch.zeros(3, B, dtype=torch.int32, device=dev)
    nvalid, ndrop, n_out = nz[0], nz[1], nz[2]
    _chk(lib.mq_tta_merge_prep(_ptr(packed), _ptr(counts), _ptr(tparam), _ptr(band), _ptr(cls_rank), cls_rank.numel(), _ptr(boxes), _ptr(scores),
                               _ptr(labels), _ptr(valid), _ptr(boxes_s), _ptr(scores_s), _ptr(labels_s), _ptr(src_s), _ptr(nvalid),
                               _ptr(ndrop), T, B, K, _stream()), "mq_tta_merge_prep")
    if thresh > 0:
        if N > TTA_MERGE_MAX_ROWS:
            raise ValueError(f"TTA merge: {N} rows per image (transforms x detection slots) exceed the {TTA_MERGE_MAX_ROWS} of mq_ml_nms")
        keep = ml_nms(boxes_s, labels_s, nvalid, thresh, as_bool=False)
    else:
        keep = torch.ones(B, N, dtype=torch.uint8, device=dev)
    boxes_o, scores_o, labels_o, thr = f(B, N, 4), f(B, N), torch.empty(B, N, dtype=torch.int64, device=dev), f(B)
    _chk(lib.mq_tta_merge_finalize(_ptr(boxes_s), _ptr(scores_s), _ptr(labels_s), _ptr(src_s), _ptr(keep), _ptr(nvalid), _ptr(thr),
                                   _ptr(cls_rank), _ptr(boxes_o), _ptr(scores_o), _ptr(labels_o), _ptr(n_out), B, N, int(top_n), _stream()),
         "mq_tta_merge_finalize")
    return boxes_o, scores_o, labels_o, n_out, ndrop


LVIS_MATCH_LANES = 40


def lvis_match(pair_dt, pair_gt, pair_nel, dt_box, gt_box, gt_area, gt_ign, gt_nz, area_rng, iou_thr):
    lib = load_library()
    _need_gpu(pair_dt, pair_gt, pair_nel, dt_box, gt_box, gt_area, gt_ign, gt_nz, area_rng, iou_thr)
    assert pair_dt.dtype == pair_gt.dtype == torch.int32 and pair_nel.dtype == gt_ign.dtype == gt_nz.dtype == torch.uint8
    assert dt_box.dtype == torch.float32 and gt_box.dtype == gt_area.dtype == area_rng.dtype == iou_thr.dtype == torch.float64
    assert area_rng.numel() == 8 and iou_thr.numel() == 10
    for t in (pair_dt, pair_gt, pair_nel, dt_box, gt_box, gt_area, gt_ign, gt_nz):
        assert t.is_contiguous()
    P, Nd, Ng, dev = len(pair_dt), len(dt_box), len(gt_box), dt_box.device
    dt_bits = torch.zeros(Nd, 2, dtype=torch.int64, device=dev)
    gt_count = torch.zeros(P, 4, dtype=torch.int32, device=dev)
    ws = torch.empty(LVIS_MATCH_LANES * max(Ng, 1), dtype=torch.uint8, device=dev)
    with _timed("lvis_match"):
        _chk(lib.mq_lvis_match(_ptr(pair_dt), _ptr(pair_gt), _ptr(pair_nel), _ptr(dt_box), _ptr(gt_box), _ptr(gt_area), _ptr(gt_ign), _ptr(gt_nz),
                               _ptr(area_rng), _ptr(iou_thr), _ptr(dt_bits), _ptr(gt_count), _ptr(ws), P, Ng, _stream()), "mq_lvis_match")
    return dt_bits, gt_count


def lvis_accumulate(cat_off, order, dt_bits, num_gt, rec_thr, n_thr=10):
    lib = load_library()
    _need_gpu(cat_off, order, dt_bits, num_gt, rec_thr)
    assert cat_off.dtype == order.dtype == num_gt.dtype == torch.int32 and dt_bits.dtype == torch.int64 and rec_thr.dtype == torch.float64
    assert rec_thr.numel() == 101 and n_thr == 10 and num_gt.is_contiguous() and dt_bits.is_contiguous()
    K, dev = len(cat_off) - 1, dt_bits.device
    precision = torch.empty(n_thr, 101, K, 4, dtype=torch.float64, device=dev)
    recall = torch.empty(n_thr, K, 4, dtype=torch.float64, device=dev)
    with _timed("lvis_accumulate"):
        _chk(lib.mq_lvis_accumulate(_ptr(cat_off), _ptr(order), _ptr(dt_bits), _ptr(num_gt), _ptr(rec_thr), _ptr(precision), _ptr(recall), K,
                                    _stream()), "mq_lvis_accumulate")
    return precision, recall


def bank_admit(cand, sorted_labels, order, pool, inv_norm, slots, counts, state, label_lo, num_labels, maxq, exclude, thr):
    lib = load_library()
    _need_gpu(cand, sorted_labels, order, pool, inv_norm, slots, counts, state)
    assert cand.dtype == pool.dtype == inv_norm.dtype == torch.float32 and sorted_labels.dtype == order.dtype == torch.int64
    assert slots.dtype == counts.dtype == state.dtype == torch.int32 and state.numel() == 2
    for t in (cand, sorted_labels, order, pool, inv_norm, slots, counts, state):
        assert t.is_contiguous()
    N, D = cand.shape
    R, cap = pool.shape[0], slots.shape[1]
    assert len(sorted_labels) == len(order) == N and pool.numel() == R * D and len(inv_norm) == R and len(counts) == slots.shape[0]
    assert 0 <= label_lo and label_lo + num_labels <= len(counts) and 0 < maxq <= cap
    with _timed("bank_admit"):
        _chk(lib.mq_bank_admit(_ptr(cand), _ptr(sorted_labels), _ptr(order), _ptr(pool), _ptr(inv_norm), _ptr(slots), _ptr(counts), _ptr(state),
                               N, D, R, cap, int(label_lo), int(num_labels), int(maxq), int(bool(exclude)), float(thr), _stream()), "mq_bank_admit")
```

mq_det_amd/selection.py:

```python
import os

KERNEL_DEFAULTS = {
    "LN_VARIANT": 2,
    "OFFSET_CONV_VARIANT": 3,
    "PATCH_MERGE_FUSED": 1,
    "FPN_VIA_DCN": 1,
    "NMS_EARLY_STOP": 1,
    "ATTN_RESIDENT": 1,
    "SWIN_MLP_VARIANT": 2,
    "SWIN_MLP2_FLAGS": -1,
    "SWIN_QKV_FUSED": 2,
    "FPN_TOPDOWN_FUSED": 1,
    "DYRELU_IN_LN": 1,
    "VLFUSE_I2T_VARIANT": 0,
    "SWIN_MLP_TAIL_STREAM": 0,
    "DYCONV_EPILOGUE_GROUPED": 1,
    "BERT_CLAMP_FUSED": 1,
    "PATCH_EMBED_FUSED": 1,
    "BERT_QKV_FUSED": 1,
    "FRONT_SIDE_STREAM": 1,
    "LANG_SIDE_STREAMS": 0,
    "GCP_ATTN_FUSED": 1,
    "BERT_ATTN_QKV_FUSED": 1,
    "POST_FUSED": 1,
    "F32_OPERANDS": 0,
    "DCN_BDMA": 1,
    "POOLED_TOKENS_FUSED": 1,
    "ALIGN_FUSED": 1,
}
class _ThreadLocalTable(dict):

    def __init__(self, init):
        super().__init__()
        import threading
        object.__setattr__(self, "_tl", threading.local())
        object.__setattr__(self, "_base", dict(init))

    def _cur(self):
        t = self._tl
        if not hasattr(t, "d"):
            t.d = dict(self._base)
        return t.d

    def __getitem__(self, k): return self._cur()[k]
    def __setitem__(self, k, v): self._cur()[k] = v
    def __delitem__(self, k): del self._cur()[k]
    def __contains__(self, k): return k in self._cur()
    def __iter__(self): return iter(self._cur())
    def __len__(self): return len(self._cur())
    def __eq__(self, other): return self._cur() == (other._cur() if isinstance(other, _ThreadLocalTable) else other)
    def __ne__(self, other): return not self.__eq__(other)
    def __repr__(self): return repr(self._cur())
    def get(self, k, default=None): return self._cur().get(k, default)
    def keys(self): return self._cur().keys()
    def values(self): return self._cur().values()
    def items(self): return self._cur().items()
    def clear(self): self._cur().clear()
    def update(self, *a, **k): self._cur().update(*a, **k)
    def copy(self): return dict(self._cur())

    def set_base(self, d):
        object.__setattr__(self, "_base", dict(d))


KERNELS = _ThreadLocalTable(KERNEL_DEFAULTS)


def configure(cfg=None):
    sel = dict(KERNEL_DEFAULTS)
    node = None
    if cfg is not None:
        node = cfg.MODEL.get("KERNELS", None) if hasattr(cfg.MODEL, "get") else getattr(cfg.MODEL, "KERNELS", None)
    if cfg is not None:
        name = str(cfg.MODEL.get("COMPUTE_DTYPE", "float16") if hasattr(cfg.MODEL, "get") else getattr(cfg.MODEL, "COMPUTE_DTYPE", "float16")).lower()
        sel["F32_OPERANDS"] = 1 if name in ("float32", "fp32", "float") else 0
    for k in sel:
        if node is not None and k in node:
            sel[k] = int(node[k])
        v = os.environ.get("MQ_" + k)
        if v is not None:
            try:
                sel[k] = int(v)
            except ValueError:
                raise ValueError(f"environment variable MQ_{k} = {v!r}: the kernel selection takes integers") from None
    KERNELS.clear()
    KERNELS.update(sel)
    if cfg is None:
        KERNELS.set_base(sel)
    return KERNELS


def activate(sel):
    if sel is not None and KERNELS != sel:
        KERNELS.clear()
        KERNELS.update(sel)


configure()
```

Before: 500.4 images/sec.

## Add fused text-path GEMM kernel with GELU and residual-LayerNorm epilogues

```diff
diff --git a/include/mqdet_hip.h b/include/mqdet_hip.h
--- a/include/mqdet_hip.h
+++ b/include/mqdet_hip.h
@@ -182,6 +182,9 @@
                          int B, int T, int C, int H, long x_bs, long x_rs, long o_bs, long o_rs, long bias_bs, float scale, float clamp,
                          void* stream);
 
+int mq_text_gemm_fwd(const void* a, long lda, const void* w, const void* bias, int epilogue, const void* res, int res_f32, const void* gamma,
+                     const void* beta, void* y, void* out, long M, int K, int N, float eps, float clamp, int rows_per_block, void* stream);
+
 #ifdef __cplusplus
 #define MQ_BF16_TWIN(name) extern decltype(name) name##_bf16;
 #else
@@ -198,6 +201,7 @@
 MQ_BF16_TWIN(mq_gcp_sparse_attn_fwd)
 MQ_BF16_TWIN(mq_gcp_gate_residual_fwd)
 MQ_BF16_TWIN(mq_gcp_attn_fwd)
+MQ_BF16_TWIN(mq_text_gemm_fwd)
 MQ_BF16_TWIN(mq_vlfuse_i2t_fwd)
 MQ_BF16_TWIN(mq_vlfuse_t2i_fwd)
 MQ_BF16_TWIN(mq_layernorm_fwd)
@@ -245,6 +249,7 @@
 MQ_F32_TWIN(mq_gcp_sparse_attn_fwd)
 MQ_F32_TWIN(mq_gcp_gate_residual_fwd)
 MQ_F32_TWIN(mq_gcp_attn_fwd)
+MQ_F32_TWIN(mq_text_gemm_fwd)
 MQ_F32_TWIN(mq_vlfuse_i2t_fwd)
 MQ_F32_TWIN(mq_vlfuse_t2i_fwd)
 MQ_F32_TWIN(mq_layernorm_fwd)
diff --git a/mq_det_amd/build.py b/mq_det_amd/build.py
--- a/mq_det_amd/build.py
+++ b/mq_det_amd/build.py
@@ -6,7 +6,7 @@
 CSRC = os.path.join(HERE, "csrc")
 LIB_DIR = os.path.join(HERE, "lib")
 LIB = os.path.join(LIB_DIR, "libmqdet_hip.so")
-SOURCES = ["api.hip", "attn.hip", "attn_resident.hip", "attn_text.hip", "bert_attn.hip", "vlfuse_attn.hip", "window_attn.hip", "patch_embed.hip", "gcp.hip", "gcp_fused.hip", "conv_igemm.hip", "conv_small.hip", "conv_small2.hip", "conv_small3.hip", "dcn_fused.hip", "layernorm.hip", "layernorm2.hip", "dyconv.hip", "post.hip", "post2.hip", "align_fused.hip", "nms2.hip", "roi_align.hip", "swin_mlp2.hip", "msda.hip", "tta.hip", "lvis_eval.hip", "query_bank.hip"]
+SOURCES = ["api.hip", "attn.hip", "attn_resident.hip", "attn_text.hip", "bert_attn.hip", "vlfuse_attn.hip", "window_attn.hip", "patch_embed.hip", "gcp.hip", "gcp_fused.hip", "text_gemm.hip", "conv_igemm.hip", "conv_small.hip", "conv_small2.hip", "conv_small3.hip", "dcn_fused.hip", "layernorm.hip", "layernorm2.hip", "dyconv.hip", "post.hip", "post2.hip", "align_fused.hip", "nms2.hip", "roi_align.hip", "swin_mlp2.hip", "msda.hip", "tta.hip", "lvis_eval.hip", "query_bank.hip"]
 F32_SKIP = ("roi_align.hip", "nms2.hip", "post2.hip", "tta.hip", "lvis_eval.hip", "query_bank.hip")
 FLAGS = ["--offload-arch=gfx950", "-O3", "-std=c++17", "-fPIC"]
 EXTRA_FLAGS = {"dcn_fused.hip": ["-fno-slp-vectorize"],
diff --git a/mq_det_amd/csrc/text_gemm.hip b/mq_det_amd/csrc/text_gemm.hip
--- /dev/null
+++ b/mq_det_amd/csrc/text_gemm.hip
@@ -0,0 +1,320 @@
+#include "common.h"
+
+MQ_NAMESPACE_BEGIN
+
+namespace {
+constexpr int TG_D = 4;
+constexpr int TG_N = 768, TG_SP = TG_N + 4;
+constexpr int TG_TP = 64 + 8;
+constexpr size_t TG_LDS_MAX = 160 * 1024;
+}
+
+struct TextGemmParams {
+  const half_t* a;
+  long lda;
+  const half_t* w;
+  const half_t* bias;
+  const void* res;
+  const half_t *gamma, *beta;
+  half_t* y;
+  void* out;
+  long M;
+  int K, N;
+  float eps, clamp;
+};
+
+template <int ROWS, int NT, int U>
+__device__ __forceinline__ void tg_stage_rows(const TextGemmParams& p, half_t* At, long row0, int tid) {
+  const int kc8 = p.K / 8, P = p.K + 8, total = ROWS * kc8;
+  for (int base = 0; base < total; base += U * NT) {
+    half8 v[U];
+    int dst[U];
+#pragma unroll
+    for (int u = 0; u < U; ++u) {
+      const int c = base + u * NT + tid, cc = min(c, total - 1);
+      const int r = cc / kc8, kc = cc - r * kc8;
+      const long row = min(row0 + r, p.M - 1);
+      v[u] = *(const half8*)(p.a + row * p.lda + kc * 8);
+      dst[u] = c < total ? r * P + kc * 8 : -1;
+    }
+#pragma unroll
+    for (int u = 0; u < U; ++u)
+      if (dst[u] >= 0) *(half8*)(At + dst[u]) = v[u];
+  }
+}
+
+template <int MB, int NTL>
+__device__ __forceinline__ void tg_kloop(const half_t* At, int P, int KS, const half_t* const (&wrow)[NTL], half8 (&w)[TG_D][NTL], float4_ (&acc)[MB][NTL]) {
+  for (int ks = 0; ks < KS; ks += TG_D) {
+#pragma unroll
+    for (int d = 0; d < TG_D; ++d) {
+      half8 af[MB];
+#pragma unroll
+      for (int mb = 0; mb < MB; ++mb) af[mb] = *(const half8*)(At + mb * 16 * P + (ks + d) * 32);
+#pragma unroll
+      for (int mb = 0; mb < MB; ++mb)
+#pragma unroll
+        for (int j = 0; j < NTL; ++j) acc[mb][j] = mfma16(af[mb], w[d][j], acc[mb][j]);
+      const int kn = min(ks + d + TG_D, KS - 1);
+#pragma unroll
+      for (int j = 0; j < NTL; ++j) w[d][j] = *(const half8*)(wrow[j] + (long)kn * 512);
+      __builtin_amdgcn_sched_barrier(0);
+    }
+  }
+}
+
+template <int EPI, bool RF32>
+__global__ __launch_bounds__(512) void text_gemm_rows_kernel(TextGemmParams p) {
+  constexpr int NTL = 6;
+  extern __shared__ __attribute__((aligned(16))) char smem[];
+  const int P = p.K + 8, KS = p.K / 32;
+  half_t* At = (half_t*)smem;
+  float* S = (float*)(At + 16 * P);
+  const int tid = threadIdx.x, lane = tid & 63, l15 = lane & 15, lg = lane >> 4;
+  const int wave = __builtin_amdgcn_readfirstlane(tid >> 6);
+  const long row0 = (long)blockIdx.x * 16;
+
+  const half_t* wrow[NTL];
+  half8 w[TG_D][NTL];
+#pragma unroll
+  for (int j = 0; j < NTL; ++j) wrow[j] = p.w + (long)(wave * NTL + j) * KS * 512 + lane * 8;
+#pragma unroll
+  for (int d = 0; d < TG_D; ++d)
+#pragma unroll
+    for (int j = 0; j < NTL; ++j) w[d][j] = *(const half8*)(wrow[j] + (long)d * 512);
+  float4_ rr[2][3];
+#pragma unroll
+  for (int r = 0; r < 2; ++r) {
+    const long row = min(row0 + wave * 2 + r, p.M - 1);
+#pragma unroll
+    for (int i = 0; i < 3; ++i) {
+      const long off = row * TG_N + 256 * i + 4 * lane;
+      if constexpr (RF32) {
+        rr[r][i] = *(const float4_*)((const float*)p.res + off);
+      } else {
+        const half4 h = *(const half4*)((const half_t*)p.res + off);
+#pragma unroll
+        for (int e = 0; e < 4; ++e) rr[r][i][e] = (float)h[e];
+      }
+    }
+  }
+  const half_t* bp = p.bias ? p.bias : p.gamma ? p.gamma : (const half_t*)p.w;
+  half_t bv[NTL];
+#pragma unroll
+  for (int j = 0; j < NTL; ++j) bv[j] = bp[wave * 96 + j * 16 + l15];
+  tg_stage_rows<16, 512, 4>(p, At, row0, tid);
+  float4_ acc[1][NTL];
+#pragma unroll
+  for (int j = 0; j < NTL; ++j) {
+    const float b = p.bias ? (float)bv[j] : 0.f;
+#pragma unroll
+    for (int r = 0; r < 4; ++r) acc[0][j][r] = b;
+  }
+  __syncthreads();
+  tg_kloop<1, NTL>(At + l15 * P + 8 * lg, P, KS, wrow, w, acc);
+
+  const float cl = (float)(half_t)p.clamp;
+#pragma unroll
+  for (int j = 0; j < NTL; ++j)
+#pragma unroll
+    for (int r = 0; r < 4; ++r) {
+      float v = acc[0][j][r];
+      if (EPI == 1 && p.clamp > 0.f) v = __builtin_amdgcn_fmed3f(v, -cl, cl);
+      S[(4 * lg + r) * TG_SP + wave * 96 + j * 16 + l15] = v;
+    }
+  __syncthreads();
+
+  half4 g4[3], b4[3];
+  if constexpr (EPI == 1) {
+#pragma unroll
+    for (int i = 0; i < 3; ++i) {
+      g4[i] = *(const half4*)(p.gamma + 256 * i + 4 * lane);
+      b4[i] = *(const half4*)(p.beta + 256 * i + 4 * lane);
+    }
+  }
+#pragma unroll
+  for (int r = 0; r < 2; ++r) {
+    const int lrow = wave * 2 + r;
+    const long row = row0 + lrow;
+    const bool ok = row < p.M;
+    float4_ v[3];
+#pragma unroll
+    for (int i = 0; i < 3; ++i) {
+      v[i] = *(const float4_*)(S + lrow * TG_SP + 256 * i + 4 * lane);
+#pragma unroll
+      for (int e = 0; e < 4; ++e) {
+        v[i][e] += rr[r][i][e];
+        if constexpr (!RF32) v[i][e] = (float)(half_t)v[i][e];
+      }
+    }
+    if constexpr (EPI == 1) {
+      float s = 0.f;
+#pragma unroll
+      for (int i = 0; i < 3; ++i)
+#pragma unroll
+        for (int e = 0; e < 4; ++e) s += v[i][e];
+      const float mean = wave_sum(s) / (float)TG_N;
+      float q = 0.f;
+#pragma unroll
+      for (int i = 0; i < 3; ++i)
+#pragma unroll
+        for (int e = 0; e < 4; ++e) { const float d = v[i][e] - mean; q += d * d; }
+      const float rstd = rsqrtf(wave_sum(q) / (float)TG_N + p.eps);
+#pragma unroll
+      for (int i = 0; i < 3; ++i)
+#pragma unroll
+        for (int e = 0; e < 4; ++e) {
+          float o = (v[i][e] - mean) * rstd * (float)g4[i][e] + (float)b4[i][e];
+          if (p.clamp > 0.f) o = __builtin_amdgcn_fmed3f(o, -cl, cl);
+          v[i][e] = o;
+        }
+    }
+    if (ok) {
+#pragma unroll
+      for (int i = 0; i < 3; ++i) {
+        const long off = row * TG_N + 256 * i + 4 * lane;
+        half4 h;
+#pragma unroll
+        for (int e = 0; e < 4; ++e) h[e] = (half_t)v[i][e];
+        if (p.y) *(half4*)(p.y + off) = h;
+        if (p.out) {
+          if constexpr (RF32) *(float4_*)((float*)p.out + off) = v[i];
+          else *(half4*)((half_t*)p.out + off) = h;
+        }
+      }
+    }
+  }
+}
+
+template <int MB>
+__global__ __launch_bounds__(256) void text_gemm_gelu_kernel(TextGemmParams p) {
+  constexpr int NTL = 4;
+  extern __shared__ __attribute__((aligned(16))) char smem[];
+  const int P = p.K + 8, KS = p.K / 32;
+  half_t* At = (half_t*)smem;
+  const int tid = threadIdx.x, lane = tid & 63, l15 = lane & 15, lg = lane >> 4;
+  const int wave = __builtin_amdgcn_readfirstlane(tid >> 6);
+  half_t* Tw = At + 16 * MB * P + wave * 16 * TG_TP;
+  const long row0 = (long)blockIdx.y * (16 * MB);
+  const int col0 = blockIdx.x * 256 + wave * 64;
+
+  const half_t* wrow[NTL];
+  half8 w[TG_D][NTL];
+#pragma unroll
+  for (int j = 0; j < NTL; ++j) wrow[j] = p.w + (long)(col0 / 16 + j) * KS * 512 + lane * 8;
+#pragma unroll
+  for (int d = 0; d < TG_D; ++d)
+#pragma unroll
+    for (int j = 0; j < NTL; ++j) w[d][j] = *(const half8*)(wrow[j] + (long)d * 512);
+  const half_t* bp = p.bias ? p.bias : (const half_t*)p.w;
+  half_t bv[NTL];
+#pragma unroll
+  for (int j = 0; j < NTL; ++j) bv[j] = bp[col0 + j * 16 + l15];
+  tg_stage_rows<16 * MB, 256, (MB == 4 ? 8 : 6)>(p, At, row0, tid);
+  float4_ acc[MB][NTL];
+#pragma unroll
+  for (int j = 0; j < NTL; ++j) {
+    const float b = p.bias ? (float)bv[j] : 0.f;
+#pragma unroll
+    for (int mb = 0; mb < MB; ++mb)
+#pragma unroll
+      for (int r = 0; r < 4; ++r) acc[mb][j][r] = b;
+  }
+  __syncthreads();
+  tg_kloop<MB, NTL>(At + l15 * P + 8 * lg, P, KS, wrow, w, acc);
+
+  const float cl = (float)(half_t)p.clamp;
+#pragma unroll
+  for (int mb = 0; mb < MB; ++mb) {
+#pragma unroll
+    for (int j = 0; j < NTL; ++j)
+#pragma unroll
+      for (int r = 0; r < 4; ++r) {
+        float a = acc[mb][j][r];
+        if (p.clamp > 0.f) a = __builtin_amdgcn_fmed3f(a, -cl, cl);
+        const float gl = a * 0.5f * (1.f + erff(a * 0.70710678118654752440f));
+        half_t h = (half_t)gl;
+        if (p.clamp > 0.f) h = (half_t)__builtin_amdgcn_fmed3f((float)h, -cl, cl);
+        Tw[(4 * lg + r) * TG_TP + j * 16 + l15] = h;
+      }
+    wave_lds_fence();
+#pragma unroll
+    for (int h2 = 0; h2 < 2; ++h2) {
+      const int lrow = h2 * 8 + (lane >> 3);
+      const long row = row0 + mb * 16 + lrow;
+      const half8 o = *(const half8*)(Tw + lrow * TG_TP + (lane & 7) * 8);
+      if (row < p.M) *(half8*)(p.y + row * p.N + col0 + (lane & 7) * 8) = o;
+    }
+    wave_lds_fence();
+  }
+}
+
+template <int EPI, bool RF32>
+static int tg_launch_rows(const TextGemmParams& p, hipStream_t stream) {
+  const size_t smem = (size_t)16 * (p.K + 8) * sizeof(half_t) + (size_t)16 * TG_SP * sizeof(float);
+  if (smem > TG_LDS_MAX) return -5;
+  static MqMaxPerDevice attr;
+  if (attr.need(smem)) {
+    hipError_t e = hipFuncSetAttribute((const void*)text_gemm_rows_kernel<EPI, RF32>, hipFuncAttributeMaxDynamicSharedMemorySize, (int)smem);
+    if (e != hipSuccess) return (int)e;
+    attr.done(smem);
+  }
+  hipLaunchKernelGGL((text_gemm_rows_kernel<EPI, RF32>), dim3((unsigned)((p.M + 15) / 16)), dim3(512), smem, stream, p);
+  MQ_CHECK_LAUNCH();
+  return 0;
+}
+
+template <int MB>
+static int tg_launch_gelu(const TextGemmParams& p, hipStream_t stream) {
+  const size_t smem = ((size_t)16 * MB * (p.K + 8) + (size_t)4 * 16 * TG_TP) * sizeof(half_t);
+  if (smem > TG_LDS_MAX) return -5;
+  static MqMaxPerDevice attr;
+  if (attr.need(smem)) {
+    hipError_t e = hipFuncSetAttribute((const void*)text_gemm_gelu_kernel<MB>, hipFuncAttributeMaxDynamicSharedMemorySize, (int)smem);
+    if (e != hipSuccess) return (int)e;
+    attr.done(smem);
+  }
+  const long rb = (p.M + 16 * MB - 1) / (16 * MB);
+  if (rb > 65535) return -6;
+  hipLaunchKernelGGL((text_gemm_gelu_kernel<MB>), dim3((unsigned)(p.N / 256), (unsigned)rb), dim3(256), smem, stream, p);
+  MQ_CHECK_LAUNCH();
+  return 0;
+}
+
+extern "C" int MQ_SYM(mq_text_gemm_fwd)(const void* a, long lda, const void* w, const void* bias, int epilogue, const void* res, int res_f32,
+                                        const void* gamma, const void* beta, void* y, void* out, long M, int K, int N, float eps, float clamp,
+                                        int rows_per_block, void* stream) {
+  if (M <= 0) return 0;
+  if (K <= 0 || K % (32 * TG_D)) return -1;
+  if (lda < K || lda % 8) return -2;
+  if (!a || !w) return -4;
+  TextGemmParams p;
+  p.a = (const half_t*)a; p.lda = lda; p.w = (const half_t*)w; p.bias = (const half_t*)bias; p.res = res;
+  p.gamma = (const half_t*)gamma; p.beta = (const half_t*)beta; p.y = (half_t*)y; p.out = out;
+  p.M = M; p.K = K; p.N = N; p.eps = eps; p.clamp = clamp;
+  hipStream_t s = (hipStream_t)stream;
+  if (epilogue == 0) {
+    if (N <= 0 || N % 256) return -3;
+    if (!y) return -4;
+    int rpb = rows_per_block;
+    if (rpb == 0) {
+      rpb = M <= 16 ? 16 : (M <= 256 ? 32 : 64);
+      while (rpb > 16 && ((size_t)rpb * (K + 8) + (size_t)4 * 16 * TG_TP) * sizeof(half_t) > TG_LDS_MAX) rpb /= 2;
+    }
+    if (rpb == 16) return tg_launch_gelu<1>(p, s);
+    if (rpb == 32) return tg_launch_gelu<2>(p, s);
+    if (rpb == 64) return tg_launch_gelu<4>(p, s);
+    return -3;
+  }
+  if (epilogue != 1 && epilogue != 2) return -3;
+  if (N != TG_N) return -3;
+  if (!res) return -4;
+  if (epilogue == 1) {
+    if (!gamma || !beta || !y) return -4;
+    return res_f32 ? tg_launch_rows<1, true>(p, s) : tg_launch_rows<1, false>(p, s);
+  }
+  if (!out) return -4;
+  return res_f32 ? tg_launch_rows<2, true>(p, s) : tg_launch_rows<2, false>(p, s);
+}
+
+MQ_NAMESPACE_END
diff --git a/mq_det_amd/modeling/pipeline.py b/mq_det_amd/modeling/pipeline.py
--- a/mq_det_amd/modeling/pipeline.py
+++ b/mq_det_amd/modeling/pipeline.py
@@ -56,6 +56,8 @@
             b = f"{p}.encoder.qv_layer.{i}"
             P[b + ".ff.linear2.gated"] = (f32(b + ".ff.linear2.weight") * torch.tanh(f32(b + ".ff_gate"))).to(dtype)
             P[b + ".attn_gate.w2"] = h(b + ".attn_gate.linear2.weight").reshape(-1)
+            _pack_text_gemm(P, b + ".ff.linear1", h(b + ".ff.linear1.weight"))
+            _pack_text_gemm(P, b + ".ff.linear2", P[b + ".ff.linear2.gated"])
             for n in (".attn.to_q", ".attn.to_out", ".attn_gate.linear1"):
                 _pack_frag(P, b + n + ".frag", h(b + n + ".weight"))
         for i in range(2):
@@ -68,6 +70,25 @@
 def _pack_frag(P, key, w):
     if w.shape[0] % 16 == 0 and w.shape[1] % 32 == 0:
         P[key] = ops.pack_b_fragments(w)
+
+
+def _pack_text_gemm(P, name, w=None):
+    w = P[name + ".weight"] if w is None else w
+    if w.dtype != torch.float32 and w.shape[0] % 256 == 0 and w.shape[1] % 128 == 0:
+        P[name + ".frag"] = ops.pack_b_fragments(w.contiguous())
+
+
+_EPI_BIAS_GELU, _EPI_RESIDUAL_LN, _EPI_RESIDUAL = 0, 1, 2
+
+
+def _text_gemm(P, name, x, epilogue, **kw):
+    w = P.get(name + ".frag")
+    if w is None or not x.is_cuda or x.dtype != w.dtype or not x.is_contiguous():
+        return None
+    K = x.shape[-1]
+    if not ops.text_gemm_fits(x.numel() // K, K, w.shape[0] * 16, epilogue):
+        return None
+    return ops.text_gemm(x, w, P.get(name + ".bias"), epilogue, **kw)
 
 
 def _pack_bert_layer(P, sd, b, device, dtype):
@@ -78,6 +99,8 @@
     P[b + ".qkv.weight"] = torch.cat([P[b + ".qk.weight"], h(b + ".attention.self.value.weight")], 0)
     P[b + ".qkv.bias"] = torch.cat([P[b + ".qk.bias"], h(b + ".attention.self.value.bias")], 0)
     _pack_frag(P, b + ".qkv.frag", P[b + ".qkv.weight"])
+    for n in (".attention.output.dense", ".intermediate.dense", ".output.dense"):
+        _pack_text_gemm(P, b + n, h(b + n + ".weight"))
 
 
 def _dcn_tiles(P, key):
@@ -130,6 +153,7 @@
         P[b + ".olc.weight"] = torch.einsum("ohe,hec->ohc", wol, wvv).reshape(wol.shape[0], -1).to(dtype).contiguous()
         P[b + ".olc.bias"] = (torch.einsum("ohe,he->o", wol, f32(b + ".attn.values_v_proj.bias").reshape(8, hd))
                               + f32(b + ".attn.out_l_proj.bias") * gl).to(dtype)
+        _pack_text_gemm(P, b + ".olc")
         wl = f32(b + ".attn.l_proj.weight").reshape(8, hd, -1)
         bl = f32(b + ".attn.l_proj.bias").reshape(8, hd)
         wvl = f32(b + ".attn.values_l_proj.weight").reshape(8, hd, -1)
@@ -376,9 +400,29 @@
                            .expand(Bn, -1, -1), x.transpose(1, 2))
         ctx = ops.attention(qk[:, :, :C], qk[:, :, C:], vt, 12, C // 12, key_bias=key_bias, clamp=50000.0 if clamp else 0.0,
                             kv_len=kv_len, qk_mask=qk_mask)
-    a = _add_ln(P, b + ".attention.output.LayerNorm", _lin(P, b + ".attention.output.dense", ctx), x32 if r32 else x, 1e-12,
-                want_sum=False, want_y32=r32)
+    fused = ops.KERNELS["TEXT_GEMM_FUSED"] >= 1 and (not clamp or ops.KERNELS["BERT_CLAMP_FUSED"] == 1)
+    cl = 50000.0 if clamp else 0.0
+
+    def ln(n):
+        return (P[n + ".weight"], P[n + ".bias"])
+    a = _text_gemm(P, b + ".attention.output.dense", ctx, _EPI_RESIDUAL_LN, residual=(x32 if r32 else x).contiguous(),
+                   ln=ln(b + ".attention.output.LayerNorm"), eps=1e-12, want_out=r32) if fused else None
+    if a is None:
+        a = _add_ln(P, b + ".attention.output.LayerNorm", _lin(P, b + ".attention.output.dense", ctx), x32 if r32 else x, 1e-12,
+                    want_sum=False, want_y32=r32)
     a16, a32 = a if r32 else (a, None)
+    if fused:
+        g = _text_gemm(P, b + ".intermediate.dense", a16, _EPI_BIAS_GELU, clamp=cl)
+        if g is not None:
+            y = _text_gemm(P, b + ".output.dense", g, _EPI_RESIDUAL_LN, residual=(a32 if r32 else a16).contiguous(),
+                           ln=ln(b + ".output.LayerNorm"), eps=1e-12, clamp=cl, want_out=r32)
+            if y is not None:
+                return y
+            o = _lin(P, b + ".output.dense", g)
+            if clamp:
+                return ops.layer_norm(o.contiguous(), P[b + ".output.LayerNorm.weight"], P[b + ".output.LayerNorm.bias"], 1e-12,
+                                      residual=(a32 if r32 else a16).contiguous(), want_sum=False, want_y32=r32, clamp=50000.0)
+            return _add_ln(P, b + ".output.LayerNorm", o, a32 if r32 else a16, 1e-12, want_sum=False, want_y32=r32)
     hmid = _lin(P, b + ".intermediate.dense", a16)
     if clamp and ops.KERNELS["BERT_CLAMP_FUSED"] == 1 and hmid.numel() % 8 == 0:
         o = _lin(P, b + ".output.dense", ops.clamp_gelu_clamp(hmid.contiguous(), 50000.0))
@@ -440,7 +484,22 @@
     return F.linear(_ln(P, b + ".attn.norm_kv", vision), P[b + ".attn.to_kv.weight"])
 
 
-def gcp_block(P, b, x, vision, idx, gates=None, kv=None):
+def _gcp_ff(P, ff, x, xn, want16):
+    out = None
+    if ops.KERNELS["TEXT_GEMM_FUSED"] >= 1 and xn.dtype != torch.float32:
+        g = _text_gemm(P, ff + ".linear1", xn, _EPI_BIAS_GELU)
+        if g is not None:
+            out = _text_gemm(P, ff + ".linear2", g, _EPI_RESIDUAL, residual=x.contiguous(), want_y=want16 and x.dtype == torch.float32)
+            if out is None:
+                out = x + F.linear(g, P[ff + ".linear2.gated"])
+    if out is None:
+        out = x + F.linear(F.gelu(F.linear(xn, P[ff + ".linear1.weight"])), P[ff + ".linear2.gated"])
+    if not want16:
+        return out
+    return out if isinstance(out, tuple) else (out, None)
+
+
+def gcp_block(P, b, x, vision, idx, gates=None, kv=None, want16=False):
     if kv is None:
         kv = gcp_kv(P, b, vision)
     ff = b + ".ff"
@@ -453,7 +512,7 @@
         x, xn = r[0], r[1]
         if gates is not None:
             gates.append(r[2])
-        return x + F.linear(F.gelu(F.linear(xn, P[ff + ".linear1.weight"])), P[ff + ".linear2.gated"])
+        return _gcp_ff(P, ff, x, xn, want16)
     q = F.linear(_ln(P, b + ".attn.norm", x), P[b + ".attn.to_q.weight"])
     sup = F.linear(ops.gcp_sparse_attention(q, kv, idx), P[b + ".attn.to_out.weight"])
     gh = F.linear(_ln(P, b + ".attn_gate.norm", sup), P[b + ".attn_gate.linear1.weight"])
@@ -462,7 +521,7 @@
         gates.append(g)
     else:
         x = ops.gcp_gate_residual(sup, gh, P[b + ".attn_gate.w2"], x.contiguous())
-    return x + F.linear(F.gelu(F.linear(_ln(P, ff + ".norm", x), P[ff + ".linear1.weight"])), P[ff + ".linear2.gated"])
+    return _gcp_ff(P, ff, x, _ln(P, ff + ".norm", x), want16)
 
 
 def language_front(P, cfg, input_ids, attention_mask, use_vq, p="language_backbone.body.model", position_ids=None, qk_mask=None, max_kv=0):
@@ -525,8 +584,8 @@
             if x32 is None:
                 x = gcp_block(P, f"{p}.encoder.qv_layer.{i - qv0}", x, vision, idx, gates, kv=kv_ahead.get(i))
             else:
-                x32 = gcp_block(P, f"{p}.encoder.qv_layer.{i - qv0}", x32, vision, idx, gates, kv=kv_ahead.get(i))
-                x = x32.to(x.dtype)
+                x32, x16 = gcp_block(P, f"{p}.encoder.qv_layer.{i - qv0}", x32, vision, idx, gates, kv=kv_ahead.get(i), want16=True)
+                x = x16 if x16 is not None else x32.to(x.dtype)
         x, x32 = _bert(P, f"{p}.encoder.layer.{i}", x, x32, key_bias, False, kv_len, max_kv=max_kv)
         hidden.append(x if x32 is None else x32)
     n = LB.N_LAYERS
@@ -571,12 +630,20 @@
     return ops.vlfuse_i2t(v_ln, prep["kf"], prep["vo"], prep["bias"], P[b + ".ov.bias"], kv_len=kv_len, max_kv=max_kv)
 
 
-def vl_text_side(P, b, v_ln, prep, kv_len=None, max_kv=0):
+def vl_text_side(P, b, v_ln, prep, kv_len=None, max_kv=0, want16=False):
     Bn, N, _ = v_ln.shape
     T = prep["l_ln"].shape[1]
     t_live = min(T, max_kv) if (kv_len is not None and max_kv > 0) else T
     out_l = ops.vlfuse_t2i(prep["kf"], v_ln, _nsplit_t2i(Bn, prep["kf"].shape[1], t_live, -(-N // 64)), kv_len=kv_len, max_kv=t_live)
-    return prep["l_res"] + _lin(P, b + ".olc", out_l)
+    l_res = prep["l_res"]
+    r = None
+    if ops.KERNELS["TEXT_GEMM_FUSED"] >= 1:
+        r = _text_gemm(P, b + ".olc", out_l, _EPI_RESIDUAL, residual=l_res.contiguous(), want_y=want16 and l_res.dtype == torch.float32)
+    if r is None:
+        r = l_res + _lin(P, b + ".olc", out_l)
+    if not want16:
+        return r
+    return r if isinstance(r, tuple) else (r, None)
 
 
 def vl_fuse_tokens(P, b, v, hidden, key_bias, kv_len=None, max_kv=0):
@@ -724,8 +791,8 @@
     two_streams = bool(tok.is_cuda and cfg.MODEL.DYHEAD.get("LEVEL_STREAMS", True)) and trace is None
 
     def text_side(b, v_ln, prep):
-        hnew = vl_text_side(P, b, v_ln, prep, kv_len, max_kv)
-        return (hnew.to(tok.dtype), hnew) if h32 is not None else (hnew, None)
+        hnew, h16 = vl_text_side(P, b, v_ln, prep, kv_len, max_kv, want16=True)
+        return (h16 if h16 is not None else hnew.to(tok.dtype), hnew) if h32 is not None else (hnew, None)
 
     defer = ops.KERNELS["DYRELU_IN_LN"] == 1 and tok.shape[-1] == 256 and len(sizes) <= 8
     relu_coef = None
diff --git a/mq_det_amd/ops.py b/mq_det_amd/ops.py
--- a/mq_det_amd/ops.py
+++ b/mq_det_amd/ops.py
@@ -23,6 +23,7 @@
     "mq_gcp_sparse_attn_fwd": (_i, [_vp, _vp, _vp, _vp, _i, _i, _i, _i, _i, _i, _vp]),
     "mq_gcp_gate_residual_fwd": (_i, [_vp, _vp, _vp, _vp, _i, _vp, _vp, _l, _i, _i, _vp]),
     "mq_gcp_attn_fwd": (_i, [_vp] * 16 + [_l, _i, _i, _i, _i, _i, _i, _i, _f, _i, _vp]),
+    "mq_text_gemm_fwd": (_i, [_vp, _l, _vp, _vp, _i, _vp, _i, _vp, _vp, _vp, _vp, _l, _i, _i, _f, _f, _i, _vp]),
     "mq_vlfuse_i2t_fwd": (_i, [_vp, _vp, _vp, _l, _l, _l, _vp, _vp, _vp, _vp, _i, _i, _i, _i, _i, _f, _i, _vp]),
     "mq_vlfuse_t2i_workspace_bytes": (_l, [_i, _i, _i]),
     "mq_vlfuse_t2i_fwd": (_i, [_vp, _l, _l, _l, _vp, _vp, _vp, _l, _vp, _vp, _i, _i, _i, _i, _i, _i, _f, _i, _vp]),
@@ -69,7 +70,7 @@
     "mq_lvis_accumulate": (_i, [_vp] * 7 + [_i, _vp]),
     "mq_bank_admit": (_i, [_vp] * 8 + [_i] * 8 + [_f, _vp]),
 }
-BF16_TWINS = ("mq_attn_fwd", "mq_attn_resident_fwd", "mq_attn_text_fwd", "mq_bert_attn_qkv_fwd", "mq_patch_embed_fwd", "mq_attn_chunked_fwd", "mq_window_attn_fwd", "mq_window_attn_qkv_fwd", "mq_gcp_sparse_attn_fwd", "mq_gcp_gate_residual_fwd", "mq_gcp_attn_fwd", "mq_vlfuse_i2t_fwd", "mq_vlfuse_t2i_fwd",
+BF16_TWINS = ("mq_attn_fwd", "mq_attn_resident_fwd", "mq_attn_text_fwd", "mq_bert_attn_qkv_fwd", "mq_patch_embed_fwd", "mq_attn_chunked_fwd", "mq_window_attn_fwd", "mq_window_attn_qkv_fwd", "mq_gcp_sparse_attn_fwd", "mq_gcp_gate_residual_fwd", "mq_gcp_attn_fwd", "mq_text_gemm_fwd", "mq_vlfuse_i2t_fwd", "mq_vlfuse_t2i_fwd",
               "mq_layernorm_fwd", "mq_layernorm2_fwd", "mq_layernorm_clamp_fwd", "mq_clamp_gelu_clamp", "mq_patch_merge_ln_fwd", "mq_swin_mlp2_fwd", "mq_conv3x3_fwd", "mq_conv3x3_nchw32_fwd", "mq_conv3x3_nchw32_v2_fwd", "mq_conv3x3_nchw32_group_fwd", "mq_dcnv2_fwd", "mq_dcnv2_group_fwd",
               "mq_dyconv_stats", "mq_dyconv_coef", "mq_dyconv_coef_group", "mq_dyconv_fuse", "mq_dyrelu_coef", "mq_dyconv_epilogue_group", "mq_dyrelu_apply", "mq_dyrelu_ln_fwd", "mq_add_upsample_nearest", "mq_pool2x2_tokens_fwd",
               "mq_align_scores_fwd", "mq_align_fused_fwd", "mq_box_decode", "mq_roi_align_fwd", "mq_msdeform_attn_fwd", "mq_msdeform_attn_q_fwd")
@@ -492,6 +493,62 @@
     return res if len(res) > 1 else out
 
 
+TEXT_GEMM_BIAS_GELU, TEXT_GEMM_RESIDUAL_LN, TEXT_GEMM_RESIDUAL = 0, 1, 2
+TEXT_GEMM_ROWS_MAX_K = 768
+
+
+def text_gemm_fits(M, K, N, epilogue, policy=True):
+    if K <= 0 or K % 128 or K > 3072 or M <= 0:
+        return False
+    ok = (N > 0 and N % 256 == 0) if epilogue == TEXT_GEMM_BIAS_GELU else N == 768
+    if ok and policy:
+        sel = KERNELS.get("TEXT_GEMM_FUSED", 0)
+        ok = sel == 2 or (sel == 1 and M <= FUSED_TEXT_MAX_ROWS and not f32_operands()
+                          and (epilogue == TEXT_GEMM_BIAS_GELU or K <= TEXT_GEMM_ROWS_MAX_K))
+    return ok
+
+
+def text_gemm(a, wfrag, bias, epilogue, residual=None, ln=None, eps=1e-5, clamp=0.0, want_out=True, want_y=True, rows_per_block=0):
+    lib = load_library()
+    _need_gpu(a, wfrag, bias, residual)
+    K = a.shape[-1]
+    N = wfrag.shape[0] * 16
+    assert wfrag.dim() == 4 and wfrag.shape[1:] == (K // 32, 64, 8) and wfrag.is_contiguous() and wfrag.dtype == a.dtype and a.dtype in _H16
+    if a.is_contiguous():
+        lda = K
+    else:
+        assert a.dim() == 2 and a.stride(1) == 1, "mq_text_gemm_fwd takes one row stride"
+        lda = a.stride(0)
+    M = a.numel() // K
+    assert a.data_ptr() % 16 == 0 and (bias is None or (bias.dtype == a.dtype and bias.numel() == N and bias.is_contiguous()))
+    shape = tuple(a.shape[:-1]) + (N,)
+    y = out = None
+    r32 = False
+    if epilogue == TEXT_GEMM_BIAS_GELU:
+        y = torch.empty(shape, dtype=a.dtype, device=a.device)
+    else:
+        assert residual is not None and residual.numel() == M * N and residual.is_contiguous() and residual.dtype in (a.dtype, torch.float32)
+        r32 = residual.dtype == torch.float32
+        if epilogue == TEXT_GEMM_RESIDUAL_LN:
+            assert ln is not None and all(t.dtype == a.dtype and t.numel() == N and t.is_contiguous() for t in ln)
+            want_y = True
+        else:
+            want_out = True
+        if want_y:
+            y = torch.empty(shape, dtype=a.dtype, device=a.device)
+        if want_out:
+            out = torch.empty(shape, dtype=residual.dtype, device=a.device)
+    with _timed(f"text_gemm_e{epilogue}_k{K}_n{N}"):
+        rc = _fn(lib, "mq_text_gemm_fwd", a)(_ptr(a), lda, _ptr(wfrag), _ptr(bias), int(epilogue), _ptr(residual), int(r32),
+                                             _ptr(ln[0]) if ln is not None else _vp(0), _ptr(ln[1]) if ln is not None else _vp(0), _ptr(y), _ptr(out),
+                                             M, K, N, float(eps), float(clamp), int(rows_per_block), _stream())
+    _chk(rc, "mq_text_gemm_fwd")
+    if epilogue == TEXT_GEMM_BIAS_GELU:
+        return y
+    res = ((y,) + ((out,) if want_out else ())) if epilogue == TEXT_GEMM_RESIDUAL_LN else ((out,) + ((y,) if want_y else ()))
+    return res if len(res) > 1 else res[0]
+
+
 def gcp_gate_residual(sup, h, w2, x, want_gate=False):
     lib = load_library()
     _need_gpu(sup, h, w2, x)
diff --git a/mq_det_amd/selection.py b/mq_det_amd/selection.py
--- a/mq_det_amd/selection.py
+++ b/mq_det_amd/selection.py
@@ -22,6 +22,7 @@
     "LANG_SIDE_STREAMS": 0,
     "GCP_ATTN_FUSED": 1,
     "BERT_ATTN_QKV_FUSED": 1,
+    "TEXT_GEMM_FUSED": 1,
     "POST_FUSED": 1,
     "F32_OPERANDS": 0,
     "DCN_BDMA": 1,
```

Result: slower. 492.4 images/sec (-1.6%).
